# CloudEngineHub/dexrobot_isaac

Hardware: AMD Instinct MI355X
Metric: env-steps/sec BlindGrasping num_envs=4096 per MI355X (random actions) (higher is better)
Workload: dtype f32

## Files before the change

__graft_entry__.py:

```python
import os
import sys

ROOT = os.path.dirname(os.path.abspath(__file__))
if ROOT not in sys.path:
    sys.path.insert(0, ROOT)


def build():
    from dexrobot_isaac_amd.build import build_lib
    path = build_lib(force=True)
    from dexrobot_isaac_amd.build import build_debug_spin
    build_debug_spin(force=True)
    from oracle.oracle import build as build_oracle
    build_oracle(force=True)
    import dexrobot_isaac_amd
    from dexrobot_isaac_amd import _lib
    _lib.load()
    print(f"built {path}")


def smoke():
    import numpy as np
    import torch
    from dexrobot_isaac_amd.config import build_sim_config, default_cfg
    from dexrobot_isaac_amd.core import DexSimCore
    from oracle.oracle import Oracle
    cfg = default_cfg("BlindGrasping")
    cfg["env"]["numEnvs"] = 64
    sc, model = build_sim_config(cfg)
    ms = model.to_struct()
    core = DexSimCore(sc, ms, "cuda:0")
    orc = Oracle(sc, ms)
    core.reset()
    obs_ref = orc.reset()
    torch.cuda.synchronize()
    np.testing.assert_allclose(core.obs_buf.cpu().numpy(), obs_ref, atol=2e-4)
    rng = np.random.default_rng(0)
    for _ in range(3):
        a = (2 * rng.random((64, 18)) - 1).astype(np.float32)
        core.step(torch.as_tensor(a, device="cuda:0"))
        o_ref, r_ref, d_ref = orc.step(a)
        torch.cuda.synchronize()
        np.testing.assert_allclose(core.obs_buf.cpu().numpy(), o_ref, atol=5e-4)
        np.testing.assert_allclose(core.rew_buf.cpu().numpy(), r_ref, atol=5e-3, rtol=1e-4)
        assert (core.reset_buf.cpu().numpy() == d_ref).all()
    print("smoke ok: HIP step matches the CPU oracle")


if __name__ == "__main__":
    build()
```

dexrobot_isaac_amd/build.py:

```python
import os
import shutil
import subprocess

HERE = os.path.dirname(os.path.abspath(__file__))
CSRC = os.path.join(HERE, "csrc")
LIB = os.path.join(HERE, "libdexsim.so")
SOURCES = ["dexsim.hip", "dexsim_device.h", "dexsim_physics.hip.inc", "dexsim_l2.hip.inc", "dexsim_state.hip.inc",
           "dexsim_chain.hip.inc", "dexsim_render.hip.inc", "dexsim_kindyn.hip.inc", "dexsim_ik.hip.inc", "dexsim_proximity.hip.inc",
           "dexsim_invdyn.hip.inc"]


DEBUG_SPIN_LIB = os.path.join(HERE, "libdexsim_dbgspin.so")
CODEGEN_FLAGS = ["--offload-arch=gfx950", "-O3", "-fno-slp-vectorize", "-fno-hip-fp32-correctly-rounded-divide-sqrt",
                 "-mllvm", "-amdgpu-sched-strategy=max-ilp", "-std=c++17"]


def _stale(lib=LIB):
    if not os.path.exists(lib):
        return True
    t = os.path.getmtime(lib)
    deps = [os.path.join(CSRC, s) for s in SOURCES] + [os.path.join(HERE, "..", "include", "dexsim.h")]
    return any(os.path.getmtime(d) > t for d in deps if os.path.exists(d))


def build_debug_spin(force=False, bound=2000000):
    return build_lib(force=force, defs=(f"-DDEXSIM_DEBUG_SPIN={int(bound)}",), out=DEBUG_SPIN_LIB)


def build_lib(force=False, verbose=False, defs=(), out=None):
    lib = out or LIB
    if not force and not _stale(lib):
        return lib
    hipcc = shutil.which("hipcc") or "/opt/rocm/bin/hipcc"
    if not os.path.exists(hipcc):
        raise RuntimeError("hipcc not found: libdexsim.so cannot be built on this machine")
    cmd = [hipcc, *CODEGEN_FLAGS, "-fPIC", "-shared", *defs, "-o", lib, os.path.join(CSRC, "dexsim.hip")]
    if verbose:
        print(" ".join(cmd))
    subprocess.check_call(cmd, cwd=CSRC)
    return lib


if __name__ == "__main__":
    print(build_lib(force=True, verbose=True))
```

dexrobot_isaac_amd/csrc/dexsim_physics.hip.inc:

```

#define GPTR(p) ((__attribute__((address_space(1))) __typeof__(*(p))*)(p))
#define FLD(f, r) GPTR(A.f)[(size_t)(r) * N + e]
#define ROWADDR(w, lane) ((((w) >> 2) * 64 + (lane)) * 4 + ((w) & 3))

DI int wave_role(int w) { return w == 2 ? 5 : ((w >= 3 && w <= 5) ? w - 1 : w); }
#ifndef SPEC_SPLIT_NUM
#define SPEC_SPLIT_NUM 12
#endif

#define CODE_TYPE(c) ((c) & 3)
#define CODE_CAP(c) (((c) >> 2) & 31)
#define CODE_SAMPLE(c) (((c) >> 7) & 7)
#define CODE_FINGER(c) ((((c) >> 16) & 7) - 1)
#define CODE_LEVEL(c) (((c) >> 19) & 3)
#define CODE_FSLOT(c) (((c) >> 21) & 31)
DI int code_info(const DexHandModel& M, int cap) {
  const int jp = M.cap_parent[cap];
  return ((jp >= 6 ? ((jp - 6) >> 2) + 1 : 0) << 16) | ((jp >= 6 ? (jp - 6) & 3 : 0) << 19) | (M.cap_fslot[cap] << 21);
}
#define CODE_HKEY(c) (CODE_TYPE(c) == 3 ? 88 + ((CODE_FINGER(c) * 4 + CODE_LEVEL(c)) * 2 + (CODE_SAMPLE(c) & 1)) \
                                         : (CODE_CAP(c) * 2 + CODE_TYPE(c)) * 2 + (CODE_SAMPLE(c) & 1))
#define SPLIT_NB(s) ((s) & 15)
#define SPLIT_NX(s) (((s) >> 4) & 15)
#define SPLIT_NF(s, f) (((s) >> (8 + 4 * (f))) & 15)
#define SPLIT_RS(s) (((s) >> 28) & 1)
#define NP_TAG 0x40000000
#define NP_COUNT(w) (((w) >> 1) & 0x7f)
#define NP_TMASK(w) (((w) >> 8) & 0x7fff)
DI int split_pack(int nbg, const int (&cnt)[6], int hmask) {
  int nh = 0;
#pragma unroll
  for (int w = 0; w < 6; w++) nh += cnt[w];
  const int rs = nh > 12 ? 1 : 0;
  int split = max(1, (nh + rs) >> rs) | (rs << 28);
  int a = 0;
#pragma unroll
  for (int w = 0; w < 6; w++) {
    if (w < 5) split |= (cnt[w] > 0 ? (((a + cnt[w] - 1) >> rs) - (a >> rs) + 1) : 1) << (8 + 4 * w);
    a += cnt[w];
  }
  const int bmask = rs ? ((hmask | (hmask >> 1)) & 0x555555) : hmask;
  const int nX = (nbg > 0 ? 1 : 0) + __popc(bmask);
  return split | (max(nX, 1) << 4);
}
DI void push_contact(const Arena& A, int N, int e, int& nc, int type, int cap, int sample, V3 p, V3 n, float gap, float mu, int sw = -1,
                     int* tmask = nullptr, int cinfo = 0) {
  if (sw >= 0) {
    if (nc >= NP_STAGE) return;
    if (tmask && type == 1) *tmask |= 1 << nc;
    const int sc = sw * NP_STAGE + nc;
    *FQ(cstage, 2 * sc) = f4{p.x, p.y, p.z, n.x};
    *FQ(cstage, 2 * sc + 1) = f4{n.y, n.z, gap, mu};
    FLD(cstage, CSTAGE_CODE0 + sc) = __int_as_float(type | (cap << 2) | (sample << 7) | cinfo);
    nc++;
    return;
  }
  if (nc >= DEXSIM_KMAX) return;
  if (tmask && type == 1) *tmask |= 1 << nc;
  *FQ(cgeom, 2 * nc) = f4{p.x, p.y, p.z, n.x};
  *FQ(cgeom, 2 * nc + 1) = f4{n.y, n.z, gap, mu};
  FLD(ccode, nc) = type | (cap << 2) | (sample << 7) | cinfo;
  nc++;
}

DI void sphere_box(V3 P, float r, float hb, V3& nl, V3& pl, float& gapraw) {
  V3 qv = {clampf(P.x, -hb, hb), clampf(P.y, -hb, hb), clampf(P.z, -hb, hb)};
  V3 d = P - qv;
  float d2 = dot(d, d);
  if (d2 > 1e-12f) {
    float dist = sqrt_n(d2);
    nl = {div_n(d.x, dist), div_n(d.y, dist), div_n(d.z, dist)};
    pl = qv;
    gapraw = dist - r;
  } else {
    float px = hb - fabsf(P.x), py = hb - fabsf(P.y), pz = hb - fabsf(P.z);
    int ax = 0; float best = px;
    if (py < best) { best = py; ax = 1; }
    if (pz < best) { best = pz; ax = 2; }
    float c = ax == 0 ? P.x : (ax == 1 ? P.y : P.z);
    float sgn = c >= 0.f ? 1.f : -1.f;
    nl = {ax == 0 ? sgn : 0.f, ax == 1 ? sgn : 0.f, ax == 2 ? sgn : 0.f};
    pl = {ax == 0 ? sgn * hb : P.x, ax == 1 ? sgn * hb : P.y, ax == 2 ? sgn * hb : P.z};
    gapraw = -best - r;
  }
}

DI float seg_box_dfdt(V3 a, V3 d, float t, float hb) {
  V3 Pt = {a.x + t * d.x, a.y + t * d.y, a.z + t * d.z};
  V3 ex = {Pt.x - clampf(Pt.x, -hb, hb), Pt.y - clampf(Pt.y, -hb, hb), Pt.z - clampf(Pt.z, -hb, hb)};
  return ex.x * d.x + ex.y * d.y + ex.z * d.z;
}

DI void collide_capsule(const Arena& A, int N, int e, int& nc, const DexSimConfig& C, int cap, V3 e0, V3 e1, float r,
                        bool has_box, V3 bpos, const M3& Rb, float hb, float mu_hb, float mu_hg, int sw = -1, int* tmask = nullptr, int cinfo = 0) {
  const float co = C.contact_offset, rest = C.rest_offset;
  if (has_box) {
    V3 a = mulT(Rb, e0 - bpos), b = mulT(Rb, e1 - bpos), d = b - a;
    V3 mid = {0.5f * (a.x + b.x), 0.5f * (a.y + b.y), 0.5f * (a.z + b.z)};
    float reach = 0.5f * norm_n(d) + r + 1.7320508f * hb + co;
    bool near = dot(mid, mid) < reach * reach;
    if (__any(near)) {
      if (near) {
        float lo = 0.f, hi = 1.f;
#pragma unroll 4
        for (int it = 0; it < DEXSIM_BISECT_ITERS; it++) {
          float mdl = 0.5f * (lo + hi);
          if (seg_box_dfdt(a, d, mdl, hb) > 0.f) hi = mdl; else lo = mdl;
        }
        float ts = 0.5f * (lo + hi);
        const float tp = ts <= 0.02f ? 0.f : (ts >= 0.98f ? 1.f : ts);
        for (int s = 0; s < 2; s++) {
          float tc = s == 0 ? tp : (tp < 0.5f ? 1.f : 0.f);
          V3 Pc = {a.x + tc * d.x, a.y + tc * d.y, a.z + tc * d.z}, nl, pl;
          float gr;
          sphere_box(Pc, r, hb, nl, pl, gr);
          if (gr < co) push_contact(A, N, e, nc, 1, cap, s, mul(Rb, pl) + bpos, mul(Rb, nl), gr - rest, mu_hb, sw, tmask, cinfo);
        }
      }
    }
  }
  float z0 = e0.z - r, z1 = e1.z - r;
  if (z0 < co) push_contact(A, N, e, nc, 0, cap, 0, v3(e0.x, e0.y, z0), v3(0, 0, 1), z0 - rest, mu_hg, sw, tmask, cinfo);
  if (z1 < co) push_contact(A, N, e, nc, 0, cap, 1, v3(e1.x, e1.y, z1), v3(0, 0, 1), z1 - rest, mu_hg, sw, tmask, cinfo);
}

DI void collide_capsules3(const Arena& A, int N, int e, int& nc, const DexSimConfig& C, const int (&cap)[3], const V3 (&E0)[3],
                          const V3 (&E1)[3], const float (&r)[3], bool has_box, V3 bpos, const M3& Rb, float hb, float mu_hb, float mu_hg,
                          int sw, int* tmask, const int (&cinfo)[3]) {
  const float co = C.contact_offset, rest = C.rest_offset;
  V3 a[3], d[3];
  bool near[3] = {false, false, false};
  float ts[3] = {0.f, 0.f, 0.f};
  if (has_box) {
#pragma unroll
    for (int c = 0; c < 3; c++) {
      a[c] = mulT(Rb, E0[c] - bpos);
      const V3 b = mulT(Rb, E1[c] - bpos);
      d[c] = b - a[c];
      const V3 mid = {0.5f * (a[c].x + b.x), 0.5f * (a[c].y + b.y), 0.5f * (a[c].z + b.z)};
      const float reach = 0.5f * norm_n(d[c]) + r[c] + 1.7320508f * hb + co;
      near[c] = dot(mid, mid) < reach * reach;
    }
    if (__any(near[0] || near[1] || near[2])) {
      float lo[3] = {0.f, 0.f, 0.f}, hi[3] = {1.f, 1.f, 1.f};
#pragma unroll 2
      for (int it = 0; it < DEXSIM_BISECT_ITERS; it++) {
#pragma unroll
        for (int c = 0; c < 3; c++) {
          const float mdl = 0.5f * (lo[c] + hi[c]);
          if (seg_box_dfdt(a[c], d[c], mdl, hb) > 0.f) hi[c] = mdl; else lo[c] = mdl;
        }
      }
#pragma unroll
      for (int c = 0; c < 3; c++) ts[c] = 0.5f * (lo[c] + hi[c]);
    }
  }
#pragma unroll
  for (int c = 0; c < 3; c++) {
    const V3 ac = a[c], dc = d[c], e0 = E0[c], e1 = E1[c];
    const float rc = r[c], tsc = ts[c];
    const bool nr = near[c];
    const int capc = cap[c], ci = cinfo[c];
    if (has_box && nr) {
      const float tp = tsc <= 0.02f ? 0.f : (tsc >= 0.98f ? 1.f : tsc);
      for (int s = 0; s < 2; s++) {
        const float tc = s == 0 ? tp : (tp < 0.5f ? 1.f : 0.f);
        V3 Pc = {ac.x + tc * dc.x, ac.y + tc * dc.y, ac.z + tc * dc.z}, nl, pl;
        float gr;
        sphere_box(Pc, rc, hb, nl, pl, gr);
        if (gr < co) push_contact(A, N, e, nc, 1, capc, s, mul(Rb, pl) + bpos, mul(Rb, nl), gr - rest, mu_hb, sw, tmask, ci);
      }
    }
    const float z0 = e0.z - rc, z1 = e1.z - rc;
    if (z0 < co) push_contact(A, N, e, nc, 0, capc, 0, v3(e0.x, e0.y, z0), v3(0, 0, 1), z0 - rest, mu_hg, sw, tmask, ci);
    if (z1 < co) push_contact(A, N, e, nc, 0, capc, 1, v3(e1.x, e1.y, z1), v3(0, 0, 1), z1 - rest, mu_hg, sw, tmask, ci);
  }
}


struct BaseChain {
  V3 ab[6], ob[6];
  float qb[6], qdb[6];
  Q4 q5;
  V3 o5, w5, al5, ao5;
};

DI Q4 qmul_axis_y(Q4 a, float s, float c) {
  return {fmaf(-a.z, s, mulr(a.x, c)), fmaf(a.y, c, mulr(a.w, s)), fmaf(a.z, c, mulr(a.x, s)), fmaf(-a.y, s, mulr(a.w, c))};
}
DI Q4 qmul_axis_z(Q4 a, float s, float c) {
  return {fmaf(a.y, s, mulr(a.x, c)), fmaf(a.y, c, -mulr(a.x, s)), fmaf(a.z, c, mulr(a.w, s)), fmaf(-a.z, s, mulr(a.w, c))};
}
DI V3 q2mat_col_y(Q4 q) {
  return {2.f * fmaf(q.x, q.y, -mulr(q.z, q.w)), fmaf(fmaf(q.z, q.z, mulr(q.x, q.x)), -2.f, 1.f), 2.f * fmaf(q.y, q.z, mulr(q.x, q.w))};
}
DI V3 q2mat_col_z(Q4 q) {
  return {2.f * fmaf(q.x, q.z, mulr(q.y, q.w)), 2.f * fmaf(q.y, q.z, -mulr(q.x, q.w)), fmaf(fmaf(q.y, q.y, mulr(q.x, q.x)), -2.f, 1.f)};
}

template <bool MS>
DI void base_chain(const Arena& A, const DevParams* __restrict__ P, V3 grav, int N, int e, BaseChain& B, bool write_jframe,
                   const float* s_q = nullptr, const float* s_qd = nullptr, int lane = 0) {
#pragma unroll
  for (int j = 0; j < 6; j++) {
    if (s_q) { B.qb[j] = s_q[j * 64 + lane]; B.qdb[j] = s_qd[j * 64 + lane]; }
    else { B.qb[j] = FLD(q, j); B.qdb[j] = FLD(qd, j); }
  }
  V3 t = {0, 0, 0};
#pragma unroll
  for (int j = 0; j < 4; j++) {
    const V3 Aj = v3p(P->base_A[j]);
    if (j < 3) t += B.qb[j] * Aj;
    B.ab[j] = Aj;
    B.ob[j] = v3p(P->base_Oc[j]) + t;
  }
  Q4 qc;
  {
    const V3 ax = v3p(P->jc[3].axis);
    float s, c;
    sincos_joint(0.5f * B.qb[3], &s, &c);
    qc = qmul(q4p(P->base_Q3z), Q4{ax.x * s, ax.y * s, ax.z * s, c});
  }
  V3 oc = B.ob[3];
  V3 w = B.qdb[3] * B.ab[3], al = {0, 0, 0}, ao = {-grav.x, -grav.y, -grav.z};
#pragma unroll
  for (int j = 4; j < 6; j++) {
    if (MS) {
      const V3 aw = j == 4 ? q2mat_col_y(qc) : q2mat_col_z(qc);
      float s, c;
      sincos_joint(0.5f * B.qb[j], &s, &c);
      const Q4 qn = j == 4 ? qmul_axis_y(qc, s, c) : qmul_axis_z(qc, s, c);
      const V3 cw = cross(w, aw);
      al += B.qdb[j] * cw; w += B.qdb[j] * aw;
      B.ab[j] = aw; B.ob[j] = oc; qc = qn;
      continue;
    }
    M3 Rp = q2mat(qc);
    V3 on = oc + mul(Rp, v3p(P->jc[j].poff));
    Q4 qz = qmul(qc, q4p(P->jc[j].qoff));
    V3 ax = v3p(P->jc[j].axis);
    V3 aw = mul(q2mat(qz), ax);
    float s, c;
    sincos_joint(0.5f * B.qb[j], &s, &c);
    Q4 qn = qmul(qz, Q4{ax.x * s, ax.y * s, ax.z * s, c});
    V3 r = on - oc;
    V3 aoj = ao + cross(al, r) + cross(w, cross(w, r));
    V3 cw = cross(w, aw);
    al += B.qdb[j] * cw; w += B.qdb[j] * aw;
    ao = aoj; B.ab[j] = aw; B.ob[j] = on; qc = qn; oc = on;
  }
  B.q5 = qc; B.o5 = oc; B.w5 = w; B.al5 = al; B.ao5 = ao;
  if (write_jframe) {
#pragma unroll
    for (int j = 0; j < 6; j++) {
      FLD(jframe, 6 * j + 0) = B.ab[j].x; FLD(jframe, 6 * j + 1) = B.ab[j].y; FLD(jframe, 6 * j + 2) = B.ab[j].z;
      FLD(jframe, 6 * j + 3) = B.ob[j].x; FLD(jframe, 6 * j + 4) = B.ob[j].y; FLD(jframe, 6 * j + 5) = B.ob[j].z;
    }
  }
}

DI bool hand_clear(const DevParams* __restrict__ P, const BaseChain& B, V3 bpos) {
  const DexSimConfig& C = P->cfg;
  const float reach = P->hand_reach, co = C.contact_offset;
  bool clear = B.o5.z - reach > co;
  if (C.has_box) {
    const V3 d = B.o5 - bpos;
    const float rr = reach + 0.8660254f * C.box_size * 1.001f + co;
    clear = clear && dot(d, d) > rr * rr;
  }
  return __all(clear);
}

DI bool capsule_clear(V3 e0, V3 e1, float r, const DexSimConfig& C, V3 bpos, const M3& Rb) {
  const float co = C.contact_offset;
  bool clear = !((e0.z - r) < co) && !((e1.z - r) < co);
  if (C.has_box) {
    const V3 d = e1 - e0;
    const V3 mid = mulT(Rb, V3{0.5f * (e0.x + e1.x) - bpos.x, 0.5f * (e0.y + e1.y) - bpos.y, 0.5f * (e0.z + e1.z) - bpos.z});
    const float hb = 0.5f * C.box_size;
    const V3 ex = {mid.x - clampf(mid.x, -hb, hb), mid.y - clampf(mid.y, -hb, hb), mid.z - clampf(mid.z, -hb, hb)};
    const float reach = (0.5f * norm_n(d) + r + co) * 1.0001f + 1e-6f;
    clear = clear && !(dot(ex, ex) < reach * reach);
  }
  return clear;
}

#define SH(i) sh[(i) * 64 + lane]
DI void sh_put3(float* sh, int lane, int i, V3 v) { SH(i) = v.x; SH(i + 1) = v.y; SH(i + 2) = v.z; }
DI void comp_put(float* sh, int lane, int w, const Comp& c, V3 o5) {
  const V3 d = c.c - o5;
  const S6 J = c.I + pa(c.m, d);
  sh[(w) * 64 + lane] = c.m; sh_put3(sh, lane, w + 1, d);
  sh[(w + 4) * 64 + lane] = J.xx; sh[(w + 5) * 64 + lane] = J.yy; sh[(w + 6) * 64 + lane] = J.zz;
  sh[(w + 7) * 64 + lane] = J.xy; sh[(w + 8) * 64 + lane] = J.xz; sh[(w + 9) * 64 + lane] = J.yz;
}
DI V3 sh_get3(const float* sh, int lane, int i) { return {SH(i), SH(i + 1), SH(i + 2)}; }
DI void bch_get2(const float* s_bch, int lane, int i2, V3& a0, V3& o0, V3& a1, V3& o1) {
  const f4 q0 = *(const f4*)(s_bch + ROWADDR(12 * i2, lane)), q1 = *(const f4*)(s_bch + ROWADDR(12 * i2 + 4, lane)),
           q2 = *(const f4*)(s_bch + ROWADDR(12 * i2 + 8, lane));
  a0 = {q0.x, q0.y, q0.z}; o0 = {q0.w, q1.x, q1.y}; a1 = {q1.z, q1.w, q2.x}; o1 = {q2.y, q2.z, q2.w};
}


#define DL_SINV 0
#define DL_SCHUR_S 0
#define DL_SCHUR_GSUM 27
#define DL_PALM 36
#define DL_PALM_WRENCH 46
#define DL_NC 52
#define DL_PERSIST 53
#define DL_SSUB(b, f) ((b) + (f) * 43)
#define DL_GSUM(b, f) ((b) + (f) * 43 + 21)
#define DL_COMP(b, f) ((b) + (f) * 43 + 27)
#define DL_WRENCH(b, f) ((b) + (f) * 43 + 37)
#define DL_CAPS(b, f) ((b) + 215 + (f) * 18)
#define DL_HANDOFF 305
#define DL_WORDS (DL_PERSIST + DL_HANDOFF)
#define DL_SPLIT DL_WORDS

#define FS_UB 53
#define FS_BOXV 59
#define FS_UF 65
#define FS_LAM 85
#define FS_HDR 157
#define FS_ROW 197
#define FS_HDR_HI 197
#define FS_X 253
#define FS_FORCE 253
#define FS_T 513
#define FS_SPRE 513
#define FS_SPRE_BIAS 534
#define FS_BCH 545
#define FS_CTAB 581
#define FS_NITEM 593
#define FS_CMP 594
#define FS_CARRY_QD 606
#define FS_CARRY_BP 612
#define FS_COMPCNT 615
#define FS_GEN 617
#define FS_SPLIT 618
#define FS_CPACK 619
#define FS_CMP_INVM 620
#define FS_FLAG 622
#define FS_CARRY_Q 628
#define FS_TGTB 634
#define FS_WORDS 640
#define FS_LDS_BYTES (FS_WORDS * 64 * sizeof(float))

enum : unsigned { LIVE_ACROSS = 1u << 6, LIVE_PUB = 1u << 7, LIVE_POST = 1u << 8 };
constexpr unsigned lds_live(int first, int last) {
  unsigned m = 0;
  for (int p = first; p <= last; p++) m |= 1u << (p == 0 ? 1 : p);
  return m;
}
constexpr unsigned LIVE_CARRY = lds_live(5, 5) | LIVE_ACROSS | lds_live(0, 0);
constexpr unsigned LIVE_LAUNCH = lds_live(0, 5) | LIVE_ACROSS;
struct LdsRegion { int start, words; unsigned live; };
constexpr LdsRegion LDS_MAP[] = {
  {DL_SINV,      36,                      lds_live(2, 3)},
  {DL_PALM,      16,                      lds_live(1, 2)},
  {DL_NC,        1,                       lds_live(1, 5)},
  {FS_UB,        6,                       lds_live(2, 5)},
  {FS_BOXV,      6,                       lds_live(1, 5)},
  {FS_UF,        20,                      lds_live(1, 5)},
  {FS_LAM,       3 * DEXSIM_KMAX,         lds_live(1, 5)},
  {FS_HDR,       FS_HDR_HI - FS_HDR,      lds_live(1, 5)},
  {FS_ROW,       DL_HANDOFF,              lds_live(1, 2)},
  {FS_HDR_HI,    4 * DEXSIM_KMAX - (FS_HDR_HI - FS_HDR), lds_live(3, 5)},
  {FS_X,         13 * 5 * 4,              lds_live(3, 4)},
  {FS_FORCE,     5 * 3 * DEXSIM_NFSLOT,   lds_live(5, 5)},
  {FS_T,         8 * 4,                   lds_live(3, 4)},
  {FS_SPRE,      27,                      lds_live(1, 2)},
  {FS_BCH,       36,                      lds_live(1, 3)},
  {FS_CTAB,      12,                      lds_live(2, 4)},
  {FS_NITEM,     1,                       lds_live(2, 4)},
  {FS_CMP,       12,                      lds_live(1, 4)},
  {FS_CARRY_QD,  6,                       LIVE_CARRY},
  {FS_CARRY_BP,  3,                       LIVE_CARRY},
  {FS_COMPCNT,   1,                       LIVE_LAUNCH},
  {FS_GEN,       1,                       lds_live(1, 4)},
  {FS_SPLIT,     1,                       lds_live(2, 4)},
  {FS_CPACK,     1,                       lds_live(1, 4)},
  {FS_CMP_INVM,  2,                       lds_live(1, 4)},
  {FS_FLAG,      6,                       LIVE_LAUNCH},
  {FS_CARRY_Q,   6,                       LIVE_CARRY},
  {FS_TGTB,      6,                       lds_live(1, 2)},
};
constexpr int lds_map_conflict(LdsRegion extra = {0, 0, 0}) {
  constexpr int n = sizeof(LDS_MAP) / sizeof(LDS_MAP[0]);
  for (int i = 0; i <= n; i++) {
    const LdsRegion a = i < n ? LDS_MAP[i] : extra;
    if (a.start < 0 || a.words < 0 || a.start + a.words > FS_WORDS) return 1000 * (a.start < 0 ? 0 : a.start) + 999;
    for (int j = 0; j < i; j++) {
      const LdsRegion b = LDS_MAP[j];
      if ((a.live & b.live) && a.start < b.start + b.words && b.start < a.start + a.words) return 1000 * a.start + b.start;
    }
  }
  return -1;
}
static_assert(FS_LDS_BYTES == 160 * 1024, "the sub-step kernels own the CU's whole LDS: one workgroup per CU");
static_assert(lds_map_conflict() < 0, "LDS map: a region leaves the LDS or shares a word with a region live in a common phase "
                                      "(the note shows 1000 x the first word of one + the first word of the other)");
static_assert(DL_CAPS(0, 5) == DL_HANDOFF, "the per-finger hand-off is DL_HANDOFF words");
#define SOLVE_LDS_WORDS(kstage) (60 + DEXSIM_KMAX * 3 + DEXSIM_KMAX * 4 + (kstage) * 3 * CROW_W)
static_assert((DL_SPLIT + 1) * 64 * sizeof(float) <= FS_LDS_BYTES, "k_dynamics' LDS does not fit into the CU's");
static_assert(SOLVE_LDS_WORDS(4) * 64 * sizeof(float) <= FS_LDS_BYTES, "k_solve's LDS does not fit into the CU's");

struct FingerIn { float ql[4], qdl[4], tg[4]; };
DI void finger_load(const Arena& A, int f, int N, int e, FingerIn& in) {
#pragma unroll
  for (int l = 0; l < 4; l++) { const int j = 6 + 4 * f + l; in.ql[l] = FLD(q, j); in.qdl[l] = FLD(qd, j); in.tg[l] = FLD(targets, j); }
}

template <bool MS>
DI bool finger_dynamics(const Arena& A, const DevParams* __restrict__ P, const BaseChain& B, const FingerIn& in, float* sh, const int dlb,
                        float* s_uf, int lane, int f, int N, int e, int tok_seq = 0, bool sphere_clear = false,
                        V3 bpos = V3{0, 0, 0}, const M3& Rb = M3{{1, 0, 0, 0, 1, 0, 0, 0, 1}}, float* Gk = nullptr) {
  const DexHandModel& M = P->model;
  const float h = P->h;
  const int j0 = 6 + 4 * f;
  Q4 qf = B.q5; V3 of = B.o5; V3 wf = B.w5, alf = B.al5, aof = B.ao5;
  V3 a[4], o[4], cl[4], fl[4], nl[4];
  S6 Iw[4];
  float ql[4], qdl[4], tg[4];
  bool clr = true;
  if (tok_seq > 0 && sphere_clear && lane == 0) sh[(FS_FLAG + f) * 64] = __int_as_float((tok_seq << 1) | 1);
#pragma unroll
  for (int l = 0; l < 4; l++) {
    const int j = j0 + l;
    ql[l] = in.ql[l]; qdl[l] = in.qdl[l]; tg[l] = in.tg[l];
    M3 Rp = q2mat(qf);
    V3 on = of + mul(Rp, v3p(P->jc[j].poff));
    Q4 qz = qmul(qf, q4p(P->jc[j].qoff));
    V3 ax = v3p(P->jc[j].axis);
    float s, c;
    sincos_joint(0.5f * ql[l], &s, &c);
    Q4 qn = qmul(qz, Q4{ax.x * s, ax.y * s, ax.z * s, c});
    M3 R = q2mat(qn);
    V3 aw = MS && l >= 1 ? V3{mulr(R.m[1], ax.y), mulr(R.m[4], ax.y), mulr(R.m[7], ax.y)} : mul(R, ax);
    V3 r = on - of;
    V3 aoj = aof + cross(alf, r) + cross(wf, cross(wf, r));
    V3 cw = cross(wf, aw);
    alf += qdl[l] * cw; wf += qdl[l] * aw; aof = aoj;
    cl[l] = on + mul(R, v3p(P->jc[j].com));
    Iw[l] = (tok_seq > 0 && P->inertia_diag) ? rotate_inertia_diag(R, P->jc[j].inertia) : rotate_inertia(R, P->jc[j].inertia);
    V3 rc = cl[l] - on;
    V3 ac = aof + cross(alf, rc) + cross(wf, cross(wf, rc));
    fl[l] = P->jc[j].mass * ac;
    nl[l] = mul(Iw[l], alf) + cross(wf, mul(Iw[l], wf)) + cross(rc, fl[l]);
    if (l >= 1 && !(tok_seq > 0 && sphere_clear)) {
      const int cap = 3 + 3 * f + (l - 1);
      const V3 c0 = on + mul(R, v3p(M.cap_p0[cap])), c1 = on + mul(R, v3p(M.cap_p1[cap]));
      sh_put3(sh, lane, DL_CAPS(dlb, f) + 6 * (l - 1), c0);
      sh_put3(sh, lane, DL_CAPS(dlb, f) + 6 * (l - 1) + 3, c1);
      if (tok_seq > 0) clr = clr && capsule_clear(c0, c1, M.cap_r[cap], P->cfg, bpos, Rb);
    }
    a[l] = aw; o[l] = on; qf = qn; of = on;
  }
  bool fclear = false;
  if (tok_seq > 0) {
    fclear = sphere_clear || __all(clr);
    if (!sphere_clear && lane == 0) sh[(FS_FLAG + f) * 64] = __int_as_float((tok_seq << 1) | (fclear ? 1 : 0));
  }
  if (!fclear) {
    const float w24[24] = {a[0].x, a[0].y, a[0].z, o[0].x, o[0].y, o[0].z, a[1].x, a[1].y, a[1].z, o[1].x, o[1].y, o[1].z,
                           a[2].x, a[2].y, a[2].z, o[2].x, o[2].y, o[2].z, a[3].x, a[3].y, a[3].z, o[3].x, o[3].y, o[3].z};
#pragma unroll
    for (int qd = 0; qd < 6; qd++) *FQ(jframe, JFRAME_FQ0 + 6 * f + qd) = f4{w24[4 * qd], w24[4 * qd + 1], w24[4 * qd + 2], w24[4 * qd + 3]};
  }
  float bias[4];
#pragma unroll
  for (int l = 3; l >= 0; l--) {
    bias[l] = dot(a[l], nl[l]);
    if (l > 0) { fl[l - 1] += fl[l]; nl[l - 1] += nl[l] + cross(o[l] - o[l - 1], fl[l]); }
  }
  sh_put3(sh, lane, DL_WRENCH(dlb, f), fl[0]);
  sh_put3(sh, lane, DL_WRENCH(dlb, f) + 3, nl[0] + cross(o[0] - B.o5, fl[0]));
  float Fm[16], Cm[24];
  Comp cc;
#pragma unroll
  for (int l = 3; l >= 0; l--) {
    Comp b; b.m = P->jc[j0 + l].mass; b.c = cl[l]; b.I = Iw[l];
    if (l == 3) cc = b; else { comp_add(b, cc); cc = b; }
    V3 Pm = cc.m * cross(a[l], cc.c - o[l]);
    V3 Lm = mul(cc.I, a[l]);
#pragma unroll
    for (int k = 0; k <= l; k++) {
      float v = dot(a[k], Lm + cross(cc.c - o[k], Pm));
      Fm[l * 4 + k] = v; Fm[k * 4 + l] = v;
    }
    if (MS) {
      const V3 Xm = Lm + cross(cc.c - B.ob[3], Pm);
      Cm[l] = Pm.x; Cm[4 + l] = Pm.y; Cm[8 + l] = Pm.z;
#pragma unroll
      for (int i = 3; i < 6; i++) Cm[i * 4 + l] = dot(B.ab[i], Xm);
    } else {
#pragma unroll
      for (int i = 0; i < 6; i++)
        Cm[i * 4 + l] = i < 3 ? dot(B.ab[i], Pm) : dot(B.ab[i], Lm + cross(cc.c - B.ob[i], Pm));
    }
  }
  comp_put(sh, lane, DL_COMP(dlb, f), cc, B.o5);
  if (tok_seq > 0) {
    asm volatile("" ::: "memory");
    if (lane == 0) __hip_atomic_fetch_add((int*)(sh + FS_COMPCNT * 64), 1, __ATOMIC_RELAXED, __HIP_MEMORY_SCOPE_WORKGROUP);
  }
  float tau[4];
#pragma unroll
  for (int l = 0; l < 4; l++) {
    const int j = j0 + l;
    const float kp = P->jc[j].kp, kdh = P->jc[j].kd + h * kp;
    Fm[l * 4 + l] += P->jc[j].armature + h * kdh;
    tau[l] = kp * (tg[l] - ql[l]) - kdh * qdl[l] - bias[l];
  }
  spd_inverse<4>(Fm);
  float G[24];
  f2 G2[12];
#pragma unroll
  for (int l = 0; l < 4; l++)
#pragma unroll
    for (int ip = 0; ip < 3; ip++) {
      f2 s2 = {0.f, 0.f};
#pragma unroll
      for (int k = 0; k < 4; k++) s2 = f2{Cm[(2 * ip) * 4 + k], Cm[(2 * ip + 1) * 4 + k]} * Fm[l * 4 + k] + s2;
      G2[l * 3 + ip] = s2;
      G[l * 6 + 2 * ip] = s2.x; G[l * 6 + 2 * ip + 1] = s2.y;
    }
  if (!(tok_seq > 0 && sphere_clear && Gk)) {
#pragma unroll
    for (int qd = 0; qd < 6; qd++) *FQ(fac_g, 6 * f + qd) = f4{G[4 * qd], G[4 * qd + 1], G[4 * qd + 2], G[4 * qd + 3]};
  }
  if (Gk) {
#pragma unroll
    for (int i = 0; i < 24; i++) Gk[i] = G[i];
  }
#pragma unroll
  for (int i = 0; i < 6; i++)
#pragma unroll
    for (int kp = 0; kp <= i / 2; kp++) {
      f2 s2 = {0.f, 0.f};
#pragma unroll
      for (int l = 0; l < 4; l++) s2 = G2[l * 3 + kp] * Cm[i * 4 + l] + s2;
      SH(DL_SSUB(dlb, f) + i * (i + 1) / 2 + 2 * kp) = s2.x;
      if (2 * kp + 1 <= i) SH(DL_SSUB(dlb, f) + i * (i + 1) / 2 + 2 * kp + 1) = s2.y;
    }
  if (!fclear) {
    *FQ(fac_finv, 3 * f) = f4{Fm[0], Fm[4], Fm[5], Fm[8]};
    *FQ(fac_finv, 3 * f + 1) = f4{Fm[9], Fm[10], Fm[12], Fm[13]};
    *FQ(fac_finv, 3 * f + 2) = f4{Fm[14], Fm[15], 0.f, 0.f};
  }
#pragma unroll
  for (int ip = 0; ip < 3; ip++) {
    f2 s2 = {0.f, 0.f};
#pragma unroll
    for (int l = 0; l < 4; l++) s2 = G2[l * 3 + ip] * tau[l] + s2;
    SH(DL_GSUM(dlb, f) + 2 * ip) = s2.x; SH(DL_GSUM(dlb, f) + 2 * ip + 1) = s2.y;
  }
#pragma unroll
  for (int l = 0; l < 4; l++) {
    float s = qdl[l];
#pragma unroll
    for (int i = 0; i < 6; i++) s += G[l * 6 + i] * B.qdb[i];
    float acc = 0.f;
#pragma unroll
    for (int k = 0; k < 4; k++) acc += Fm[l * 4 + k] * tau[k];
    const float uf = s + h * acc;
    if (s_uf) s_uf[(4 * f + l) * 64 + lane] = uf;
    else FLD(ufree, j0 + l) = uf;
  }
  return fclear;
}

#define SCHUR_SPLIT_BIT (1 << 30)
#ifdef DEXSIM_DEBUG_SPIN
#define SPIN_GUARD_INIT() int spin_polls_ = 0
#define SPIN_GUARD(cntp, site, seq) if (++spin_polls_ > (DEXSIM_DEBUG_SPIN)) { if (cntp) GPTR(cntp)[CNT_SPIN_TIMEOUT] = ((site) << 24) | (seq); break; }
#else
#define SPIN_GUARD_INIT() do {} while (0)
#define SPIN_GUARD(cntp, site, seq) do {} while (0)
#endif
DI Comp schur_comp(const float* sh, const int dlb, int lane, V3 o5) {
  float M = SH(DL_PALM);
  V3 sd = M * sh_get3(sh, lane, DL_PALM + 1);
  S6 J = {SH(DL_PALM + 4), SH(DL_PALM + 5), SH(DL_PALM + 6), SH(DL_PALM + 7), SH(DL_PALM + 8), SH(DL_PALM + 9)};
#pragma unroll
  for (int f = 0; f < 5; f++) {
    const float mf = SH(DL_COMP(dlb, f));
    M += mf;
    sd += mf * sh_get3(sh, lane, DL_COMP(dlb, f) + 1);
    J = J + S6{SH(DL_COMP(dlb, f) + 4), SH(DL_COMP(dlb, f) + 5), SH(DL_COMP(dlb, f) + 6), SH(DL_COMP(dlb, f) + 7), SH(DL_COMP(dlb, f) + 8), SH(DL_COMP(dlb, f) + 9)};
  }
  const float inv = M > 0.f ? 1.f / M : 0.f;
  const V3 d = inv * sd;
  const S6 sh_back = pa(M, d);
  Comp c;
  c.m = M; c.c = o5 + d;
  c.I = {J.xx - sh_back.xx, J.yy - sh_back.yy, J.zz - sh_back.zz, J.xy - sh_back.xy, J.xz - sh_back.xz, J.yz - sh_back.yz};
  return c;
}
template <int i, int k0 = 0, int k1 = i>
DI void schur_row(float* sh, const int dlb, int lane) {
  float r[k1 - k0 + 1];
#pragma unroll
  for (int k = k0; k <= k1; k++) {
    const float v = SH(FS_SPRE + i * (i + 1) / 2 + k);
    float ss = 0.f;
#pragma unroll
    for (int f = 0; f < 5; f++) ss += SH(DL_SSUB(dlb, f) + i * (i + 1) / 2 + k);
    r[k - k0] = v - ss;
  }
#pragma unroll
  for (int k = k0; k <= k1; k++) SH(DL_SCHUR_S + i * (i + 1) / 2 + k) = r[k - k0];
}
DI void schur_precompute(float* sh, const int dlb, int lane, const BaseChain& B, int seq, int* dbg_cnt) {
  {
    SPIN_GUARD_INIT();
    while (*(volatile int*)(sh + FS_COMPCNT * 64) < 5 * seq) { __builtin_amdgcn_s_sleep(2); SPIN_GUARD(dbg_cnt, 4, seq); }
  }
  asm volatile("" ::: "memory");
  const Comp comp5 = schur_comp(sh, dlb, lane, B.o5);
  int idx = 0;
#pragma unroll
  for (int i = 0; i < 6; i++) {
    V3 Pm, Lm;
    if (i < 3) { Pm = comp5.m * B.ab[i]; Lm = {0, 0, 0}; }
    else { Pm = comp5.m * cross(B.ab[i], comp5.c - B.ob[i]); Lm = mul(comp5.I, B.ab[i]); }
#pragma unroll
    for (int k = 0; k <= i; k++) {
      SH(FS_SPRE + idx) = k < 3 ? dot(B.ab[k], Pm) : dot(B.ab[k], Lm + cross(comp5.c - B.ob[k], Pm));
      idx++;
    }
  }
  V3 ff = sh_get3(sh, lane, DL_PALM_WRENCH), nn = sh_get3(sh, lane, DL_PALM_WRENCH + 3);
#pragma unroll
  for (int f = 0; f < 5; f++) {
    ff += sh_get3(sh, lane, DL_WRENCH(dlb, f));
    nn += sh_get3(sh, lane, DL_WRENCH(dlb, f) + 3);
  }
  SH(FS_SPRE_BIAS + 5) = dot(B.ab[5], nn);
#pragma unroll
  for (int j = 4; j >= 0; j--) {
    nn += cross(B.ob[j + 1] - B.ob[j], ff);
    SH(FS_SPRE_BIAS + j) = j < 3 ? dot(B.ab[j], ff) : dot(B.ab[j], nn);
  }
}
DI void schur_helper(float* sh, const int dlb, int job, int lane) {
  if (job == 1) {
    float gsum[6] = {0, 0, 0, 0, 0, 0};
#pragma unroll
    for (int f = 0; f < 5; f++)
#pragma unroll
      for (int i = 0; i < 6; i++) gsum[i] += SH(DL_GSUM(dlb, f) + i);
#pragma unroll
    for (int i = 0; i < 6; i++) SH(DL_SCHUR_GSUM + i) = gsum[i];
    schur_row<0>(sh, dlb, lane); schur_row<1>(sh, dlb, lane); schur_row<2>(sh, dlb, lane);
  } else if (job == 0) {
    schur_row<3>(sh, dlb, lane); schur_row<5, 4, 5>(sh, dlb, lane);
  } else schur_row<4>(sh, dlb, lane);
}

DI void schur_base(const Arena& A, const DevParams* __restrict__ P, const BaseChain& B, float* sh, const int dlb, float* uB_out,
                   int lane, int N, int e, int tgt_lds = -1, bool solve_only = false, int split_seq = 0,
                   unsigned long long dbg_t0 = 0, int dbg_row = 0, int* dbg_cnt = nullptr) {
#if defined(DEXSIM_PROFILE_PHASES) && defined(DBG_SCHUR)
#define SCHUR_STAMP(i) do { if (lane == 0) A.crow[(size_t)(dbg_row + (i)) * N + e] = __int_as_float((int)(__builtin_amdgcn_s_memtime() - dbg_t0)); } while (0)
#else
#define SCHUR_STAMP(i) do {} while (0)
#endif
  const float h = P->h;
  SCHUR_STAMP(0);
  Comp comp5;
  V3 f5 = sh_get3(sh, lane, DL_PALM_WRENCH), n5 = sh_get3(sh, lane, DL_PALM_WRENCH + 3);
  float Ssub[21], gsum[6] = {0, 0, 0, 0, 0, 0};
#pragma unroll
  for (int i = 0; i < 21; i++) Ssub[i] = 0.f;
  if (split_seq == 0) comp5 = schur_comp(sh, dlb, lane, B.o5);
  if (split_seq == 0) {
#pragma unroll
    for (int f = 0; f < 5; f++) {
      f5 += sh_get3(sh, lane, DL_WRENCH(dlb, f));
      n5 += sh_get3(sh, lane, DL_WRENCH(dlb, f) + 3);
#pragma unroll
      for (int i = 0; i < 21; i++) Ssub[i] += SH(DL_SSUB(dlb, f) + i);
#pragma unroll
      for (int i = 0; i < 6; i++) gsum[i] += SH(DL_GSUM(dlb, f) + i);
    }
  }
  SCHUR_STAMP(1);
  float S[36];
  if (split_seq > 0) schur_row<5, 0, 3>(sh, dlb, lane);
  else {
    int idx = 0;
#pragma unroll
    for (int i = 0; i < 6; i++) {
      V3 Pm, Lm;
      if (i < 3) { Pm = comp5.m * B.ab[i]; Lm = {0, 0, 0}; }
      else { Pm = comp5.m * cross(B.ab[i], comp5.c - B.ob[i]); Lm = mul(comp5.I, B.ab[i]); }
#pragma unroll
      for (int k = 0; k <= i; k++) {
        float v = k < 3 ? dot(B.ab[k], Pm) : dot(B.ab[k], Lm + cross(comp5.c - B.ob[k], Pm));
        v -= Ssub[idx++];
        S[i * 6 + k] = v; S[k * 6 + i] = v;
      }
    }
  }
  SCHUR_STAMP(2);
  float tauB[6];
  float bias[6];
  if (split_seq > 0) {
    const int want = (split_seq << 1) | 1 | SCHUR_SPLIT_BIT;
#pragma unroll 1
    for (int w = 1; w <= 3; w++) {
      SPIN_GUARD_INIT();
      while (__float_as_int(*(volatile float*)(sh + (FS_FLAG + w) * 64)) != want) { __builtin_amdgcn_s_sleep(1); SPIN_GUARD(dbg_cnt, 1, split_seq); }
    }
    asm volatile("" ::: "memory");
    SCHUR_STAMP(3);
    {
      int idx = 0;
#pragma unroll
      for (int i = 0; i < 6; i++)
#pragma unroll
        for (int k = 0; k <= i; k++) {
          const float v = SH(DL_SCHUR_S + idx); idx++;
          S[i * 6 + k] = v; S[k * 6 + i] = v;
        }
    }
#pragma unroll
    for (int i = 0; i < 6; i++) { bias[i] = SH(FS_SPRE_BIAS + i); gsum[i] = SH(DL_SCHUR_GSUM + i); }
  } else {
    V3 nn = n5, ff = f5;
    bias[5] = dot(B.ab[5], nn);
#pragma unroll
    for (int j = 4; j >= 0; j--) {
      nn += cross(B.ob[j + 1] - B.ob[j], ff);
      bias[j] = j < 3 ? dot(B.ab[j], ff) : dot(B.ab[j], nn);
    }
  }
  {
#pragma unroll
    for (int i = 0; i < 6; i++) {
      const float kp = P->jc[i].kp, kdh = P->jc[i].kd + h * kp;
      S[i * 6 + i] += P->jc[i].armature + h * kdh;
      const float tgt = tgt_lds >= 0 ? SH(tgt_lds + i) : FLD(targets, i);
      tauB[i] = kp * (tgt - B.qb[i]) - kdh * B.qdb[i] - bias[i] - gsum[i];
    }
  }
  SCHUR_STAMP(4);
  if (solve_only) {
    float x[6];
    spd_solve<6>(S, tauB, x);
#pragma unroll
    for (int i = 0; i < 6; i++) uB_out[i] = B.qdb[i] + h * x[i];
    SCHUR_STAMP(5);
    return;
  }
  spd_inverse<6>(S);
#pragma unroll
  for (int qd = 0; qd < 9; qd++) *(f4*)(sh + DL_SINV * 64 + ROWADDR(4 * qd, lane)) = f4{S[4 * qd], S[4 * qd + 1], S[4 * qd + 2], S[4 * qd + 3]};
#pragma unroll
  for (int i = 0; i < 6; i++) {
    float acc = 0.f;
#pragma unroll
    for (int k = 0; k < 6; k++) acc += S[i * 6 + k] * tauB[k];
    const float ub = B.qdb[i] + h * acc;
    if (uB_out) uB_out[i] = ub;
    else FLD(ufree, i) = ub;
  }
}

template <bool FUSED>
DI void build_contact_rows(const Arena& A, const DevParams* __restrict__ P, const BaseChain* B, float* sh, int lane, int k, int N, int e,
                           int split, int gen) {
  const DexSimConfig& C = P->cfg;
  const float h = P->h;
  const f4 cg0 = *FQ(cgeom, 2 * k), cg1 = *FQ(cgeom, 2 * k + 1);
  const V3 p = {cg0.x, cg0.y, cg0.z};
  const V3 n = {cg0.w, cg1.x, cg1.y};
  const float gap = cg1.z, mu_k = cg1.w;
  const int code = FLD(ccode, k), type = CODE_TYPE(code);
  float inv_m = 0.f, inv_I = 0.f;
  V3 bpos = {0, 0, 0};
  if (C.has_box) {
    if (!C.box_fixed) { inv_m = rcp_n(FLD(box_mass, 0)); inv_I = P->box_inv_I_k * inv_m; }
    bpos = {FLD(box_pos, 0), FLD(box_pos, 1), FLD(box_pos, 2)};
  }
  const int f = type != 2 ? CODE_FINGER(code) : -1, lvl = f >= 0 ? CODE_LEVEL(code) : -1;
  const int nFi = (split && f >= 0) ? SPLIT_NF(split, f) : 1;
  const float nB = split ? (float)SPLIT_NB(split) : 1.f, nX = split ? (float)SPLIT_NX(split) : 1.f, nF = (float)nFi;
  f4 wq = {0.f, 0.f, 0.f, 0.f};
  if (gen >= 0) wq = *(const __attribute__((address_space(1))) f4*)(A.wlam + ((size_t)(type == 2 ? 80 + k : CODE_HKEY(code)) * N + e) * 4);
  float jfr[24], G[24], Fi[10];
  if (f >= 0) {
    const unsigned qs = (unsigned)N * 16u, oe = (unsigned)e * 16u;
    const unsigned oj = (unsigned)(JFRAME_FQ0 + 6 * f) * qs + oe, og = (unsigned)(6 * f) * qs + oe, of = (unsigned)(3 * f) * qs + oe;
    f4 qj[6], qg[6], qf[3];
#pragma unroll
    for (int qd = 0; qd < 6; qd++) {
      qj[qd] = *(const __attribute__((address_space(1))) f4*)((const char*)A.jframe + (oj + (unsigned)qd * qs));
      qg[qd] = *(const __attribute__((address_space(1))) f4*)((const char*)A.fac_g + (og + (unsigned)qd * qs));
    }
#pragma unroll
    for (int qd = 0; qd < 3; qd++) qf[qd] = *(const __attribute__((address_space(1))) f4*)((const char*)A.fac_finv + (of + (unsigned)qd * qs));
#pragma unroll
    for (int qd = 0; qd < 6; qd++) {
      jfr[4 * qd] = qj[qd].x; jfr[4 * qd + 1] = qj[qd].y; jfr[4 * qd + 2] = qj[qd].z; jfr[4 * qd + 3] = qj[qd].w;
      G[4 * qd] = qg[qd].x; G[4 * qd + 1] = qg[qd].y; G[4 * qd + 2] = qg[qd].z; G[4 * qd + 3] = qg[qd].w;
    }
    Fi[0] = qf[0].x; Fi[1] = qf[0].y; Fi[2] = qf[0].z; Fi[3] = qf[0].w; Fi[4] = qf[1].x; Fi[5] = qf[1].y; Fi[6] = qf[1].z; Fi[7] = qf[1].w;
    Fi[8] = qf[2].x; Fi[9] = qf[2].y;
  }
  const bool lim = type == 3;
  V3 dir[3];
  dir[0] = n;
  tangent_basis(lim ? v3(0, 0, 1) : n, dir[1], dir[2]);
  if (lim) { dir[1] = v3(0, 0, 0); dir[2] = v3(0, 0, 0); }
  float t[3][6], jf[3][4], St[3][6], Fj[3][4];
#pragma unroll
  for (int r = 0; r < 3; r++) {
#pragma unroll
    for (int i = 0; i < 6; i++) { t[r][i] = 0.f; St[r][i] = 0.f; }
#pragma unroll
    for (int l = 0; l < 4; l++) { jf[r][l] = 0.f; Fj[r][l] = 0.f; }
  }
  float Dq[3] = {0.f, 0.f, 0.f};
  float A10 = 0.f, A20 = 0.f, A21 = 0.f;
  if (type != 2) {
#pragma unroll
    for (int i2 = 0; i2 < 3; i2++) {
      V3 aa[2], oo[2];
      if (FUSED) {
        bch_get2(sh + FS_BCH * 64, lane, i2, aa[0], oo[0], aa[1], oo[1]);
      } else { aa[0] = B->ab[2 * i2]; oo[0] = B->ob[2 * i2]; aa[1] = B->ab[2 * i2 + 1]; oo[1] = B->ob[2 * i2 + 1]; }
#pragma unroll
      for (int h = 0; h < 2; h++) {
        const int i = 2 * i2 + h;
        const V3 ci = i < 3 ? aa[h] : cross(aa[h], p - oo[h]);
#pragma unroll
        for (int r = 0; r < 3; r++) t[r][i] = dot(dir[r], ci);
      }
    }
    if (f >= 0) {
#pragma unroll
      for (int l = 0; l < 4; l++) {
        const V3 al = {jfr[6 * l], jfr[6 * l + 1], jfr[6 * l + 2]}, ol = {jfr[6 * l + 3], jfr[6 * l + 4], jfr[6 * l + 5]};
        const V3 cl = cross(al, p - ol);
#pragma unroll
        for (int r = 0; r < 3; r++) jf[r][l] = l <= lvl ? dot(dir[r], cl) : 0.f;
        if (lim) jf[0][l] = l == lvl ? (CODE_SAMPLE(code) ? -1.f : 1.f) : 0.f;
      }
#pragma unroll
      for (int l = 0; l < 4; l++)
#pragma unroll
        for (int i = 0; i < 6; i++)
#pragma unroll
          for (int r = 0; r < 3; r++) t[r][i] -= G[l * 6 + i] * jf[r][l];
#pragma unroll
      for (int l = 0; l < 4; l++)
#pragma unroll
        for (int kk = 0; kk < 4; kk++) {
          const float fv = Fi[l >= kk ? l * (l + 1) / 2 + kk : kk * (kk + 1) / 2 + l];
#pragma unroll
          for (int r = 0; r < 3; r++) Fj[r][l] += fv * jf[r][kk];
        }
#pragma unroll
      for (int r = 0; r < 3; r++) {
        float s = 0.f;
#pragma unroll
        for (int l = 0; l < 4; l++) s += jf[r][l] * Fj[r][l];
        Dq[r] += nF * s;
      }
      A10 += nF * (jf[1][0] * Fj[0][0] + jf[1][1] * Fj[0][1] + jf[1][2] * Fj[0][2] + jf[1][3] * Fj[0][3]);
      A20 += nF * (jf[2][0] * Fj[0][0] + jf[2][1] * Fj[0][1] + jf[2][2] * Fj[0][2] + jf[2][3] * Fj[0][3]);
      A21 += nF * (jf[2][0] * Fj[1][0] + jf[2][1] * Fj[1][1] + jf[2][2] * Fj[1][2] + jf[2][3] * Fj[1][3]);
    }
#pragma unroll
    for (int i2 = 0; i2 < 3; i2++) {
      const f4 s0 = *(const f4*)(sh + DL_SINV * 64 + ROWADDR(12 * i2, lane)), s1 = *(const f4*)(sh + DL_SINV * 64 + ROWADDR(12 * i2 + 4, lane)),
               s2 = *(const f4*)(sh + DL_SINV * 64 + ROWADDR(12 * i2 + 8, lane));
      const float si[12] = {s0.x, s0.y, s0.z, s0.w, s1.x, s1.y, s1.z, s1.w, s2.x, s2.y, s2.z, s2.w};
#pragma unroll
      for (int h = 0; h < 2; h++)
#pragma unroll
        for (int r = 0; r < 3; r++) {
          float s = 0.f;
#pragma unroll
          for (int kk = 0; kk < 6; kk++) s += si[6 * h + kk] * t[r][kk];
          St[r][2 * i2 + h] = s;
        }
    }
#pragma unroll
    for (int r = 0; r < 3; r++) {
      float s = 0.f;
#pragma unroll
      for (int i = 0; i < 6; i++) s += t[r][i] * St[r][i];
      Dq[r] += nB * s;
    }
    {
      float s10 = 0.f, s20 = 0.f, s21 = 0.f;
#pragma unroll
      for (int i = 0; i < 6; i++) { s10 += t[1][i] * St[0][i]; s20 += t[2][i] * St[0][i]; s21 += t[2][i] * St[1][i]; }
      A10 += nB * s10; A20 += nB * s20; A21 += nB * s21;
    }
  }
  V3 db[3], rxd[3];
#pragma unroll
  for (int r = 0; r < 3; r++) { db[r] = {0, 0, 0}; rxd[r] = {0, 0, 0}; }
  if (type == 1 || type == 2) {
    const float sgn = type == 2 ? 1.f : -1.f;
    const V3 rb = p - bpos;
#pragma unroll
    for (int r = 0; r < 3; r++) {
      const V3 c = cross(rb, dir[r]);
      db[r] = sgn * dir[r]; rxd[r] = sgn * c;
      Dq[r] += nX * (inv_m + inv_I * dot(c, c));
    }
    const float xm = nX * inv_m, xI = nX * inv_I;
    A10 += xm * dot(db[1], db[0]) + xI * dot(rxd[1], rxd[0]);
    A20 += xm * dot(db[2], db[0]) + xI * dot(rxd[2], rxd[0]);
    A21 += xm * dot(db[2], db[1]) + xI * dot(rxd[2], rxd[1]);
  }
#pragma unroll
  for (int r = 0; r < 3; r++) {
    const float Dinv = (lim && r > 0) ? 0.f : 1.f / (Dq[r] + 1e-9f);
    const float pad = r == 0 ? A10 : (r == 1 ? A20 : A21);
    const int rw = (k * 3 + r) * CROW_W;
    if (FUSED) {
      float* qb = A.crowq + ((size_t)(k * 21 + r * 7) * N + e) * 4;
      st4_global(qb, t[r][0], t[r][1], t[r][2], t[r][3]);
      st4_global(qb + (size_t)1 * N * 4, t[r][4], t[r][5], jf[r][0], jf[r][1]);
      st4_global(qb + (size_t)2 * N * 4, jf[r][2], jf[r][3], St[r][0], St[r][1]);
      st4_global(qb + (size_t)3 * N * 4, St[r][2], St[r][3], St[r][4], St[r][5]);
      st4_global(qb + (size_t)4 * N * 4, Fj[r][0], Fj[r][1], Fj[r][2], Fj[r][3]);
      st4_global(qb + (size_t)5 * N * 4, db[r].x, db[r].y, db[r].z, rxd[r].x);
      st4_global(qb + (size_t)6 * N * 4, rxd[r].y, rxd[r].z, Dinv, pad);
    } else {
#pragma unroll
      for (int i = 0; i < 6; i++) { FLD(crow, rw + i) = t[r][i]; FLD(crow, rw + 10 + i) = St[r][i]; }
#pragma unroll
      for (int l = 0; l < 4; l++) { FLD(crow, rw + 6 + l) = jf[r][l]; FLD(crow, rw + 16 + l) = Fj[r][l]; }
      FLD(crow, rw + 20) = db[r].x; FLD(crow, rw + 21) = db[r].y; FLD(crow, rw + 22) = db[r].z;
      FLD(crow, rw + 23) = rxd[r].x; FLD(crow, rw + 24) = rxd[r].y; FLD(crow, rw + 25) = rxd[r].z;
      FLD(crow, rw + 26) = Dinv; FLD(crow, rw + 27) = pad;
    }
  }
  const float cb = gap > 0.f ? div_n(gap, h) : -fminf(div_n(-gap * C.erp, h), C.max_depenetration_velocity);
  const bool warm = gen >= 0 && __float_as_int(wq.w) == 8 * gen + (type == 2 ? CODE_SAMPLE(code) : 0);
  if (!FUSED) {
    FLD(clam, 3 * k) = warm ? wq.x : 0.f; FLD(clam, 3 * k + 1) = warm ? wq.y : 0.f; FLD(clam, 3 * k + 2) = warm ? wq.z : 0.f;
    FLD(chdr, 8 * k + 0) = __int_as_float(code | (nFi << 12));
    FLD(chdr, 8 * k + 1) = __int_as_float(f >= 0 ? 4 * f : -1);
    FLD(chdr, 8 * k + 2) = mu_k;
    FLD(chdr, 8 * k + 3) = cb;
  }
  FLD(chdr, 8 * k + 4) = __int_as_float(CODE_FSLOT(code));
  FLD(chdr, 8 * k + 5) = n.x; FLD(chdr, 8 * k + 6) = n.y; FLD(chdr, 8 * k + 7) = n.z;
  if (FUSED) {
    float* s_hdr = sh + FS_HDR * 64;
    float* s_lam = sh + FS_LAM * 64;
    s_hdr[(4 * k) * 64 + lane] = __int_as_float(code | (nFi << 12)); s_hdr[(4 * k + 1) * 64 + lane] = __int_as_float(f >= 0 ? 4 * f : -1);
    s_hdr[(4 * k + 2) * 64 + lane] = mu_k; s_hdr[(4 * k + 3) * 64 + lane] = cb;
    s_lam[(3 * k) * 64 + lane] = warm ? wq.x : 0.f; s_lam[(3 * k + 1) * 64 + lane] = warm ? wq.y : 0.f;
    s_lam[(3 * k + 2) * 64 + lane] = warm ? wq.z : 0.f;
  }
}

__global__ __launch_bounds__(384) void k_dynamics(Arena A, const DevParams* __restrict__ P, int N) {
  __shared__ __attribute__((aligned(16))) float sh[(DL_SPLIT + 1) * 64];
  constexpr int dlb = DL_PERSIST;
  const int wv = threadIdx.x >> 6, lane = threadIdx.x & 63;
  const int e = blockIdx.x * 64 + lane;
  const DexHandModel& M = P->model;
  const DexSimConfig& C = P->cfg;
  const V3 grav = v3p(C.gravity);
  const bool has_box = C.has_box != 0;
  BaseChain B;
  FingerIn fin;
  if (wv < 5) finger_load(A, wv, N, e, fin);
  base_chain<false>(A, P, grav, N, e, B, wv == 5);

  int nc = 0;
  V3 bpos = {0, 0, 0}; M3 Rb = q2mat(Q4{0, 0, 0, 1});
  float hb = 0.f, bmu = 0.f;
  if (wv < 5) {
    finger_dynamics<false>(A, P, B, fin, sh, dlb, nullptr, lane, wv, N, e);
  } else {
    const M3 R5 = q2mat(B.q5);
    Comp comp5;
    comp5.m = P->jc[5].mass;
    comp5.c = B.o5 + mul(R5, v3p(P->jc[5].com));
    comp5.I = rotate_inertia(R5, P->jc[5].inertia);
    V3 rc = comp5.c - B.o5;
    V3 ac = B.ao5 + cross(B.al5, rc) + cross(B.w5, cross(B.w5, rc));
    V3 f5 = comp5.m * ac;
    V3 n5 = mul(comp5.I, B.al5) + cross(B.w5, mul(comp5.I, B.w5)) + cross(rc, f5);
    comp_put(sh, lane, DL_PALM, comp5, B.o5);
    sh_put3(sh, lane, DL_PALM_WRENCH, f5); sh_put3(sh, lane, DL_PALM_WRENCH + 3, n5);
    const float h = P->h;
    if (has_box) {
      bpos = {FLD(box_pos, 0), FLD(box_pos, 1), FLD(box_pos, 2)};
      Rb = q2mat(Q4{FLD(box_quat, 0), FLD(box_quat, 1), FLD(box_quat, 2), FLD(box_quat, 3)});
      hb = 0.5f * C.box_size;
      bmu = FLD(box_mu, 0);
      const float mu_bg = 0.5f * (bmu + C.ground_friction);
#pragma unroll
      for (int i = 0; i < 8; i++) {
        V3 l = {(i & 1) ? hb : -hb, (i & 2) ? hb : -hb, (i & 4) ? hb : -hb};
        V3 p = mul(Rb, l) + bpos;
        if (!C.box_fixed && p.z < C.contact_offset && nc < 4) push_contact(A, N, e, nc, 2, 0, i, p, v3(0, 0, 1), p.z - C.rest_offset, mu_bg, -1, nullptr, DEXSIM_FSLOT_BOX << 21);
      }
      const float hg = C.box_fixed ? 0.f : h;
      FLD(ufree, 26) = FLD(box_lin, 0) + hg * grav.x;
      FLD(ufree, 27) = FLD(box_lin, 1) + hg * grav.y;
      FLD(ufree, 28) = FLD(box_lin, 2) + hg * grav.z;
      FLD(ufree, 29) = FLD(box_ang, 0); FLD(ufree, 30) = FLD(box_ang, 1); FLD(ufree, 31) = FLD(box_ang, 2);
    } else {
#pragma unroll
      for (int i = 26; i < 32; i++) FLD(ufree, i) = 0.f;
    }
  }
  __syncthreads();

  if (wv == 0) schur_base(A, P, B, sh, dlb, nullptr, lane, N, e);
  if (wv == 5) {
    const float mu_hg = 0.5f * (M.hand_friction + C.ground_friction);
    const float mu_hb = 0.5f * (M.hand_friction + bmu);
    const int nbg = nc;
    int cntw[6], tmask = 0;
#pragma unroll 1
    for (int f = 0; f < 5; f++) {
      const int n0 = nc;
#pragma unroll 1
      for (int l = 3; l >= 1; l--) {
        const int cap = 3 + 3 * f + (l - 1);
        const V3 e0 = sh_get3(sh, lane, DL_CAPS(dlb, f) + 6 * (l - 1)), e1 = sh_get3(sh, lane, DL_CAPS(dlb, f) + 6 * (l - 1) + 3);
        collide_capsule(A, N, e, nc, C, cap, e0, e1, M.cap_r[cap], has_box, bpos, Rb, hb, mu_hb, mu_hg, -1, &tmask, code_info(M, cap));
      }
      if (f == 0) cntw[0] = nc - n0; else if (f == 1) cntw[1] = nc - n0; else if (f == 2) cntw[2] = nc - n0; else if (f == 3) cntw[3] = nc - n0; else cntw[4] = nc - n0;
    }
    const M3 R5 = q2mat(B.q5);
    const int n5 = nc;
#pragma unroll 1
    for (int cpl = 0; cpl < 3; cpl++)
      collide_capsule(A, N, e, nc, C, cpl, B.o5 + mul(R5, v3p(M.cap_p0[cpl])), B.o5 + mul(R5, v3p(M.cap_p1[cpl])), M.cap_r[cpl],
                      has_box, bpos, Rb, hb, mu_hb, mu_hg, -1, &tmask, code_info(M, cpl));
    cntw[5] = nc - n5;
    FLD(ncontact, 0) = nc;
    SH(DL_NC) = __int_as_float(nc);
    const int split = split_pack(nbg, cntw, (int)((unsigned)tmask >> nbg));
    FLD(csplit, 0) = split;
    SH(DL_SPLIT) = __int_as_float(split);
  }
  __syncthreads();

  nc = __float_as_int(SH(DL_NC));
  int kmax = nc;
#pragma unroll
  for (int s = 32; s >= 1; s >>= 1) kmax = max(kmax, __shfl_xor(kmax, s));
  const int split = __float_as_int(SH(DL_SPLIT)), gen = FLD(wgen, 0);
#pragma unroll 1
  for (int k = wv; k < kmax; k += 6) {
    if (k < nc) build_contact_rows<false>(A, P, &B, sh, lane, k, N, e, split, gen);
  }
}

DI void solve_masks(const float* s_hdr, int nc, int kmax, int lane, unsigned& hand_mask, unsigned& fing_mask, unsigned& box_mask) {
  hand_mask = fing_mask = box_mask = 0;
  for (int k = 0; k < kmax; k++) {
    const int code = __float_as_int(s_hdr[(4 * k) * 64 + lane]), fo = __float_as_int(s_hdr[(4 * k + 1) * 64 + lane]);
    const int type = code & 3;
    const bool act = k < nc;
    if (__any(act && type != 2)) hand_mask |= 1u << k;
    if (__any(act && type != 2 && fo >= 0)) fing_mask |= 1u << k;
    if (__any(act && type != 0)) box_mask |= 1u << k;
  }
}

struct BoxBlock {
  float rx[4], ry[4], rz[4];
  float Dv[4][3], A10[4], A20[4], A21[4], mu4[4], cb4[4], lam4[4][3];
  float im, iI;
  int kms;
  template <bool QUAD>
  DI void load(int kmax, float inv_m, float inv_I, const float* s_lam, const float* s_hdr, const float* rows, int rw, int ro, int lane,
               int nc_lane, bool resume, float split = 1.f) {
    kms = __builtin_amdgcn_readfirstlane(kmax);
    inv_m *= split; inv_I *= split;
    im = inv_m; iI = inv_I;
#pragma unroll
    for (int k = 0; k < 4; k++) {
      const bool use = k < kms && (nc_lane < 0 || k < nc_lane);
      float x = 0.f, y = 0.f, z = 0.f;
      if (k < kms) {
        if (QUAD) {
          y = rows[ROWADDR((k * 3) * rw + ro + 3, lane)]; x = -rows[ROWADDR((k * 3) * rw + ro + 4, lane)];
          z = rows[ROWADDR((k * 3 + 1) * rw + ro + 3, lane)];
        } else {
          x = rows[(3 * k) * 64 + lane]; y = rows[(3 * k + 1) * 64 + lane]; z = rows[(3 * k + 2) * 64 + lane];
        }
      }
      rx[k] = use ? x : 0.f; ry[k] = use ? y : 0.f; rz[k] = use ? z : 0.f;
      mu4[k] = use ? s_hdr[(4 * k + 2) * 64 + lane] : 0.f;
      cb4[k] = use ? s_hdr[(4 * k + 3) * 64 + lane] : 0.f;
#pragma unroll
      for (int r = 0; r < 3; r++) lam4[k][r] = (use && resume) ? s_lam[(3 * k + r) * 64 + lane] : 0.f;
      const float xx = rx[k] * rx[k], yy = ry[k] * ry[k], zz = rz[k] * rz[k];
      Dv[k][0] = use ? 1.f / (inv_m + inv_I * (xx + yy) + 1e-9f) : 0.f;
      Dv[k][1] = use ? 1.f / (inv_m + inv_I * (xx + zz) + 1e-9f) : 0.f;
      Dv[k][2] = use ? 1.f / (inv_m + inv_I * (yy + zz) + 1e-9f) : 0.f;
      A10[k] = inv_I * ry[k] * rz[k]; A20[k] = -inv_I * rx[k] * rz[k]; A21[k] = inv_I * rx[k] * ry[k];
    }
  }
  DI bool sweep(f2& v01, f2& v23, f2& v45) {
    float vx = v01.x, vy = v01.y, vz = v23.x, wx = v23.y, wy = v45.x, wz = v45.y;
    bool chg = false;
#pragma unroll
    for (int k = 0; k < 4; k++) {
      if (k < kms) {
        const float vr0 = vz + ry[k] * wx - rx[k] * wy;
        float vr1 = -vy + rz[k] * wx - rx[k] * wz, vr2 = vx + rz[k] * wy - ry[k] * wz;
        const float nl0 = fmaxf(0.f, lam4[k][0] - (vr0 + cb4[k]) * Dv[k][0]);
        const float dl0 = nl0 - lam4[k][0], lim = mu4[k] * nl0;
        vr1 += A10[k] * dl0; vr2 += A20[k] * dl0;
        const float nl1 = __builtin_amdgcn_fmed3f(lam4[k][1] - vr1 * Dv[k][1], -lim, lim);
        const float dl1 = nl1 - lam4[k][1];
        vr2 += A21[k] * dl1;
        const float nl2 = __builtin_amdgcn_fmed3f(lam4[k][2] - vr2 * Dv[k][2], -lim, lim);
        const float dl2 = nl2 - lam4[k][2];
        lam4[k][0] = nl0; lam4[k][1] = nl1; lam4[k][2] = nl2;
        chg = chg || dl0 != 0.f || dl1 != 0.f || dl2 != 0.f;
        apply(k, dl0, dl1, dl2, f2{im, iI}, vx, vy, vz, wx, wy, wz);
      }
    }
    v01 = f2{vx, vy}; v23 = f2{vz, wx}; v45 = f2{wy, wz};
    return chg;
  }
  DI void sweep_delta(f2& v01, f2& v23, f2& v45, f2& d01, f2& d23, f2& d45, f2 mI0) {
    float vx = v01.x, vy = v01.y, vz = v23.x, wx = v23.y, wy = v45.x, wz = v45.y;
    float dx = 0.f, dy = 0.f, dz = 0.f, ex = 0.f, ey = 0.f, ez = 0.f;
#pragma unroll
    for (int k = 0; k < 4; k++) {
      if (k < kms) {
        const float vr0 = vz + ry[k] * wx - rx[k] * wy;
        float vr1 = -vy + rz[k] * wx - rx[k] * wz, vr2 = vx + rz[k] * wy - ry[k] * wz;
        const float nl0 = fmaxf(0.f, lam4[k][0] - (vr0 + cb4[k]) * Dv[k][0]);
        const float dl0 = nl0 - lam4[k][0], lim = mu4[k] * nl0;
        vr1 += A10[k] * dl0; vr2 += A20[k] * dl0;
        const float nl1 = __builtin_amdgcn_fmed3f(lam4[k][1] - vr1 * Dv[k][1], -lim, lim);
        const float dl1 = nl1 - lam4[k][1];
        vr2 += A21[k] * dl1;
        const float nl2 = __builtin_amdgcn_fmed3f(lam4[k][2] - vr2 * Dv[k][2], -lim, lim);
        const float dl2 = nl2 - lam4[k][2];
        lam4[k][0] = nl0; lam4[k][1] = nl1; lam4[k][2] = nl2;
        apply(k, dl0, dl1, dl2, f2{im, iI}, vx, vy, vz, wx, wy, wz);
        apply(k, dl0, dl1, dl2, mI0, dx, dy, dz, ex, ey, ez);
      }
    }
    v01 = f2{vx, vy}; v23 = f2{vz, wx}; v45 = f2{wy, wz};
    d01 = f2{dx, dy}; d23 = f2{dz, ex}; d45 = f2{ey, ez};
  }
  DI void apply(int k, float dl0, float dl1, float dl2, f2 mI, float& vx, float& vy, float& vz, float& wx, float& wy, float& wz) const {
    const float m0 = mI.x * dl0, m1 = mI.x * dl1, m2 = mI.x * dl2, i0 = mI.y * dl0, i1 = mI.y * dl1, i2 = mI.y * dl2;
    vz += m0; vy -= m1; vx += m2;
    wx += ry[k] * i0 + rz[k] * i1;
    wy += rz[k] * i2 - rx[k] * i0;
    wz -= rx[k] * i1 + ry[k] * i2;
  }
  DI void warm(f2& v01, f2& v23, f2& v45, f2 mI) const {
    float vx = v01.x, vy = v01.y, vz = v23.x, wx = v23.y, wy = v45.x, wz = v45.y;
#pragma unroll
    for (int k = 0; k < 4; k++) {
      if (k < kms) apply(k, lam4[k][0], lam4[k][1], lam4[k][2], mI, vx, vy, vz, wx, wy, wz);
    }
    v01 = f2{vx, vy}; v23 = f2{vz, wx}; v45 = f2{wy, wz};
  }
  DI void store(float* s_lam, int lane, int nmine = -1) const {
#pragma unroll
    for (int k = 0; k < 4; k++) {
      if (nmine < 0 || k < nmine) {
#pragma unroll
        for (int r = 0; r < 3; r++) s_lam[(3 * k + r) * 64 + lane] = lam4[k][r];
      }
    }
  }
};

DI void cache_box_ground(const Arena& A, const float* s_lam, int gen, int cpack, int nmine, int lane, int N, int e) {
#pragma unroll
  for (int k = 0; k < 4; k++) {
    if (k < nmine)
      st4_global(A.wlam + ((size_t)(80 + k) * N + e) * 4, s_lam[(3 * k) * 64 + lane], s_lam[(3 * k + 1) * 64 + lane], s_lam[(3 * k + 2) * 64 + lane],
                 __int_as_float(8 * gen + ((cpack >> (3 * k)) & 7)));
  }
}

DI void solve_forces(const Arena& A, const DevParams* __restrict__ P, int* __restrict__ cnt, const float* s_hdr, const float* s_lam,
                     float* s_f, int nc, int lane, int N, int e, int NR) {
  const float h = P->h;
#pragma unroll
  for (int i = 0; i < DEXSIM_NFSLOT * 3; i++) s_f[i * 64 + lane] = 0.f;
  int nhand = 0;
  for (int k = 0; k < nc; k++) {
    const int type = __float_as_int(s_hdr[(4 * k) * 64 + lane]) & 3;
    nhand += type < 2 ? 1 : 0;
    if (type == 3) continue;
    const int slot = __float_as_int(FLD(chdr, 8 * k + 4));
    const V3 n = {FLD(chdr, 8 * k + 5), FLD(chdr, 8 * k + 6), FLD(chdr, 8 * k + 7)};
    V3 t1, t2;
    tangent_basis(n, t1, t2);
    const float l0 = s_lam[(3 * k) * 64 + lane] / h, l1 = s_lam[(3 * k + 1) * 64 + lane] / h, l2 = s_lam[(3 * k + 2) * 64 + lane] / h;
    const V3 F = l0 * n + l1 * t1 + l2 * t2;
    s_f[(3 * slot) * 64 + lane] += F.x; s_f[(3 * slot + 1) * 64 + lane] += F.y; s_f[(3 * slot + 2) * 64 + lane] += F.z;
    if (type == 1) {
      s_f[(3 * DEXSIM_FSLOT_BOX) * 64 + lane] -= F.x; s_f[(3 * DEXSIM_FSLOT_BOX + 1) * 64 + lane] -= F.y;
      s_f[(3 * DEXSIM_FSLOT_BOX + 2) * 64 + lane] -= F.z;
    }
  }
#pragma unroll
  for (int i = 0; i < DEXSIM_NFSLOT * 3; i++) FLD(cforce, i) = s_f[i * 64 + lane];
  if (cnt) {
    int tot = e < NR ? (nc | (nhand << 16)) : 0;
#pragma unroll
    for (int s = 32; s >= 1; s >>= 1) tot += __shfl_xor(tot, s);
    if (lane == 0) { atomicAdd(&cnt[CNT_CONTACTS], tot & 0xffff); if (tot >> 16) atomicAdd(&cnt[CNT_HAND_CONTACTS], tot >> 16); }
  }
}

DI void solve_forces_box(const Arena& A, const DevParams* __restrict__ P, int* __restrict__ cnt, const float* s_lam, int nc, int lane, int N,
                         int e, int NR) {
  const float h = P->h;
  V3 n = v3(0, 0, 1), t1, t2;
  tangent_basis(n, t1, t2);
  V3 acc = {0.f, 0.f, 0.f};
  for (int k = 0; k < nc; k++) {
    const float l0 = s_lam[(3 * k) * 64 + lane] / h, l1 = s_lam[(3 * k + 1) * 64 + lane] / h, l2 = s_lam[(3 * k + 2) * 64 + lane] / h;
    const V3 F = l0 * n + l1 * t1 + l2 * t2;
    acc.x += F.x; acc.y += F.y; acc.z += F.z;
  }
#pragma unroll
  for (int i = 0; i < DEXSIM_NFSLOT * 3; i++) FLD(cforce, i) = 0.f;
  FLD(cforce, 3 * DEXSIM_FSLOT_BOX) = acc.x; FLD(cforce, 3 * DEXSIM_FSLOT_BOX + 1) = acc.y; FLD(cforce, 3 * DEXSIM_FSLOT_BOX + 2) = acc.z;
  if (cnt) {
    int tot = e < NR ? nc : 0;
#pragma unroll
    for (int s = 32; s >= 1; s >>= 1) tot += __shfl_xor(tot, s);
    if (lane == 0) atomicAdd(&cnt[CNT_CONTACTS], tot);
  }
}

DI void forces_partial(const Arena& A, const DevParams* __restrict__ P, const float* s_hdr, const float* s_lam, float* s_f, int nc, int w,
                       int lane, int N, int e) {
  const float rh = rcp_n(P->h);
#pragma unroll
  for (int i = 0; i < DEXSIM_NFSLOT * 3; i++) s_f[i * 64 + lane] = 0.f;
  int slot[5];
  V3 nn[5];
#pragma unroll
  for (int i = 0; i < 5; i++) {
    const int k = w + 5 * i;
    const bool act = k < nc;
    slot[i] = act ? __float_as_int(FLD(chdr, 8 * k + 4)) : 0;
    nn[i] = act ? V3{FLD(chdr, 8 * k + 5), FLD(chdr, 8 * k + 6), FLD(chdr, 8 * k + 7)} : V3{0.f, 0.f, 1.f};
  }
#pragma unroll
  for (int i = 0; i < 5; i++) {
    const int k = w + 5 * i;
    if (k < nc) {
      const int type = __float_as_int(s_hdr[(4 * k) * 64 + lane]) & 3;
      if (type == 3) continue;
      V3 t1, t2;
      tangent_basis(nn[i], t1, t2);
      const float l0 = s_lam[(3 * k) * 64 + lane] * rh, l1 = s_lam[(3 * k + 1) * 64 + lane] * rh, l2 = s_lam[(3 * k + 2) * 64 + lane] * rh;
      const V3 F = l0 * nn[i] + l1 * t1 + l2 * t2;
      const int sl = slot[i];
      s_f[(3 * sl) * 64 + lane] += F.x; s_f[(3 * sl + 1) * 64 + lane] += F.y; s_f[(3 * sl + 2) * 64 + lane] += F.z;
      if (type == 1) {
        s_f[(3 * DEXSIM_FSLOT_BOX) * 64 + lane] -= F.x; s_f[(3 * DEXSIM_FSLOT_BOX + 1) * 64 + lane] -= F.y;
        s_f[(3 * DEXSIM_FSLOT_BOX + 2) * 64 + lane] -= F.z;
      }
    }
  }
}
DI void forces_reduce(const Arena& A, int* __restrict__ cnt, const float* s_hdr, const float* s_f, int nc, int lane, int N, int e, int NR,
                      int w0 = 0, int nw = 1) {
#pragma unroll 3
  for (int i = w0; i < DEXSIM_NFSLOT * 3; i += nw) {
    float v = s_f[i * 64 + lane];
#pragma unroll
    for (int w = 1; w < 5; w++) v += s_f[(w * DEXSIM_NFSLOT * 3 + i) * 64 + lane];
    FLD(cforce, i) = v;
  }
}
DI void contact_stats(int* __restrict__ cnt, const float* s_hdr, int nc, int lane, int e, int NR) {
  if (cnt) {
    int nhand = 0;
    for (int k = 0; k < nc; k++) nhand += (__float_as_int(s_hdr[(4 * k) * 64 + lane]) & 3) < 2 ? 1 : 0;
    int tot = e < NR ? (nc | (nhand << 16)) : 0;
#pragma unroll
    for (int s = 32; s >= 1; s >>= 1) tot += __shfl_xor(tot, s);
    if (lane == 0) { atomicAdd(&cnt[CNT_CONTACTS], tot & 0xffff); if (tot >> 16) atomicAdd(&cnt[CNT_HAND_CONTACTS], tot >> 16); }
  }
}

DI void integrate_joint(const Arena& A, const DevParams* __restrict__ P, float h, int j, float q0, float v, int N, int e,
                        float* q_new = nullptr, float* qd_new = nullptr, bool store = true) {
  float qn = q0 + h * v;
  const float lo = P->jc[j].lo, hi = P->jc[j].hi;
  if (qn < lo) { qn = lo; v = fmaxf(v, 0.f); }
  if (qn > hi) { qn = hi; v = fminf(v, 0.f); }
  if (store) { FLD(q, j) = qn; FLD(qd, j) = v; }
  if (q_new) { *q_new = qn; *qd_new = v; }
}
DI void integrate_box(const Arena& A, float h, const float* vb, const float* wb, int N, int e) {
#pragma unroll
  for (int i = 0; i < 3; i++) { FLD(box_lin, i) = vb[i]; FLD(box_ang, i) = wb[i]; FLD(box_pos, i) = fmaf(h, vb[i], FLD(box_pos, i)); }
  Q4 bq = {FLD(box_quat, 0), FLD(box_quat, 1), FLD(box_quat, 2), FLD(box_quat, 3)};
  Q4 dq = qmul(Q4{wb[0], wb[1], wb[2], 0.f}, bq);
  Q4 qn = {bq.x + 0.5f * h * dq.x, bq.y + 0.5f * h * dq.y, bq.z + 0.5f * h * dq.z, bq.w + 0.5f * h * dq.w};
  float l = sqrt_n(qn.x * qn.x + qn.y * qn.y + qn.z * qn.z + qn.w * qn.w);
  FLD(box_quat, 0) = div_n(qn.x, l); FLD(box_quat, 1) = div_n(qn.y, l); FLD(box_quat, 2) = div_n(qn.z, l); FLD(box_quat, 3) = div_n(qn.w, l);
}

__global__ __launch_bounds__(64) void k_solve(Arena A, const DevParams* __restrict__ P, int* __restrict__ cnt, int stamp, int kstage,
                                              int N, int NR) {
  extern __shared__ float lds[];
  const int lane = threadIdx.x;
  const int e = blockIdx.x * 64 + lane;
  float* s_uf = lds;
  float* s_lam = lds + 60 * 64;
  float* s_hdr = lds + (60 + DEXSIM_KMAX * 3) * 64;
  float* s_row = lds + (60 + DEXSIM_KMAX * 3 + DEXSIM_KMAX * 4) * 64;
  const DexSimConfig& C = P->cfg;
  const float h = P->h;
  const bool has_box = C.has_box != 0;

  float uB[6], vb[3], wb[3];
#pragma unroll
  for (int i = 0; i < 6; i++) uB[i] = FLD(ufree, i);
#pragma unroll
  for (int i = 0; i < 20; i++) s_uf[i * 64 + lane] = FLD(ufree, 6 + i);
#pragma unroll
  for (int i = 0; i < 3; i++) { vb[i] = FLD(ufree, 26 + i); wb[i] = FLD(ufree, 29 + i); }
  const int nc = FLD(ncontact, 0);
  float inv_m = 0.f, inv_I = 0.f;
  if (has_box && !C.box_fixed) { inv_m = rcp_n(FLD(box_mass, 0)); inv_I = P->box_inv_I_k * inv_m; }
  int kmax = nc;
#pragma unroll
  for (int s = 32; s >= 1; s >>= 1) kmax = max(kmax, __shfl_xor(kmax, s));
  const int kst = min(kmax, kstage);
  for (int k = 0; k < kmax * 3; k++) s_lam[k * 64 + lane] = k < nc * 3 ? FLD(clam, k) : 0.f;
#pragma unroll 4
  for (int k = 0; k < kmax; k++) {
    const bool act = k < nc;
    const float w0 = act ? FLD(chdr, 8 * k + 0) : __int_as_float(2), w1 = act ? FLD(chdr, 8 * k + 1) : __int_as_float(0);
    const float w2 = act ? FLD(chdr, 8 * k + 2) : 0.f, w3 = act ? FLD(chdr, 8 * k + 3) : 0.f;
    s_hdr[(4 * k) * 64 + lane] = w0; s_hdr[(4 * k + 1) * 64 + lane] = w1;
    s_hdr[(4 * k + 2) * 64 + lane] = w2; s_hdr[(4 * k + 3) * 64 + lane] = w3;
  }
  unsigned hand_mask, fing_mask, box_mask;
  solve_masks(s_hdr, nc, kmax, lane, hand_mask, fing_mask, box_mask);
  for (int k = 0; k < kst; k++) {
    const int base = k * 3 * CROW_W;
    const bool act = k < nc;
    if ((hand_mask >> k) & 1) {
      float tmp[3 * CROW_W];
#pragma unroll
      for (int w = 0; w < 3 * CROW_W; w++) tmp[w] = act ? FLD(crow, base + w) : 0.f;
#pragma unroll
      for (int w = 0; w < 3 * CROW_W; w++) s_row[ROWADDR(base + w, lane)] = tmp[w];
    } else {
      float tmp[24];
#pragma unroll
      for (int r = 0; r < 3; r++)
#pragma unroll
        for (int w = 0; w < 8; w++) tmp[8 * r + w] = act ? FLD(crow, base + r * CROW_W + 20 + w) : 0.f;
#pragma unroll
      for (int r = 0; r < 3; r++)
#pragma unroll
        for (int w = 0; w < 8; w++) s_row[ROWADDR(base + r * CROW_W + 20 + w, lane)] = tmp[8 * r + w];
    }
  }
  const int gen = FLD(wgen, 0);
  int nbg = 0;
  for (int k = 0; k < min(kmax, 4); k++) nbg += (k < nc && (__float_as_int(s_hdr[(4 * k) * 64 + lane]) & 3) == 2) ? 1 : 0;
  if (hand_mask == 0 && kmax <= 4 && kmax <= kst) {
    BoxBlock bb;
    bb.load<true>(kmax, inv_m, inv_I, s_lam, s_hdr, s_row, CROW_W, 20, lane, nc, true);
    f2 v01 = {vb[0], vb[1]}, v23 = {vb[2], wb[0]}, v45 = {wb[1], wb[2]};
    bb.warm(v01, v23, v45, f2{inv_m, inv_I});
#pragma unroll 1
    for (int it = 0; it < C.num_position_iterations; it++) bb.sweep(v01, v23, v45);
    vb[0] = v01.x; vb[1] = v01.y; vb[2] = v23.x; wb[0] = v23.y; wb[1] = v45.x; wb[2] = v45.y;
    bb.store(s_lam, lane);
  } else {
    const int split = FLD(csplit, 0), rs = SPLIT_RS(split), nh = nc - nbg;
    const float nBf = (float)SPLIT_NB(split), nXf = (float)SPLIT_NX(split);
    float* s_ufl = s_uf + 20 * 64;
    float* s_ufd = s_uf + 40 * 64;
    auto contact = [&](int k, bool act, float (&U)[6], float (&Vb)[3], float (&Wb)[3], float* uf, float sB, float sX, int mode) {
      const int kk = act ? k : 0;
      const int code = __float_as_int(s_hdr[(4 * kk) * 64 + lane]), fo = __float_as_int(s_hdr[(4 * kk + 1) * 64 + lane]);
      const float mu = s_hdr[(4 * kk + 2) * 64 + lane], cb = s_hdr[(4 * kk + 3) * 64 + lane];
      const float sF = mode ? (float)((code >> 12) & 15) : 1.f;
      const bool fing = act && fo >= 0;
      const int foe = max(fo, 0);
      float lam_n = 0.f;
      for (int r = 0; r < 3; r++) {
        const float* rp = A.crow + (size_t)((kk * 3 + r) * CROW_W) * N + e;
        float row[CROW_W];
        for (int w = 0; w < CROW_W; w++) row[w] = act ? rp[(size_t)w * N] : 0.f;
        float lam = act ? s_lam[(3 * kk + r) * 64 + lane] : 0.f, dl;
        if (mode) {
          float vr = 0.f;
          for (int i = 0; i < 6; i++) vr += row[i] * U[i];
          for (int l = 0; l < 4; l++) vr += row[6 + l] * uf[(foe + l) * 64 + lane];
          for (int i = 0; i < 3; i++) vr += row[20 + i] * Vb[i] + row[23 + i] * Wb[i];
          float nl;
          if (r == 0) { nl = fmaxf(0.f, lam - (vr + cb) * row[26]); lam_n = nl; }
          else { const float lim = mu * lam_n; nl = clampf(lam - vr * row[26], -lim, lim); }
          dl = nl - lam;
          if (act) s_lam[(3 * kk + r) * 64 + lane] = nl;
        } else dl = lam;
        for (int i = 0; i < 6; i++) U[i] += row[10 + i] * (sB * dl);
        if (fing) for (int l = 0; l < 4; l++) uf[(foe + l) * 64 + lane] += row[16 + l] * (sF * dl);
        for (int i = 0; i < 3; i++) { Vb[i] += row[20 + i] * (sX * inv_m * dl); Wb[i] += row[23 + i] * (sX * inv_I * dl); }
      }
    };
    for (int k = 0; k < kmax; k++) contact(k, k < nc, uB, vb, wb, s_uf, 1.f, 1.f, 0);
    for (int i = 0; i < 20; i++) s_ufd[i * 64 + lane] = 0.f;
#pragma unroll 1
    for (int it = 0; it < C.num_position_iterations; it++) {
      float dU[6] = {0, 0, 0, 0, 0, 0}, dV[3] = {0, 0, 0}, dW[3] = {0, 0, 0};
#pragma unroll 1
      for (int b = 0; b < 13; b++) {
        if (b < 12 && !__any((b << rs) < nh)) continue;
        float U[6], Vb[3], Wb[3];
        for (int i = 0; i < 6; i++) U[i] = uB[i];
        for (int i = 0; i < 3; i++) { Vb[i] = vb[i]; Wb[i] = wb[i]; }
        for (int i = 0; i < 20; i++) s_ufl[i * 64 + lane] = s_uf[i * 64 + lane];
        for (int i = 0; i < 4; i++) {
          const int k = b == 12 ? i : nbg + (b << rs) + i;
          const bool act = b == 12 ? i < nbg : (i < (1 << rs) && (b << rs) + i < nh);
          if (__any(act)) contact(k, act, U, Vb, Wb, s_ufl, nBf, nXf, 1);
        }
        for (int i = 0; i < 6; i++) dU[i] += (U[i] - uB[i]) / nBf;
        for (int i = 0; i < 3; i++) { dV[i] += (Vb[i] - vb[i]) / nXf; dW[i] += (Wb[i] - wb[i]) / nXf; }
        for (int i = 0; i < 20; i++) s_ufd[i * 64 + lane] += (s_ufl[i * 64 + lane] - s_uf[i * 64 + lane]) / (float)SPLIT_NF(split, i >> 2);
      }
      for (int i = 0; i < 6; i++) uB[i] += dU[i];
      for (int i = 0; i < 3; i++) { vb[i] += dV[i]; wb[i] += dW[i]; }
      for (int i = 0; i < 20; i++) { s_uf[i * 64 + lane] += s_ufd[i * 64 + lane]; s_ufd[i * 64 + lane] = 0.f; }
    }
    for (int k = nbg; k < kmax; k++) {
      if (k < nc) {
        const int code = __float_as_int(s_hdr[(4 * k) * 64 + lane]);
        st4_global(A.wlam + ((size_t)CODE_HKEY(code) * N + e) * 4, s_lam[(3 * k) * 64 + lane], s_lam[(3 * k + 1) * 64 + lane], s_lam[(3 * k + 2) * 64 + lane],
                   __int_as_float(8 * DEXSIM_WGEN_NEXT(gen)));
      }
    }
  }
  {
    int cpack = 0;
    for (int k = 0; k < 4; k++) if (k < nbg) cpack |= CODE_SAMPLE(__float_as_int(s_hdr[(4 * k) * 64 + lane])) << (3 * k);
    cache_box_ground(A, s_lam, DEXSIM_WGEN_NEXT(gen), cpack, nbg, lane, N, e);
    FLD(wgen, 0) = DEXSIM_WGEN_NEXT(gen);
  }

  solve_forces(A, P, cnt + (stamp & 1), s_hdr, s_lam, s_row , nc, lane, N, e, NR);

#pragma unroll
  for (int i = 0; i < 6; i++) integrate_joint(A, P, h, i, FLD(q, i), uB[i], N, e);
#pragma unroll
  for (int f = 0; f < 5; f++) {
#pragma unroll
    for (int l = 0; l < 4; l++) {
      float v = s_uf[(4 * f + l) * 64 + lane];
#pragma unroll
      for (int i = 0; i < 6; i++) v -= GPTR(A.fac_g)[((size_t)(6 * f + ((l * 6 + i) >> 2)) * N + e) * 4 + ((l * 6 + i) & 3)] * uB[i];
      integrate_joint(A, P, h, 6 + 4 * f + l, FLD(q, 6 + 4 * f + l), v, N, e);
    }
  }
  if (has_box && !C.box_fixed) integrate_box(A, h, vb, wb, N, e);
}

struct ApiPtrs {
  float* obs_buf; float* rew_buf; uint8_t* reset_buf; int64_t* episode_step_count; int64_t* episode_length;
  float* dof_state; float* root_state; float* rigid_body_states; float* contact_forces_all; float* full_dof_targets;
  const float* reset_samples;
  uint8_t* masks; const float* raw_targets;
  float* stats; int* counters;
  float* sink_obs; float* sink_rew; uint8_t* sink_done;
  float* sink_stats;
  float* actions_copy;
  int skip_obs_all;
  unsigned* probe;
  int stamp;
};

DI void store_pose(const Arena& A, int N, int e, int s, V3 p, Q4 q) {
  FLD(site_pose, 7 * s + 0) = p.x; FLD(site_pose, 7 * s + 1) = p.y; FLD(site_pose, 7 * s + 2) = p.z;
  FLD(site_pose, 7 * s + 3) = q.x; FLD(site_pose, 7 * s + 4) = q.y; FLD(site_pose, 7 * s + 5) = q.z;
  FLD(site_pose, 7 * s + 6) = q.w;
}

DI void publish_body(const Arena& A, const ApiPtrs& T, const DevParams* __restrict__ P, int full_bodies_req, int N, int NR, int root_wave = 5) {
  const int wv = __builtin_amdgcn_readfirstlane(wave_role(threadIdx.x >> 6));
  const int e = blockIdx.x * 64 + (threadIdx.x & 63);
  const bool w5 = wv == 5;
  const bool real = e < NR;
  const int full_bodies = full_bodies_req && real;
  const DexHandModel& M = P->model;
  const DexSimConfig& C = P->cfg;
  const int NB = DEXSIM_NUM_HAND_BODIES + (C.has_box ? 1 : 0);
  float* rbs = full_bodies ? T.rigid_body_states + (size_t)e * NB * 13 : nullptr;
  float* cfa = full_bodies ? T.contact_forces_all + (size_t)e * NB * 3 : nullptr;
  auto put_roots = [&]() {
    const int NA = 1 + (C.has_box ? 1 : 0);
    float* root = T.root_state + (size_t)e * NA * 13;
    root[0] = M.spawn_pos[0]; root[1] = M.spawn_pos[1]; root[2] = M.spawn_pos[2];
    root[3] = M.spawn_quat[0]; root[4] = M.spawn_quat[1]; root[5] = M.spawn_quat[2]; root[6] = M.spawn_quat[3];
#pragma unroll
    for (int i = 7; i < 13; i++) root[i] = 0.f;
    if (C.has_box) {
      float* b = root + 13;
      float bs[13];
#pragma unroll
      for (int i = 0; i < 3; i++) { bs[i] = FLD(box_pos, i); bs[7 + i] = FLD(box_lin, i); bs[10 + i] = FLD(box_ang, i); }
#pragma unroll
      for (int i = 0; i < 4; i++) bs[3 + i] = FLD(box_quat, i);
#pragma unroll
      for (int i = 0; i < 13; i++) b[i] = bs[i];
      if (full_bodies) {
        float* d = rbs + DEXSIM_NUM_HAND_BODIES * 13;
#pragma unroll
        for (int i = 0; i < 13; i++) d[i] = bs[i];
        float* c = cfa + DEXSIM_NUM_HAND_BODIES * 3;
#pragma unroll
        for (int i = 0; i < 3; i++) c[i] = FLD(cforce, 3 * DEXSIM_FSLOT_BOX + i);
      }
    }
  };
  if (wv > 5) {
    if (wv == root_wave && real) put_roots();
    return;
  }

  auto put_body = [&](int b, V3 o, Q4 q, V3 vo, V3 w) {
    const M3 R = q2mat(q);
    const V3 p = o + mul(R, v3p(M.body_p[b]));
    const Q4 bq = qmul(q, q4p(M.body_q[b]));
    const V3 v = vo + cross(w, p - o);
    float* d = rbs + b * 13;
    d[0] = p.x; d[1] = p.y; d[2] = p.z; d[3] = bq.x; d[4] = bq.y; d[5] = bq.z; d[6] = bq.w;
    d[7] = v.x; d[8] = v.y; d[9] = v.z; d[10] = w.x; d[11] = w.y; d[12] = w.z;
    const int s = M.body_fslot[b];
    float* c = cfa + b * 3;
    c[0] = s >= 0 ? FLD(cforce, 3 * s) : 0.f; c[1] = s >= 0 ? FLD(cforce, 3 * s + 1) : 0.f; c[2] = s >= 0 ? FLD(cforce, 3 * s + 2) : 0.f;
  };

  Q4 qc = q4p(M.spawn_quat);
  V3 oc = v3p(M.spawn_pos);
  V3 w = {0, 0, 0}, vo = {0, 0, 0};
  if (full_bodies && w5) put_body(0, oc, qc, vo, w);
  int j_first = 0;
  if (!full_bodies_req) {
    float qb[4], qdb[4];
#pragma unroll
    for (int j = 0; j < 4; j++) { qb[j] = FLD(q, j); qdb[j] = FLD(qd, j); }
    V3 t = {0, 0, 0};
#pragma unroll
    for (int j = 0; j < 3; j++) { t += qb[j] * v3p(P->base_A[j]); vo += qdb[j] * v3p(P->base_A[j]); }
    oc = v3p(P->base_Oc[3]) + t;
    const V3 ax = v3p(P->jc[3].axis);
    float s, c;
    sincos_joint(0.5f * qb[3], &s, &c);
    qc = qmul(q4p(P->base_Q3z), Q4{ax.x * s, ax.y * s, ax.z * s, c});
    w = qdb[3] * v3p(P->base_A[3]);
    if (real && w5) {
#pragma unroll
      for (int j = 0; j < 4; j++) { T.dof_state[((size_t)e * 26 + j) * 2] = qb[j]; T.dof_state[((size_t)e * 26 + j) * 2 + 1] = qdb[j]; }
    }
    j_first = 4;
  }
#pragma unroll
  for (int j = 0; j < 6; j++) {
    if (j < j_first) continue;
    const float qj = FLD(q, j), qdj = FLD(qd, j);
    M3 Rp = q2mat(qc);
    V3 on = oc + mul(Rp, v3p(P->jc[j].poff));
    Q4 qz = qmul(qc, q4p(P->jc[j].qoff));
    V3 ax = v3p(P->jc[j].axis);
    V3 aw = mul(q2mat(qz), ax);
    Q4 qn = qz;
    if (j < 3) on += qj * aw;
    else { float s, c; sincos_joint(0.5f * qj, &s, &c); qn = qmul(qz, Q4{ax.x * s, ax.y * s, ax.z * s, c}); }
    vo = vo + cross(w, on - oc);
    if (j < 3) vo += qdj * aw; else w += qdj * aw;
    qc = qn; oc = on;
    if (full_bodies && w5) put_body(j < 5 ? j + 1 : 6, oc, qc, vo, w);
    if (real && w5) { T.dof_state[((size_t)e * 26 + j) * 2] = qj; T.dof_state[((size_t)e * 26 + j) * 2 + 1] = qdj; }
  }
  const Q4 q5 = qc; const V3 o5 = oc, wb5 = w, v5 = vo;
  if (w5) {
    store_pose(A, N, e, 0, o5 + mul(q2mat(q5), v3p(M.site_p[0])), qmul(q5, q4p(M.site_q[0])));
    const V3 ps = o5 + mul(q2mat(q5), v3p(M.site_p[0]));
    const V3 v = v5 + cross(wb5, ps - o5);
    FLD(hand_vel, 0) = v.x; FLD(hand_vel, 1) = v.y; FLD(hand_vel, 2) = v.z;
    FLD(hand_vel, 3) = wb5.x; FLD(hand_vel, 4) = wb5.y; FLD(hand_vel, 5) = wb5.z;
  } else {
    const int f = wv;
    Q4 qf = q5; V3 of = o5, wf = wb5, vf = v5;
#pragma unroll
    for (int l = 0; l < 4; l++) {
      const int j = 6 + 4 * f + l;
      const float qj = FLD(q, j), qdj = FLD(qd, j);
      M3 Rp = q2mat(qf);
      V3 on = of + mul(Rp, v3p(P->jc[j].poff));
      Q4 qz = qmul(qf, q4p(P->jc[j].qoff));
      V3 ax = v3p(P->jc[j].axis);
      V3 aw = mul(q2mat(qz), ax);
      float s, c;
      sincos_joint(0.5f * qj, &s, &c);
      Q4 qn = qmul(qz, Q4{ax.x * s, ax.y * s, ax.z * s, c});
      vf = vf + cross(wf, on - of);
      wf += qdj * aw;
      qf = qn; of = on;
      if (full_bodies) put_body(7 + 6 * f + l, of, qf, vf, wf);
      if (real) { T.dof_state[((size_t)e * 26 + j) * 2] = qj; T.dof_state[((size_t)e * 26 + j) * 2 + 1] = qdj; }
    }
    const M3 R = q2mat(qf);
    store_pose(A, N, e, 1 + f, of + mul(R, v3p(M.site_p[1 + f])), qmul(qf, q4p(M.site_q[1 + f])));
    store_pose(A, N, e, 6 + f, of + mul(R, v3p(M.site_p[6 + f])), qmul(qf, q4p(M.site_q[6 + f])));
    if (full_bodies) { put_body(7 + 6 * f + 4, of, qf, vf, wf); put_body(7 + 6 * f + 5, of, qf, vf, wf); }
  }
  if (real && w5 && root_wave == 5) put_roots();
}

__global__ __launch_bounds__(384) void k_publish(Arena A, ApiPtrs T, const DevParams* __restrict__ P, const int* __restrict__ cnt,
                                                 int full_bodies_req, int N, int NR) {
  publish_body(A, T, P, full_bodies_req, N, NR);
}


#define XQ(b, q) ((f4*)(sh + FS_X * 64 + (((b) * 5 + (q)) * 64 + lane) * 4))
#define TQ(q) ((f4*)(sh + FS_T * 64 + ((q) * 64 + lane) * 4))

DI void post_pre_tasks(const Arena& A, const DevParams* __restrict__ P, const int* __restrict__ cnt, float* s_ob, int N);
#define POST_PRE_MASK 0x01

struct HandRows {
  f4 q[21];
  int kk;
  bool act;
};
DI void hand_fetch(HandRows& R, const Arena& A, int j, int nbg, int nh, int N, int e) {
  R.act = j < nh;
  R.kk = R.act ? nbg + j : 0;
  const unsigned off0 = ((unsigned)((R.act ? R.kk : DEXSIM_KMAX) * 21) * (unsigned)N + (unsigned)e) * 16u;
  const unsigned stride = R.act ? (unsigned)N * 16u : 0u;
  const char* base = (const char*)A.crowq;
#pragma unroll
  for (int q = 0; q < 21; q++) R.q[q] = *(const __attribute__((address_space(1))) f4*)(base + (off0 + (unsigned)q * stride));
}
struct TurnVel { f2 U01, U23, U45, V01, VW, W12; };
DI void turn_from_quads(TurnVel& v, f4 q0, f4 q1, f4 q2) { v.U01 = q0.xy; v.U23 = q0.zw; v.U45 = q1.xy; v.V01 = q1.zw; v.VW = q2.xy; v.W12 = q2.zw; }
DI void hand_update(const HandRows& R, TurnVel& v, f2& G01, f2& G23, f2 inv_mI_x, float nB, float nF, float mu, float cb, float (&lam)[3]) {
  const f4* q0 = R.q; const f4* q1 = R.q + 7; const f4* q2 = R.q + 14;
  f2 a0 = q0[0].xy * v.U01, a1 = q1[0].xy * v.U01, a2 = q2[0].xy * v.U01;
  a0 = q0[0].zw * v.U23 + a0; a1 = q1[0].zw * v.U23 + a1; a2 = q2[0].zw * v.U23 + a2;
  a0 = q0[1].xy * v.U45 + a0; a1 = q1[1].xy * v.U45 + a1; a2 = q2[1].xy * v.U45 + a2;
  a0 = q0[5].xy * v.V01 + a0; a1 = q1[5].xy * v.V01 + a1; a2 = q2[5].xy * v.V01 + a2;
  a0 = q0[5].zw * v.VW + a0; a1 = q1[5].zw * v.VW + a1; a2 = q2[5].zw * v.VW + a2;
  a0 = q0[6].xy * v.W12 + a0; a1 = q1[6].xy * v.W12 + a1; a2 = q2[6].xy * v.W12 + a2;
  a0 = q0[1].zw * G01 + a0; a1 = q1[1].zw * G01 + a1; a2 = q2[1].zw * G01 + a2;
  a0 = q0[2].xy * G23 + a0; a1 = q1[2].xy * G23 + a1; a2 = q2[2].xy * G23 + a2;
  float vr[3] = {a0.x + a0.y, a1.x + a1.y, a2.x + a2.y};
  const float A10 = R.q[6].w, A20 = R.q[13].w, A21 = R.q[20].w;
  const float nl0 = fmaxf(0.f, lam[0] - (vr[0] + cb) * R.q[6].z);
  const float dl0 = nl0 - lam[0], lim = mu * nl0;
  vr[1] += A10 * dl0; vr[2] += A20 * dl0;
  const float nl1 = clampf(lam[1] - vr[1] * R.q[13].z, -lim, lim);
  const float dl1 = nl1 - lam[1];
  vr[2] += A21 * dl1;
  const float nl2 = clampf(lam[2] - vr[2] * R.q[20].z, -lim, lim);
  const float dl2 = nl2 - lam[2];
  const float dl[3] = {dl0, dl1, dl2};
#pragma unroll
  for (int r = 0; r < 3; r++) {
    const f4 *q = R.q + 7 * r;
    const float dB = nB * dl[r], dF = nF * dl[r];
    v.U01 = q[2].zw * dB + v.U01; v.U23 = q[3].xy * dB + v.U23; v.U45 = q[3].zw * dB + v.U45;
    G01 = q[4].xy * dF + G01; G23 = q[4].zw * dF + G23;
    const f2 dmI = inv_mI_x * dl[r];
    v.V01 = q[5].xy * dmI.xx + v.V01; v.VW = q[5].zw * dmI + v.VW; v.W12 = q[6].xy * dmI.yy + v.W12;
  }
  lam[0] = nl0; lam[1] = nl1; lam[2] = nl2;
}
DI void hand_warm(const HandRows& R, TurnVel& v, f2& G01, f2& G23, f2 inv_mI, const float (&lam)[3]) {
#pragma unroll
  for (int r = 0; r < 3; r++) {
    const f4 *q = R.q + 7 * r;
    v.U01 = q[2].zw * lam[r] + v.U01; v.U23 = q[3].xy * lam[r] + v.U23; v.U45 = q[3].zw * lam[r] + v.U45;
    G01 = q[4].xy * lam[r] + G01; G23 = q[4].zw * lam[r] + G23;
    const f2 dmI = inv_mI * lam[r];
    v.V01 = q[5].xy * dmI.xx + v.V01; v.VW = q[5].zw * dmI + v.VW; v.W12 = q[6].xy * dmI.yy + v.W12;
  }
}

DI void build_rows_item(const DevParams* __restrict__ P, int N, int ol, int k, int eo, int split, int gen) {
  extern __shared__ __attribute__((aligned(16))) float sh[];
  build_contact_rows<true>(P->arena, P, nullptr, sh, ol, k, N, eo, split, gen);
}

#ifdef DEXSIM_PROFILE_PHASES
#define GP_STAMP(i) do { if (lane == 0) A.crow[(size_t)(stamp_base + wv * 8 + (i)) * N + e] = __int_as_float((int)(__builtin_amdgcn_s_memtime() - t_start)); } while (0)
#endif
#if defined(DEXSIM_PROFILE_PHASES) && !defined(DBG_PH2) && !defined(DBG_ROWS)
#define SWEEP_STAMP(i) do { if (it == 2 && lane == 0 && (wv == 0 || wv == 5) && stamp_base + 64 <= DEXSIM_KMAX * 3 * 28) A.crow[(size_t)(stamp_base + 56 + (i) + (wv == 5 ? 5 : 0)) * N + e] = __int_as_float((int)(__builtin_amdgcn_s_memtime() - t_start)); } while (0)
#else
#define SWEEP_STAMP(i) do {} while (0)
#endif
#ifndef DEXSIM_PROFILE_PHASES
#define GP_STAMP(i) do {} while (0)
#endif
#if defined(DEXSIM_PROFILE_PHASES) && defined(DBG_SWEEP)
#define SWEEP_STAMP2X(cond, i) do { if ((cond) && (threadIdx.x & 63) == 0 && stamp_base == 0) A.crow[(size_t)(400 + wv * 8 + (i)) * N + blockIdx.x * 64] = __int_as_float((int)(__builtin_amdgcn_s_memtime() - t_start)); } while (0)
#else
#define SWEEP_STAMP2X(cond, i) do {} while (0)
#endif
#define SWEEP_STAMP2(i) SWEEP_STAMP2X(it == 2, i)
DI void general_contact_phases(const DevParams* __restrict__ P, int N, int wv, int lane, int e,
                                                                  unsigned long long t_start, int stamp_base, unsigned* probe) {
  extern __shared__ __attribute__((aligned(16))) float sh[];
  const Arena& A = P->arena;
  const DexSimConfig& C = P->cfg;
  const bool has_box = C.has_box != 0;
  float* s_uf = sh + FS_UF * 64;
  float* s_lam = sh + FS_LAM * 64;
  float* s_hdr = sh + FS_HDR * 64;
  int nc = __float_as_int(SH(DL_NC));
  const int nbg = (nc >> 8) & 0xff; nc &= 0xff;
  const int nh = nc - nbg;
  int jmax = nh, kbg = nbg;
#pragma unroll
  for (int s = 32; s >= 1; s >>= 1) { jmax = max(jmax, __shfl_xor(jmax, s)); kbg = max(kbg, __shfl_xor(kbg, s)); }
  jmax = __builtin_amdgcn_readfirstlane(jmax); kbg = __builtin_amdgcn_readfirstlane(kbg);
  if (wv == 6) __builtin_amdgcn_s_setprio(0);
  const int n_items = __builtin_amdgcn_readfirstlane(__float_as_int(sh[FS_NITEM * 64]));
  if (wv < 6) {
#pragma unroll 1
    for (int base = wv * 64; base < n_items; base += 6 * 64) {
      const int item = base + lane;
      if (item < n_items) {
        const int ent = __float_as_int(sh[FS_CTAB * 64 + item]);
        const int ol = ent & 0xff, blk = ent >> 8;
        const int nc_o = __float_as_int(sh[DL_NC * 64 + ol]), nbg_o = (nc_o >> 8) & 0xff, nh_o = (nc_o & 0xff) - nbg_o;
        const int split_o = __float_as_int(sh[FS_SPLIT * 64 + ol]), rs_o = SPLIT_RS(split_o);
#pragma unroll 1
        for (int c = 0; c <= rs_o; c++) {
          const int j = (blk << rs_o) + c;
          if (j < nh_o) build_rows_item(P, N, ol, nbg_o + j, blockIdx.x * 64 + ol, split_o, __float_as_int(sh[FS_GEN * 64 + ol]));
        }
      }
    }
  }
  GP_STAMP(3);
  __syncthreads();
  unsigned long long pr_t4 = 0;
  if (probe && wv == 0) pr_t4 = __builtin_amdgcn_s_memtime();

  {
    const int iters = C.num_position_iterations;
    const bool bgstage = kbg > 0;
    const int split = __float_as_int(SH(FS_SPLIT)), gen = __float_as_int(SH(FS_GEN));
    float inv_m = 0.f, inv_I = 0.f;
    if (has_box) { inv_m = SH(FS_CMP_INVM); inv_I = SH(FS_CMP_INVM + 1); }
    const int nb_l = nh > 0 ? SPLIT_NB(split) : 0;
    int nbmax = nb_l;
#pragma unroll
    for (int s = 32; s >= 1; s >>= 1) nbmax = max(nbmax, __shfl_xor(nbmax, s));
    nbmax = __builtin_amdgcn_readfirstlane(nbmax);
    const float nXf = (float)SPLIT_NX(split), rX = 1.f / nXf;
    if (wv == 6) {
      const int cpack = __float_as_int(SH(FS_CPACK));
      BoxBlock bb;
      bb.load<false>(kbg, inv_m, inv_I, s_lam, s_hdr, sh + FS_CMP * 64, 0, 0, lane, nbg, true, nXf);
      f4 Tm0 = *TQ(2);
      {
        f2 d01 = {0.f, 0.f}, d23 = {0.f, 0.f}, d45 = {0.f, 0.f};
        if (bgstage) bb.warm(d01, d23, d45, f2{inv_m, inv_I});
        *XQ(12, 1) = f4{0.f, 0.f, d01.x, d01.y}; *XQ(12, 2) = f4{d23.x, d23.y, d45.x, d45.y};
      }
#pragma unroll 1
      for (int it = 0; it <= iters; it++) {
        SWEEP_STAMP2(1);
        __syncthreads();
        SWEEP_STAMP2(2);
        int b = 0;
        if (((nbmax + 3) & ~3) >= 8) {
          const f4 y0 = *XQ(0, 2), y1 = *XQ(1, 2), y2 = *XQ(2, 2), y3 = *XQ(3, 2), y4 = *XQ(4, 2), y5 = *XQ(5, 2), y6 = *XQ(6, 2), y7 = *XQ(7, 2);
          Tm0 += y0; Tm0 += y1; Tm0 += y2; Tm0 += y3; Tm0 += y4; Tm0 += y5; Tm0 += y6; Tm0 += y7;
          b = 8;
        }
#pragma unroll 1
        for (; b < ((nbmax + 3) & ~3); b += 4) {
          const f4 y0 = *XQ(b, 2), y1 = *XQ(b + 1, 2), y2 = *XQ(b + 2, 2), y3 = *XQ(b + 3, 2);
          Tm0 += y0; Tm0 += y1; Tm0 += y2; Tm0 += y3;
        }
        Tm0 += *XQ(12, 2);
        *TQ(2) = Tm0;
        SWEEP_STAMP2(3);
        __syncthreads();
        SWEEP_STAMP2(4);
        if (it == iters) break;
        SWEEP_STAMP2X(it == 1, 0);
        const f4 q1 = *TQ(1);
        const f2 o01 = q1.zw, o23 = Tm0.xy, o45 = Tm0.zw;
        f2 v01 = o01, v23 = o23, v45 = o45, d01 = {0.f, 0.f}, d23 = {0.f, 0.f}, d45 = {0.f, 0.f};
        if (bgstage) bb.sweep_delta(v01, v23, v45, d01, d23, d45, f2{inv_m, inv_I});
        *XQ(12, 1) = f4{0.f, 0.f, d01.x, d01.y}; *XQ(12, 2) = f4{d23.x, d23.y, d45.x, d45.y};
      }
      if (bgstage) { bb.store(s_lam, lane, nbg); cache_box_ground(A, s_lam, DEXSIM_WGEN_NEXT(gen), cpack, nbg, lane, N, e); }
      FLD(wgen, 0) = DEXSIM_WGEN_NEXT(gen);
      SH(FS_BOXV + 2) = Tm0.x; SH(FS_BOXV + 3) = Tm0.y; SH(FS_BOXV + 4) = Tm0.z; SH(FS_BOXV + 5) = Tm0.w;
    } else {
      const int rs_l = SPLIT_RS(split);
      int flo = 0, fcnt = 0, q4mask = 0;
      if (wv < 5) {
        int a = 0, cntf = 0;
#pragma unroll
        for (int w = 0; w < 5; w++) {
          const int word = NP_COUNT(__float_as_int(SH(FS_FLAG + w)));
          if (w < wv) a += word;
          if (w == wv) cntf = word;
        }
        cntf = max(0, min(cntf, nh - a));
        if (cntf > 0) {
          flo = a >> rs_l; fcnt = ((a + cntf - 1) >> rs_l) - flo + 1;
          if (rs_l && (a & 1)) q4mask = 1 << flo;
        }
      }
      int fcmax = fcnt;
#pragma unroll
      for (int s = 32; s >= 1; s >>= 1) fcmax = max(fcmax, __shfl_xor(fcmax, s));
      fcmax = __builtin_amdgcn_readfirstlane(fcmax);
      int it = 0;
      (void)it;
      const int nb4 = (nbmax + 3) & ~3;
      auto exchange = [&]() {
        SWEEP_STAMP2(1);
        __syncthreads();
        SWEEP_STAMP(2); SWEEP_STAMP2(2);
        if (wv < 5) {
          f4 t = *TQ(3 + wv);
#pragma unroll 1
          for (int i = 0; i < fcmax; i += 2) {
            const int b0 = min(flo + i, 11), b1 = min(flo + i + 1, 11);
            const f4 x0 = *XQ(b0, 3 + ((q4mask >> b0) & 1)), x1 = *XQ(b1, 3 + ((q4mask >> b1) & 1));
            if (i < fcnt) t += x0;
            if (i + 1 < fcnt) t += x1;
          }
          *TQ(3 + wv) = t;
        }
        if (wv == 5) {
          f4 t0 = *TQ(0);
          f4 t1 = *TQ(1);
          int b = 0;
          if (nb4 >= 8) {
            const f4 y0 = *XQ(0, 0), y1 = *XQ(1, 0), y2 = *XQ(2, 0), y3 = *XQ(3, 0), y4 = *XQ(4, 0), y5 = *XQ(5, 0), y6 = *XQ(6, 0), y7 = *XQ(7, 0);
            const f4 z0 = *XQ(0, 1), z1 = *XQ(1, 1), z2 = *XQ(2, 1), z3 = *XQ(3, 1), z4 = *XQ(4, 1), z5 = *XQ(5, 1), z6 = *XQ(6, 1), z7 = *XQ(7, 1);
            t0 += y0; t0 += y1; t0 += y2; t0 += y3; t0 += y4; t0 += y5; t0 += y6; t0 += y7;
            t1 += z0; t1 += z1; t1 += z2; t1 += z3; t1 += z4; t1 += z5; t1 += z6; t1 += z7;
            b = 8;
          }
#pragma unroll 1
          for (; b < nb4; b += 4) {
            const f4 y0 = *XQ(b, 0), y1 = *XQ(b + 1, 0), y2 = *XQ(b + 2, 0), y3 = *XQ(b + 3, 0);
            const f4 z0 = *XQ(b, 1), z1 = *XQ(b + 1, 1), z2 = *XQ(b + 2, 1), z3 = *XQ(b + 3, 1);
            t0 += y0; t0 += y1; t0 += y2; t0 += y3;
            t1 += z0; t1 += z1; t1 += z2; t1 += z3;
          }
          *TQ(0) = t0;
          t1 += *XQ(12, 1);
          *TQ(1) = t1;
        }
        SWEEP_STAMP(3); SWEEP_STAMP2(3);
        __syncthreads();
        SWEEP_STAMP2(4);
      };
      const bool fast = jmax <= 12 && n_items <= 6 * 64;
      {
      const int lane_phys = lane;
      if (fast) {
        const bool have = wv * 64 + lane_phys < n_items;
        const int ent = have ? __float_as_int(sh[FS_CTAB * 64 + wv * 64 + lane_phys]) : lane_phys;
        const int lane = ent & 0xff, blk = ent >> 8, e = blockIdx.x * 64 + lane;
        const int nc_o = __float_as_int(SH(DL_NC)), nbg_o = (nc_o >> 8) & 0xff;
        const int split_o = __float_as_int(SH(FS_SPLIT)), gen_o = __float_as_int(SH(FS_GEN));
        const float nBo = (float)SPLIT_NB(split_o), nXo = (float)SPLIT_NX(split_o), rBo = 1.f / nBo, rXo = 1.f / nXo;
        const f2 inv_mI = {has_box ? SH(FS_CMP_INVM) : 0.f, has_box ? SH(FS_CMP_INVM + 1) : 0.f}, inv_mI_x = inv_mI * nXo;
        HandRows R;
        hand_fetch(R, A, have ? blk : DEXSIM_KMAX, nbg_o, have ? (nc_o & 0xff) - nbg_o : 0, N, e);
        const int kk = R.kk;
        const int code = __float_as_int(s_hdr[(4 * kk) * 64 + lane]), fo = __float_as_int(s_hdr[(4 * kk + 1) * 64 + lane]);
        const bool hasF = R.act && fo >= 0;
        const int qi = 3 + (max(fo, 0) >> 2);
        const float nFo = hasF ? (float)((code >> 12) & 15) : 0.f, rFo = hasF ? 1.f / nFo : 0.f;
        const float mu = R.act ? s_hdr[(4 * kk + 2) * 64 + lane] : 0.f, cb = R.act ? s_hdr[(4 * kk + 3) * 64 + lane] : 0.f;
        float lam[3];
#pragma unroll
        for (int r = 0; r < 3; r++) { const float l = s_lam[(3 * kk + r) * 64 + lane]; lam[r] = R.act ? l : 0.f; }
        if (have) {
          const f4 z4 = {0.f, 0.f, 0.f, 0.f};
          TurnVel vl;
          turn_from_quads(vl, z4, z4, z4);
          f2 G01 = z4.xy, G23 = z4.xy;
          hand_warm(R, vl, G01, G23, inv_mI, lam);
          *XQ(blk, 0) = f4{vl.U01.x, vl.U01.y, vl.U23.x, vl.U23.y}; *XQ(blk, 1) = f4{vl.U45.x, vl.U45.y, vl.V01.x, vl.V01.y};
          *XQ(blk, 2) = f4{vl.VW.x, vl.VW.y, vl.W12.x, vl.W12.y}; *XQ(blk, 3) = f4{G01.x, G01.y, G23.x, G23.y};
        }
        exchange();
#pragma unroll 1
        for (it = 1; it <= iters; it++) {
          SWEEP_STAMP(0); SWEEP_STAMP2(0);
          if (have) {
            const f4 t0 = *TQ(0), t1 = *TQ(1), t2 = *TQ(2), tq = *TQ(qi);
            TurnVel vl;
            turn_from_quads(vl, t0, t1, t2);
            f2 G01 = tq.xy, G23 = tq.zw;
            hand_update(R, vl, G01, G23, inv_mI_x, nBo, nFo, mu, cb, lam);
            const f2 dU01 = (vl.U01 - t0.xy) * rBo, dU23 = (vl.U23 - t0.zw) * rBo, dU45 = (vl.U45 - t1.xy) * rBo;
            const f2 dV01 = (vl.V01 - t1.zw) * rXo, dVW = (vl.VW - t2.xy) * rXo, dW12 = (vl.W12 - t2.zw) * rXo;
            const f2 dG01 = (G01 - tq.xy) * rFo, dG23 = (G23 - tq.zw) * rFo;
            *XQ(blk, 0) = f4{dU01.x, dU01.y, dU23.x, dU23.y}; *XQ(blk, 1) = f4{dU45.x, dU45.y, dV01.x, dV01.y};
            *XQ(blk, 2) = f4{dVW.x, dVW.y, dW12.x, dW12.y}; *XQ(blk, 3) = f4{dG01.x, dG01.y, dG23.x, dG23.y};
          }
          SWEEP_STAMP(1);
          exchange();
          SWEEP_STAMP(4);
        }
        if (R.act) {
          s_lam[(3 * kk) * 64 + lane] = lam[0]; s_lam[(3 * kk + 1) * 64 + lane] = lam[1]; s_lam[(3 * kk + 2) * 64 + lane] = lam[2];
          st4_global(A.wlam + ((size_t)CODE_HKEY(code) * N + e) * 4, lam[0], lam[1], lam[2], __int_as_float(8 * DEXSIM_WGEN_NEXT(gen_o)));
        }
      } else {
        auto block_pass = [&](const bool warm) {
#pragma unroll 1
          for (int base = wv * 64; base < n_items; base += 6 * 64) {
            const bool have = base + lane_phys < n_items;
            const int ent = have ? __float_as_int(sh[FS_CTAB * 64 + base + lane_phys]) : lane_phys;
            const int lane = ent & 0xff, blk = ent >> 8, e = blockIdx.x * 64 + lane;
            const int nc_o = __float_as_int(SH(DL_NC)), nbg_o = (nc_o >> 8) & 0xff, nh_o = have ? (nc_o & 0xff) - nbg_o : 0;
            const int split_o = __float_as_int(SH(FS_SPLIT)), rs_o = SPLIT_RS(split_o);
            const float nBo = (float)SPLIT_NB(split_o), nXo = (float)SPLIT_NX(split_o);
            const f2 inv_mI = {has_box ? SH(FS_CMP_INVM) : 0.f, has_box ? SH(FS_CMP_INVM + 1) : 0.f}, inv_mI_x = inv_mI * nXo;
            const f4 z4 = {0.f, 0.f, 0.f, 0.f};
            TurnVel vl;
            if (warm) turn_from_quads(vl, z4, z4, z4); else turn_from_quads(vl, *TQ(0), *TQ(1), *TQ(2));
            int cur_fo = -1, cur_q = 3;
            float nFc = 1.f;
            f2 Gc01 = {0.f, 0.f}, Gc23 = {0.f, 0.f};
            auto flush = [&]() {
              if (cur_fo >= 0) {
                const f4 To = *TQ(3 + (cur_fo >> 2));
                const float rF = warm ? 1.f : 1.f / nFc;
                const f2 d01 = (Gc01 - (warm ? z4.xy : To.xy)) * rF, d23 = (Gc23 - (warm ? z4.zw : To.zw)) * rF;
                *XQ(blk, cur_q) = f4{d01.x, d01.y, d23.x, d23.y};
              }
            };
            HandRows R;
#pragma unroll 1
            for (int c = 0; c < (jmax > 12 ? 2 : 1); c++) {
              hand_fetch(R, A, c <= rs_o ? (blk << rs_o) + c : DEXSIM_KMAX, nbg_o, nh_o, N, e);
              const int kk = R.kk;
              const int code = __float_as_int(s_hdr[(4 * kk) * 64 + lane]), fo = __float_as_int(s_hdr[(4 * kk + 1) * 64 + lane]);
              const float mu = R.act ? s_hdr[(4 * kk + 2) * 64 + lane] : 0.f, cb = R.act ? s_hdr[(4 * kk + 3) * 64 + lane] : 0.f;
              const bool hasF = R.act && fo >= 0;
              const f4 Tq = *TQ(3 + (max(fo, 0) >> 2));
              if (hasF && fo != cur_fo) {
                flush();
                Gc01 = warm ? z4.xy : Tq.xy; Gc23 = warm ? z4.zw : Tq.zw;
                cur_fo = fo; cur_q = 3 + c; nFc = (float)((code >> 12) & 15);
              }
              float lam[3];
#pragma unroll
              for (int r = 0; r < 3; r++) { const float l = s_lam[(3 * kk + r) * 64 + lane]; lam[r] = R.act ? l : 0.f; }
              if (warm) hand_warm(R, vl, Gc01, Gc23, inv_mI, lam);
              else {
                hand_update(R, vl, Gc01, Gc23, inv_mI_x, nBo, hasF ? nFc : 0.f, mu, cb, lam);
                if (R.act) { s_lam[(3 * kk) * 64 + lane] = lam[0]; s_lam[(3 * kk + 1) * 64 + lane] = lam[1]; s_lam[(3 * kk + 2) * 64 + lane] = lam[2]; }
              }
            }
            flush();
            if (have) {
              const float sB = warm ? 1.f : 1.f / nBo, sX = warm ? 1.f : 1.f / nXo;
              TurnVel vo;
              if (warm) turn_from_quads(vo, z4, z4, z4); else turn_from_quads(vo, *TQ(0), *TQ(1), *TQ(2));
              const f2 dU01 = (vl.U01 - vo.U01) * sB, dU23 = (vl.U23 - vo.U23) * sB, dU45 = (vl.U45 - vo.U45) * sB;
              const f2 dV01 = (vl.V01 - vo.V01) * sX, dVW = (vl.VW - vo.VW) * sX, dW12 = (vl.W12 - vo.W12) * sX;
              *XQ(blk, 0) = f4{dU01.x, dU01.y, dU23.x, dU23.y}; *XQ(blk, 1) = f4{dU45.x, dU45.y, dV01.x, dV01.y};
              *XQ(blk, 2) = f4{dVW.x, dVW.y, dW12.x, dW12.y};
              if (cur_fo < 0) *XQ(blk, 3) = z4;
            }
          }
        };
#pragma unroll 1
        for (int it = 0; it <= iters; it++) {
          block_pass(it == 0);
          exchange();
        }
#pragma unroll 1
        for (int base = wv * 64; base < n_items; base += 6 * 64) {
          if (base + lane_phys < n_items) {
            const int ent = __float_as_int(sh[FS_CTAB * 64 + base + lane_phys]);
            const int lane = ent & 0xff, blk = ent >> 8, e = blockIdx.x * 64 + lane;
            const int nc_o = __float_as_int(SH(DL_NC)), nbg_o = (nc_o >> 8) & 0xff, nh_o = (nc_o & 0xff) - nbg_o;
            const int rs_o = SPLIT_RS(__float_as_int(SH(FS_SPLIT))), gen_o = __float_as_int(SH(FS_GEN));
            for (int c = 0; c <= rs_o; c++) {
              const int j = (blk << rs_o) + c;
              if (j < nh_o) {
                const int kk = nbg_o + j;
                const int code = __float_as_int(s_hdr[(4 * kk) * 64 + lane]);
                st4_global(A.wlam + ((size_t)CODE_HKEY(code) * N + e) * 4, s_lam[(3 * kk) * 64 + lane], s_lam[(3 * kk + 1) * 64 + lane],
                           s_lam[(3 * kk + 2) * 64 + lane], __int_as_float(8 * DEXSIM_WGEN_NEXT(gen_o)));
              }
            }
          }
        }
      }
      }
      if (wv < 5) {
        const f4 t = *TQ(3 + wv);
        s_uf[(4 * wv) * 64 + lane] = t.x; s_uf[(4 * wv + 1) * 64 + lane] = t.y; s_uf[(4 * wv + 2) * 64 + lane] = t.z;
        s_uf[(4 * wv + 3) * 64 + lane] = t.w;
      } else {
        const f4 t0 = *TQ(0), t1 = *TQ(1);
        SH(FS_UB) = t0.x; SH(FS_UB + 1) = t0.y; SH(FS_UB + 2) = t0.z; SH(FS_UB + 3) = t0.w; SH(FS_UB + 4) = t1.x; SH(FS_UB + 5) = t1.y;
        SH(FS_BOXV) = t1.z; SH(FS_BOXV + 1) = t1.w;
      }
    }
  }
  GP_STAMP(4);
  if (wv == 6) __builtin_amdgcn_s_setprio(2);
  __syncthreads();
  if (probe && wv == 0 && lane == 0) atomicAdd(probe + blockIdx.x * 4 + 3, (unsigned)(__builtin_amdgcn_s_memtime() - pr_t4));
}
#undef GP_STAMP
#undef SWEEP_STAMP

struct SubstepCarry { float ql[4], qdl[4], tg[4]; };
template <bool LAST, bool MS>
DI void substep_body(const Arena& A, const ApiPtrs& T, const DevParams* __restrict__ P, int* __restrict__ cnt, int N, int NR, float* sh,
                     int seq, int stamp_base, bool post_pre, bool count_contacts, SubstepCarry& carry, bool carry_in, bool carry_out) {
  constexpr int dlb = FS_ROW;
  int* const ccnt = count_contacts ? cnt + (T.stamp & 1) : nullptr;
  constexpr int last = LAST ? 1 : 0;
  const int wv = __builtin_amdgcn_readfirstlane(wave_role(threadIdx.x >> 6)), lane = threadIdx.x & 63;
  const int e = blockIdx.x * 64 + lane;
#ifdef DEXSIM_PROFILE_PHASES
  const unsigned long long t_start = __builtin_amdgcn_s_memtime();
  int stamp_i = 0;
#ifdef DBG_PH2
#define PH2_STAMP(i) do { if (lane == 0 && (wv == 1 || wv == 5)) A.crow[(size_t)(stamp_base + 56 + (i) + (wv == 5 ? 4 : 0)) * N + e] = __int_as_float((int)(__builtin_amdgcn_s_memtime() - t_start)); } while (0)
#else
#define PH2_STAMP(i) do {} while (0)
#endif
#define PHASE_STAMP() do { if (lane == 0) A.crow[(size_t)(stamp_base + wv * 8 + stamp_i) * N + e] = __int_as_float((int)(__builtin_amdgcn_s_memtime() - t_start)); stamp_i++; } while (0)
#else
#define PH2_STAMP(i) do {} while (0)
#define PHASE_STAMP() do {} while (0)
#endif
  {
  const DexHandModel& M = P->model;
  const DexSimConfig& C = P->cfg;
  const float h = P->h;
  const V3 grav = v3p(C.gravity);
  const bool has_box = C.has_box != 0;
  float* s_uf = sh + FS_UF * 64;
  float* s_lam = sh + FS_LAM * 64;
  float* s_hdr = sh + FS_HDR * 64;
  if (wv == 6) __builtin_amdgcn_s_setprio(2);
  BaseChain B;
  FingerIn fin;
  bool hand_free = false, sphere = false;
  V3 bpos_h = {0, 0, 0};
  M3 Rb_h = q2mat(Q4{0, 0, 0, 1});
  if (wv != 6) {
    if (carry_in) {
      if (has_box) bpos_h = {SH(FS_CARRY_BP), SH(FS_CARRY_BP + 1), SH(FS_CARRY_BP + 2)};
      base_chain<MS>(A, P, grav, N, e, B, false, sh + FS_CARRY_Q * 64, sh + FS_CARRY_QD * 64, lane);
      if (wv < 5) {
#pragma unroll
        for (int l = 0; l < 4; l++) { fin.ql[l] = carry.ql[l]; fin.qdl[l] = carry.qdl[l]; fin.tg[l] = carry.tg[l]; }
      }
    } else {
      if (has_box) bpos_h = {FLD(box_pos, 0), FLD(box_pos, 1), FLD(box_pos, 2)};
      base_chain<MS>(A, P, grav, N, e, B, false);
      if (wv < 5) finger_load(A, wv, N, e, fin);
    }
    sphere = hand_clear(P, B, bpos_h);
    if (!sphere && has_box) Rb_h = q2mat(Q4{FLD(box_quat, 0), FLD(box_quat, 1), FLD(box_quat, 2), FLD(box_quat, 3)});
    if (wv == 5) {
      bool pclear = sphere;
      if (!sphere) {
        const M3 R5 = q2mat(B.q5);
        bool clr = true;
#pragma unroll
        for (int cpl = 0; cpl < 3; cpl++)
          clr = clr && capsule_clear(B.o5 + mul(R5, v3p(M.cap_p0[cpl])), B.o5 + mul(R5, v3p(M.cap_p1[cpl])), M.cap_r[cpl], C, bpos_h, Rb_h);
        pclear = __all(clr);
      }
      if (lane == 0) sh[(FS_FLAG + 5) * 64] = __int_as_float((seq << 1) | (pclear ? 1 : 0));
    }
  }
  PHASE_STAMP();

  int nc = 0, nbg = 0;
  float Gkeep[24];
#pragma unroll
  for (int i = 0; i < 24; i++) Gkeep[i] = 0.f;
  V3 bpos = {0, 0, 0}; M3 Rb = q2mat(Q4{0, 0, 0, 1});
  float hb = 0.f, bmu = 0.f;
  if (wv < 5) {
    finger_dynamics<MS>(A, P, B, fin, sh, dlb, s_uf, lane, wv, N, e, seq, sphere, bpos_h, Rb_h, Gkeep);
  } else if (wv == 5) {
    const M3 R5 = q2mat(B.q5);
    Comp comp5;
    comp5.m = P->jc[5].mass;
    comp5.c = B.o5 + mul(R5, v3p(P->jc[5].com));
    comp5.I = rotate_inertia(R5, P->jc[5].inertia);
    V3 rc = comp5.c - B.o5;
    V3 ac = B.ao5 + cross(B.al5, rc) + cross(B.w5, cross(B.w5, rc));
    V3 f5 = comp5.m * ac;
    V3 n5 = mul(comp5.I, B.al5) + cross(B.w5, mul(comp5.I, B.w5)) + cross(rc, f5);
    comp_put(sh, lane, DL_PALM, comp5, B.o5);
    sh_put3(sh, lane, DL_PALM_WRENCH, f5); sh_put3(sh, lane, DL_PALM_WRENCH + 3, n5);
#pragma unroll
    for (int i = 0; i < 6; i++) SH(FS_TGTB + i) = FLD(targets, i);
#pragma unroll
    for (int i2 = 0; i2 < 3; i2++) {
      const V3 a0 = B.ab[2 * i2], o0 = B.ob[2 * i2], a1 = B.ab[2 * i2 + 1], o1 = B.ob[2 * i2 + 1];
      *(f4*)(sh + FS_BCH * 64 + ROWADDR(12 * i2, lane)) = f4{a0.x, a0.y, a0.z, o0.x};
      *(f4*)(sh + FS_BCH * 64 + ROWADDR(12 * i2 + 4, lane)) = f4{o0.y, o0.z, a1.x, a1.y};
      *(f4*)(sh + FS_BCH * 64 + ROWADDR(12 * i2 + 8, lane)) = f4{a1.z, o1.x, o1.y, o1.z};
    }
    schur_precompute(sh, dlb, lane, B, seq, cnt);
  } else if (wv == 6) {
    float bv[6] = {0, 0, 0, 0, 0, 0};
    const int gen = FLD(wgen, 0);
    f4 wq[4];
#pragma unroll
    for (int k = 0; k < 4; k++) wq[k] = *(const __attribute__((address_space(1))) f4*)(A.wlam + ((size_t)(80 + k) * N + e) * 4);
    int cpack = 0;
    SH(FS_GEN) = __int_as_float(gen);
    if (has_box) {
      bpos = {FLD(box_pos, 0), FLD(box_pos, 1), FLD(box_pos, 2)};
      Rb = q2mat(Q4{FLD(box_quat, 0), FLD(box_quat, 1), FLD(box_quat, 2), FLD(box_quat, 3)});
      hb = 0.5f * C.box_size;
      bmu = FLD(box_mu, 0);
      const float mu_bg = 0.5f * (bmu + C.ground_friction);
      const bool bfix = C.box_fixed != 0;
      const float inv_m = bfix ? 0.f : rcp_n(FLD(box_mass, 0)) , inv_I = P->box_inv_I_k * inv_m;
      SH(FS_CMP_INVM) = inv_m; SH(FS_CMP_INVM + 1) = inv_I;
      V3 dirz[3];
      dirz[0] = v3(0, 0, 1);
      tangent_basis(dirz[0], dirz[1], dirz[2]);
      int k_unused = 0;
#pragma unroll 1
      for (int i = 0; i < 8; i++) {
        V3 l = {(i & 1) ? hb : -hb, (i & 2) ? hb : -hb, (i & 4) ? hb : -hb};
        V3 p = mul(Rb, l) + bpos;
        if (!bfix && p.z < C.contact_offset && nc < 4) {
          const int k = nc++;
          cpack |= i << (3 * k);
          const float gap = p.z - C.rest_offset;
          const V3 rb = p - bpos;
          { float* rp = sh + (FS_CMP + 3 * k) * 64 + lane; rp[0] = rb.x; rp[64] = rb.y; rp[128] = rb.z; }
          const float cb = gap > 0.f ? div_n(gap, h) : -fminf(div_n(-gap * C.erp, h), C.max_depenetration_velocity);
          s_hdr[(4 * k) * 64 + lane] = __int_as_float(2); s_hdr[(4 * k + 1) * 64 + lane] = __int_as_float(-1);
          s_hdr[(4 * k + 2) * 64 + lane] = mu_bg; s_hdr[(4 * k + 3) * 64 + lane] = cb;
          if (LAST) {
            push_contact(A, N, e, k_unused, 2, 0, i, p, dirz[0], gap, mu_bg, -1, nullptr, DEXSIM_FSLOT_BOX << 21);
            FLD(chdr, 8 * k + 4) = __int_as_float(DEXSIM_FSLOT_BOX);
            FLD(chdr, 8 * k + 5) = 0.f; FLD(chdr, 8 * k + 6) = 0.f; FLD(chdr, 8 * k + 7) = 1.f;
          }
        }
      }
      if (!bfix) {
        bv[0] = FLD(box_lin, 0) + h * grav.x; bv[1] = FLD(box_lin, 1) + h * grav.y; bv[2] = FLD(box_lin, 2) + h * grav.z;
        bv[3] = FLD(box_ang, 0); bv[4] = FLD(box_ang, 1); bv[5] = FLD(box_ang, 2);
      }
    }
    nbg = nc;
#pragma unroll
    for (int i = 0; i < 6; i++) SH(FS_BOXV + i) = bv[i];
#pragma unroll
    for (int k = 0; k < 4; k++) {
      const bool warm = k < nc && __float_as_int(wq[k].w) == 8 * gen + ((cpack >> (3 * k)) & 7);
      s_lam[(3 * k) * 64 + lane] = warm ? wq[k].x : 0.f; s_lam[(3 * k + 1) * 64 + lane] = warm ? wq[k].y : 0.f;
      s_lam[(3 * k + 2) * 64 + lane] = warm ? wq[k].z : 0.f;
    }
    SH(FS_CPACK) = __int_as_float(cpack);
    BoxBlock sb;
    bool box_conv = false;
    f2 sv01 = {bv[0], bv[1]}, sv23 = {bv[2], bv[3]}, sv45 = {bv[4], bv[5]};
    const int it_split = (C.num_position_iterations * SPEC_SPLIT_NUM) >> 4;
    if (has_box) {
      int km = nc;
#pragma unroll
      for (int s = 32; s >= 1; s >>= 1) km = max(km, __shfl_xor(km, s));
      sb.load<false>(km, SH(FS_CMP_INVM), SH(FS_CMP_INVM + 1), s_lam, s_hdr, sh + FS_CMP * 64, 0, 0, lane, nc, true);
      sb.warm(sv01, sv23, sv45, f2{SH(FS_CMP_INVM), SH(FS_CMP_INVM + 1)});
#pragma unroll 1
      for (int it = 0; it < it_split && !box_conv; it++) {
        const int tokv = __float_as_int(*(volatile float*)(sh + (FS_FLAG + (lane < 6 ? lane : 0)) * 64));
        box_conv = !__any(sb.sweep(sv01, sv23, sv45));
        if (__any((tokv >> 1) == seq && !(tokv & 1))) break;
      }
    }
    {
      hand_free = true;
#pragma unroll 1
      for (int w = 0; w < 6; w++) {
        int tok;
        SPIN_GUARD_INIT();
        do {
          tok = __float_as_int(*(volatile float*)(sh + (FS_FLAG + w) * 64));
          if ((tok >> 1) != seq) { __builtin_amdgcn_s_sleep(2); SPIN_GUARD(cnt, 2, seq); }
        } while ((tok >> 1) != seq);
        hand_free = hand_free && (tok & 1) != 0;
      }
    }
    if (LAST && hand_free) FLD(ncontact, 0) = nc;
    SH(DL_NC) = __int_as_float(nc | (nbg << 8));
    PHASE_STAMP();
    __syncthreads();
    if (hand_free) {
      if (has_box) {
#pragma unroll 1
        for (int it = it_split; it < C.num_position_iterations && !box_conv; it++) box_conv = !__any(sb.sweep(sv01, sv23, sv45));
        SH(FS_BOXV) = sv01.x; SH(FS_BOXV + 1) = sv01.y; SH(FS_BOXV + 2) = sv23.x; SH(FS_BOXV + 3) = sv23.y;
        SH(FS_BOXV + 4) = sv45.x; SH(FS_BOXV + 5) = sv45.y;
        sb.store(s_lam, lane);
        cache_box_ground(A, s_lam, DEXSIM_WGEN_NEXT(gen), cpack, nc, lane, N, e);
      }
      FLD(wgen, 0) = DEXSIM_WGEN_NEXT(gen);
      if (last) solve_forces_box(A, P, ccnt, s_lam, nc, lane, N, e, NR);
    }
  }
  if (wv != 6) {
    PHASE_STAMP();
    __syncthreads();
  }
  int clear_mask = 0;
#pragma unroll
  for (int w = 0; w < 6; w++) clear_mask |= (__float_as_int(sh[(FS_FLAG + w) * 64]) & 1) << w;
  hand_free = clear_mask == 63;
  const bool early = hand_free;

  float uB[6] = {0, 0, 0, 0, 0, 0};
  if (early && wv >= 1 && wv <= 3) {
    schur_helper(sh, dlb, wv - 1, lane);
    asm volatile("" ::: "memory");
    if (lane == 0) *(volatile float*)(sh + (FS_FLAG + wv) * 64) = __int_as_float((seq << 1) | 1 | SCHUR_SPLIT_BIT);
  }
  if (wv == 0) {
    #ifdef DEXSIM_PROFILE_PHASES
    schur_base(A, P, B, sh, dlb, uB, lane, N, e, FS_TGTB, early, early ? seq : 0, t_start, stamp_base + 56, cnt);
#else
    schur_base(A, P, B, sh, dlb, uB, lane, N, e, FS_TGTB, early, early ? seq : 0, 0, 0, cnt);
#endif
    if (early) {
#pragma unroll
      for (int i = 0; i < 6; i++) SH(FS_UB + i) = uB[i];
    }
  }
  if (!hand_free) {
    int nloc = 0, tmask = 0;
    const int cw = wv == 6 ? 0 : (wv == 0 ? -1 : wv);
    if (cw >= 0 && !((clear_mask >> cw) & 1)) {
      V3 bp = {0, 0, 0}; M3 Rbx = q2mat(Q4{0, 0, 0, 1});
      float hbx = 0.f, bmux = 0.f;
      if (has_box) {
        bp = wv == 6 ? bpos : bpos_h;
        Rbx = q2mat(Q4{FLD(box_quat, 0), FLD(box_quat, 1), FLD(box_quat, 2), FLD(box_quat, 3)});
        hbx = 0.5f * C.box_size;
        bmux = FLD(box_mu, 0);
      }
      const float mu_hg = 0.5f * (M.hand_friction + C.ground_friction);
      const float mu_hb = 0.5f * (M.hand_friction + bmux);
      int caps[3], cinf[3];
      V3 E0[3], E1[3];
      float rr[3];
      if (cw < 5) {
#pragma unroll
        for (int c = 0; c < 3; c++) {
          const int l = 3 - c;
          caps[c] = 3 + 3 * cw + (l - 1);
          E0[c] = sh_get3(sh, lane, DL_CAPS(dlb, cw) + 6 * (l - 1)); E1[c] = sh_get3(sh, lane, DL_CAPS(dlb, cw) + 6 * (l - 1) + 3);
        }
      } else {
        const M3 R5 = q2mat(B.q5);
#pragma unroll
        for (int c = 0; c < 3; c++) {
          caps[c] = c;
          E0[c] = B.o5 + mul(R5, v3p(M.cap_p0[c])); E1[c] = B.o5 + mul(R5, v3p(M.cap_p1[c]));
        }
      }
#pragma unroll
      for (int c = 0; c < 3; c++) { rr[c] = M.cap_r[caps[c]]; cinf[c] = code_info(M, caps[c]); }
      collide_capsules3(A, N, e, nloc, C, caps, E0, E1, rr, has_box, bp, Rbx, hbx, mu_hb, mu_hg, cw, &tmask, cinf);
    }
    const int nreal = nloc;
    if (C.joint_limit_rows && cw >= 0 && cw < 5 && __any(nreal > 0)) {
      const bool touch = nreal > 0;
#pragma unroll
      for (int l = 0; l < 4; l++) {
        const int j = 6 + 4 * cw + l;
        const float qj = FLD(q, j);
        const float gl = qj - P->jc[j].lo, gu = P->jc[j].hi - qj;
        const int ci = ((cw + 1) << 16) | (l << 19);
        if (touch && gl < C.joint_limit_margin) push_contact(A, N, e, nloc, 3, l, 0, v3(0, 0, 0), v3(0, 0, 0), gl, 0.f, cw, nullptr, ci);
        if (touch && gu < C.joint_limit_margin) push_contact(A, N, e, nloc, 3, l, 1, v3(0, 0, 0), v3(0, 0, 0), gu, 0.f, cw, nullptr, ci);
      }
    }
    const int nbg0 = __float_as_int(SH(DL_NC)) & 0xff;
    PH2_STAMP(0);
    if (cw >= 0) SH(FS_FLAG + cw) = __int_as_float(NP_TAG | ((clear_mask >> cw) & 1) | (nloc << 1) | (tmask << 8));
    __syncthreads();
    PH2_STAMP(1);
    if (cw >= 0) {
      int off = nbg0;
      int tot = off;
#pragma unroll
      for (int w = 0; w < 6; w++) {
        const int c = NP_COUNT(__float_as_int(SH(FS_FLAG + w)));
        if (w < cw) off += c;
        tot += c;
      }
#pragma unroll 1
      for (int i0 = 0; __any(i0 < nloc); i0 += 4) {
        f4 g0[4], g1[4];
        float gc[4];
#pragma unroll
        for (int c = 0; c < 4; c++) {
          const bool ok = i0 + c < nloc && off + i0 + c < DEXSIM_KMAX;
          const int sc = cw * NP_STAGE + (ok ? i0 + c : 0);
          g0[c] = *FQ(cstage, 2 * sc); g1[c] = *FQ(cstage, 2 * sc + 1); gc[c] = FLD(cstage, CSTAGE_CODE0 + sc);
        }
#pragma unroll
        for (int c = 0; c < 4; c++) {
          const int kk = off + i0 + c;
          if (i0 + c < nloc && kk < DEXSIM_KMAX) {
            *FQ(cgeom, 2 * kk) = g0[c]; *FQ(cgeom, 2 * kk + 1) = g1[c];
            FLD(ccode, kk) = __float_as_int(gc[c]);
          }
        }
      }
      PH2_STAMP(2);
    }
    if (wv == 0) {
      int tot = nbg0;
#pragma unroll
      for (int w = 0; w < 6; w++) tot += NP_COUNT(__float_as_int(SH(FS_FLAG + w)));
      nc = min(tot, DEXSIM_KMAX);
      if (LAST) FLD(ncontact, 0) = nc;
      SH(DL_NC) = __int_as_float(nc | (nbg0 << 8));
      int cntw[6], hmask = 0, o = nbg0;
#pragma unroll
      for (int w = 0; w < 6; w++) {
        const int word = __float_as_int(SH(FS_FLAG + w));
        const int c = NP_COUNT(word), eff = max(0, min(c, DEXSIM_KMAX - o)), a = min(o - nbg0, 31);
        cntw[w] = eff;
        hmask |= (NP_TMASK(word) & ((1 << eff) - 1)) << a;
        o += c;
      }
      const int split = split_pack(nbg0, cntw, hmask);
      SH(FS_SPLIT) = __int_as_float(split);
      const int nh_l = nc - nbg0, nb_l = nh_l > 0 ? SPLIT_NB(split) : 0;
      float* ctab = sh + FS_CTAB * 64;
      int tot_items = 0;
#pragma unroll 1
      for (int b = 0; b < 12; b++) {
        const unsigned long long m = __ballot(b < nb_l);
        if (!m) break;
        if (b < nb_l) ctab[tot_items + __popcll(m & ((1ull << lane) - 1ull))] = __int_as_float(lane | (b << 8));
        tot_items += __popcll(m);
      }
      if (lane == 0) sh[FS_NITEM * 64] = __int_as_float(tot_items);
    }
  }
  PHASE_STAMP();
  __syncthreads();

  nc = __float_as_int(SH(DL_NC));
  nbg = (nc >> 8) & 0xff; nc &= 0xff;
  const int n_items_wg = early ? 0 : __builtin_amdgcn_readfirstlane(__float_as_int(sh[FS_NITEM * 64]));
  const bool gp = !early && n_items_wg > 0;
  if (!early && !gp) {
    if (wv == 0) {
#pragma unroll
      for (int i = 0; i < 6; i++) SH(FS_UB + i) = uB[i];
    } else if (wv == 6) {
      const int gen = __float_as_int(SH(FS_GEN)), cpack = __float_as_int(SH(FS_CPACK));
      if (has_box) {
        int km = nbg;
#pragma unroll
        for (int sf = 32; sf >= 1; sf >>= 1) km = max(km, __shfl_xor(km, sf));
        const f2 mI = {SH(FS_CMP_INVM), SH(FS_CMP_INVM + 1)};
        BoxBlock bb;
        f2 v01 = {SH(FS_BOXV), SH(FS_BOXV + 1)}, v23 = {SH(FS_BOXV + 2), SH(FS_BOXV + 3)}, v45 = {SH(FS_BOXV + 4), SH(FS_BOXV + 5)};
        bb.load<false>(km, mI.x, mI.y, s_lam, s_hdr, sh + FS_CMP * 64, 0, 0, lane, nbg, true);
        bb.warm(v01, v23, v45, mI);
#pragma unroll 1
        for (int it = 0; it < C.num_position_iterations; it++) if (!__any(bb.sweep(v01, v23, v45))) break;
        SH(FS_BOXV) = v01.x; SH(FS_BOXV + 1) = v01.y; SH(FS_BOXV + 2) = v23.x; SH(FS_BOXV + 3) = v23.y; SH(FS_BOXV + 4) = v45.x; SH(FS_BOXV + 5) = v45.y;
        bb.store(s_lam, lane);
        cache_box_ground(A, s_lam, DEXSIM_WGEN_NEXT(gen), cpack, nbg, lane, N, e);
      }
      FLD(wgen, 0) = DEXSIM_WGEN_NEXT(gen);
      if (last) solve_forces_box(A, P, ccnt, s_lam, nbg, lane, N, e, NR);
    }
    PHASE_STAMP(); PHASE_STAMP();
    __syncthreads();
  }
  if (gp) {
  {
    const f4 z4 = {0.f, 0.f, 0.f, 0.f};
#pragma unroll
    for (int q = 0; q < 10; q++) if (wv * 10 + q < 65) *XQ(0, wv * 10 + q) = z4;
    if (wv == 0) {
      *TQ(0) = f4{uB[0], uB[1], uB[2], uB[3]};
      float* t1 = (float*)TQ(1);
      t1[0] = uB[4]; t1[1] = uB[5];
    } else if (wv == 6) {
      float* t1 = (float*)TQ(1);
      t1[2] = SH(FS_BOXV); t1[3] = SH(FS_BOXV + 1);
      *TQ(2) = f4{SH(FS_BOXV + 2), SH(FS_BOXV + 3), SH(FS_BOXV + 4), SH(FS_BOXV + 5)};
    }
    if (wv < 5) *TQ(3 + wv) = f4{s_uf[(4 * wv) * 64 + lane], s_uf[(4 * wv + 1) * 64 + lane], s_uf[(4 * wv + 2) * 64 + lane], s_uf[(4 * wv + 3) * 64 + lane]};
  }
#pragma unroll
    for (int i = 0; i < 24; i++) Gkeep[i] = 0.f;
    unsigned long long pr_t3 = 0;
    if (T.probe && wv == 0) pr_t3 = __builtin_amdgcn_s_memtime();
#ifdef DEXSIM_PROFILE_PHASES
    general_contact_phases(P, N, wv, lane, e, t_start, stamp_base, T.probe);
    stamp_i += 2;
#else
    general_contact_phases(P, N, wv, lane, e, 0ull, 0, T.probe);
#endif
    if (T.probe && wv == 0 && lane == 0) {
      atomicAdd(T.probe + blockIdx.x * 4, (unsigned)(__builtin_amdgcn_s_memtime() - pr_t3));
      atomicAdd(T.probe + blockIdx.x * 4 + 2, 1u);
    }
  } else if (early) {
    PHASE_STAMP(); PHASE_STAMP();
  }

  if (last && gp) {
    if (wv < 5) forces_partial(A, P, s_hdr, s_lam, sh + (FS_FORCE + wv * DEXSIM_NFSLOT * 3) * 64, nc, wv, lane, N, e);
    __syncthreads();
  }
#pragma unroll
  for (int i = 0; i < 6; i++) uB[i] = SH(FS_UB + i);
  const bool store_q = LAST || !carry_out || C.joint_limit_rows != 0;
  if (wv < 5) {
    const int f = wv;
    float G[24];
    if (sphere) {
#pragma unroll
      for (int i = 0; i < 24; i++) G[i] = Gkeep[i];
    } else {
#pragma unroll
      for (int qd = 0; qd < 6; qd++) { const f4 g4 = *FQ(fac_g, 6 * f + qd); G[4 * qd] = g4.x; G[4 * qd + 1] = g4.y; G[4 * qd + 2] = g4.z; G[4 * qd + 3] = g4.w; }
    }
#pragma unroll
    for (int l = 0; l < 4; l++) {
      float v = s_uf[(4 * f + l) * 64 + lane];
#pragma unroll
      for (int i = 0; i < 6; i++) v -= G[l * 6 + i] * uB[i];
      float qn = 0.f, vn = 0.f;
      integrate_joint(A, P, h, 6 + 4 * f + l, fin.ql[l], v, N, e, &qn, &vn, store_q);
      if (carry_out) { carry.ql[l] = qn; carry.qdl[l] = vn; carry.tg[l] = fin.tg[l]; }
    }
  } else if (wv == 5) {
#pragma unroll
    for (int i = 0; i < 6; i++) {
      float qn = 0.f, vn = 0.f;
      integrate_joint(A, P, h, i, B.qb[i], uB[i], N, e, &qn, &vn, store_q);
      if (carry_out) { SH(FS_CARRY_Q + i) = qn; SH(FS_CARRY_QD + i) = vn; }
    }
  } else {
    if (has_box) {
      float vb[3], wb[3];
#pragma unroll
      for (int i = 0; i < 3; i++) { vb[i] = SH(FS_BOXV + i); wb[i] = SH(FS_BOXV + 3 + i); }
      if (carry_out) { SH(FS_CARRY_BP) = fmaf(h, vb[0], bpos.x); SH(FS_CARRY_BP + 1) = fmaf(h, vb[1], bpos.y); SH(FS_CARRY_BP + 2) = fmaf(h, vb[2], bpos.z); }
      if (!C.box_fixed) integrate_box(A, h, vb, wb, N, e);
    }
  }
  if (last && wv < 5 && gp) forces_reduce(A, ccnt, s_hdr, sh + FS_FORCE * 64, nc, lane, N, e, NR, wv, 5);
  if (last && wv == 5 && gp) contact_stats(ccnt, s_hdr, nc, lane, e, NR);
  PHASE_STAMP();
  }
  if (LAST) {
    __syncthreads();
    publish_body(A, T, P, 0, N, NR, 6);
    if (post_pre && wv == 6) post_pre_tasks(A, P, cnt, sh, N);
    PHASE_STAMP();
  }
#undef PHASE_STAMP
#undef PH2_STAMP
}

DI void reset_phase1(const Arena& A, int N, int e);
DI void finalize_stats(const ApiPtrs& T, const DevParams* __restrict__ P, int NR);
DI void post_block(const Arena& A, const ApiPtrs& T, const DevParams* __restrict__ P, int* __restrict__ cnt, float* s_ob,
                   int obs_only, int fold_reset, int N, int NR, int done_mask);
DI void actions_block(const Arena& A, const ApiPtrs& T, const DevParams* __restrict__ P, const float* __restrict__ act,
                      int zero_targets, int N, int NR);

enum {
  TAIL_RESET = 1,
  TAIL_POST = 2,
  TAIL_NOT_FINAL = 4,
};

template <bool GATED>
DI unsigned long long physics_prologue(const ApiPtrs& T, float* sh) {
  unsigned long long pr_k0 = 0;
  if (T.probe && threadIdx.x == 0) pr_k0 = __builtin_amdgcn_s_memtime();
  if (threadIdx.x < 6) sh[(FS_FLAG + threadIdx.x) * 64] = 0.f;
  if (threadIdx.x == 6) sh[FS_COMPCNT * 64] = 0.f;
  return pr_k0;
}
template <bool GATED>
DI void physics_epilogue(const ApiPtrs& T, const DevParams* __restrict__ P, int tail, unsigned long long pr_k0, int NR) {
  if (GATED && (tail & TAIL_RESET) && blockIdx.x == 0 && threadIdx.x == 0) finalize_stats(T, P, NR);
  if (!GATED && T.probe && threadIdx.x == 0) atomicAdd(T.probe + blockIdx.x * 4 + 1, (unsigned)(__builtin_amdgcn_s_memtime() - pr_k0));
}

template <bool GATED, bool MS>
__global__ __launch_bounds__(448) void k_physics4(Arena A, ApiPtrs T, const DevParams* __restrict__ P, int* __restrict__ cnt,
                                                  const float* __restrict__ act, int tail, int N, int NR) {
  extern __shared__ float sh[];
  const unsigned long long pr_k0 = physics_prologue<GATED>(T, sh);
  if (!GATED && act) actions_block(P->arena, T, P, act, 0, N, NR);
  __syncthreads();
  if (!GATED || cnt[CNT_ANY_RESET] == T.stamp) {
    SubstepCarry K;
    substep_body<false, MS>(P->arena, T, P, cnt, N, NR, sh, 1, 64, false, true, K, false, true);
    __syncthreads();
    substep_body<false, MS>(P->arena, T, P, cnt, N, NR, sh, 2, 128, false, true, K, true, true);
    __syncthreads();
    substep_body<false, MS>(P->arena, T, P, cnt, N, NR, sh, 3, 192, false, true, K, true, true);
    __syncthreads();
    substep_body<true, MS>(P->arena, T, P, cnt, N, NR, sh, 4, 256, !GATED && (tail & TAIL_POST), !GATED && !(tail & TAIL_NOT_FINAL), K, true, false);
    if (!GATED && (tail & TAIL_POST)) {
      __syncthreads();
      post_block(P->arena, T, P, cnt, sh, 0, 1, N, NR, POST_PRE_MASK);
    }
    if (GATED && (tail & TAIL_RESET)) {
      const int e = blockIdx.x * 64 + (threadIdx.x & 63);
      if (threadIdx.x < 64 && e < NR && A.reset_flag[e] != 0) reset_phase1(A, N, e);
    }
  }
  physics_epilogue<GATED>(T, P, tail, pr_k0, NR);
}

template <bool GATED, bool MS>
__global__ __launch_bounds__(448) void k_physics1(Arena A, ApiPtrs T, const DevParams* __restrict__ P, int* __restrict__ cnt,
                                                  const float* __restrict__ act, int tail, int N, int NR) {
  extern __shared__ float sh[];
  const unsigned long long pr_k0 = physics_prologue<GATED>(T, sh);
  if (!GATED && act) actions_block(P->arena, T, P, act, 0, N, NR);
  __syncthreads();
  if (!GATED || cnt[CNT_ANY_RESET] == T.stamp) {
    SubstepCarry K;
    substep_body<true, MS>(P->arena, T, P, cnt, N, NR, sh, 1, 0, !GATED && (tail & TAIL_POST), !GATED && !(tail & TAIL_NOT_FINAL), K, false, false);
    if (!GATED && (tail & TAIL_POST)) {
      __syncthreads();
      post_block(P->arena, T, P, cnt, sh, 0, 1, N, NR, POST_PRE_MASK);
    }
    if (GATED && (tail & TAIL_RESET)) {
      const int e = blockIdx.x * 64 + (threadIdx.x & 63);
      if (threadIdx.x < 64 && e < NR && A.reset_flag[e] != 0) reset_phase1(A, N, e);
    }
  }
  physics_epilogue<GATED>(T, P, tail, pr_k0, NR);
}
```

Before: 68.40 million.

## Address shared-memory words through per-window base registers within ds immediate reach

```diff
diff --git a/__graft_entry__.py b/__graft_entry__.py
--- a/__graft_entry__.py
+++ b/__graft_entry__.py
@@ -11,6 +11,8 @@
     path = build_lib(force=True)
     from dexrobot_isaac_amd.build import build_debug_spin
     build_debug_spin(force=True)
+    from dexrobot_isaac_amd.build import build_lds_flat
+    build_lds_flat(force=True)
     from oracle.oracle import build as build_oracle
     build_oracle(force=True)
     import dexrobot_isaac_amd
diff --git a/dexrobot_isaac_amd/build.py b/dexrobot_isaac_amd/build.py
--- a/dexrobot_isaac_amd/build.py
+++ b/dexrobot_isaac_amd/build.py
@@ -5,7 +5,7 @@
 HERE = os.path.dirname(os.path.abspath(__file__))
 CSRC = os.path.join(HERE, "csrc")
 LIB = os.path.join(HERE, "libdexsim.so")
-SOURCES = ["dexsim.hip", "dexsim_device.h", "dexsim_physics.hip.inc", "dexsim_l2.hip.inc", "dexsim_state.hip.inc",
+SOURCES = ["dexsim.hip", "dexsim_device.h", "dexsim_lds.h", "dexsim_physics.hip.inc", "dexsim_l2.hip.inc", "dexsim_state.hip.inc",
            "dexsim_chain.hip.inc", "dexsim_render.hip.inc", "dexsim_kindyn.hip.inc", "dexsim_ik.hip.inc", "dexsim_proximity.hip.inc",
            "dexsim_invdyn.hip.inc"]
 
@@ -27,6 +27,13 @@
     return build_lib(force=force, defs=(f"-DDEXSIM_DEBUG_SPIN={int(bound)}",), out=DEBUG_SPIN_LIB)
 
 
+LDS_FLAT_LIB = os.path.join(HERE, "libdexsim_ldsflat.so")
+
+
+def build_lds_flat(force=False):
+    return build_lib(force=force, defs=("-DDEXSIM_LDS_FLAT=1",), out=LDS_FLAT_LIB)
+
+
 def build_lib(force=False, verbose=False, defs=(), out=None):
     lib = out or LIB
     if not force and not _stale(lib):
diff --git a/dexrobot_isaac_amd/csrc/dexsim_lds.h b/dexrobot_isaac_amd/csrc/dexsim_lds.h
--- /dev/null
+++ b/dexrobot_isaac_amd/csrc/dexsim_lds.h
@@ -0,0 +1,45 @@
+#pragma once
+#ifndef DEXSIM_LDS_FLAT
+#define DEXSIM_LDS_FLAT 0
+#endif
+DI int lds_hide(int x) {
+#if !DEXSIM_LDS_FLAT
+  asm("" : "+v"(x));
+#endif
+  return x;
+}
+#define LDS_WIN 256
+#define LDS_WIN_F (LDS_WIN * 64)
+#define LDS_NWIN 3
+struct LdsWin {
+  float* sh;
+  int b0, b1, b2;
+  DI LdsWin(float* s, int lane, bool hide = true)
+      : sh(s), b0(lane), b1(hide ? lds_hide(LDS_WIN_F + lane) : LDS_WIN_F + lane), b2(hide ? lds_hide(2 * LDS_WIN_F + lane) : 2 * LDS_WIN_F + lane) {}
+  DI int base(int w) const { return w < LDS_WIN ? b0 : (w < 2 * LDS_WIN ? b1 : b2); }
+  DI float& operator()(int w) const { return sh[base(w) + (w & (LDS_WIN - 1)) * 64]; }
+  DI float& at(int cw, int dyn) const { return sh[base(cw) + ((cw & (LDS_WIN - 1)) + dyn) * 64]; }
+};
+struct LdsQuadWin {
+  float* sh;
+  int b0, b1, b2;
+  DI LdsQuadWin(float* s, int lane, bool hide = true)
+      : sh(s), b0(lane * 4), b1(hide ? lds_hide(LDS_WIN_F + lane * 4) : LDS_WIN_F + lane * 4),
+        b2(hide ? lds_hide(2 * LDS_WIN_F + lane * 4) : 2 * LDS_WIN_F + lane * 4) {}
+  DI int base(int f) const { return f < LDS_WIN_F ? b0 : (f < 2 * LDS_WIN_F ? b1 : b2); }
+  DI f4& quad(int w, int qd) const { const int f = w * 64 + qd * 256; return *(f4*)(sh + base(f) + (f & (LDS_WIN_F - 1))); }
+  DI f4& flat(int w, int qd) const { return *(f4*)(sh + (w * 64 + qd * 256) + b0); }
+  DI f4& qat(int w, int cq, int dyn) const { const int f = w * 64 + cq * 256; return *(f4*)(sh + base(f) + (f & (LDS_WIN_F - 1)) + dyn * 256); }
+};
+constexpr bool lds_word_ok(int w0, int n) {
+  for (int w = w0; w < w0 + n; w++) if ((w & (LDS_WIN - 1)) * 256 > 65280 || w >= LDS_NWIN * LDS_WIN) return false;
+  return true;
+}
+constexpr bool lds_quad_ok(int w0, int nq) {
+  for (int q = 0; q < nq; q++) {
+    const int f = w0 * 64 + q * 256;
+    if ((f & (LDS_WIN_F - 1)) * 4 > 65520 || f >= LDS_NWIN * LDS_WIN_F) return false;
+  }
+  return true;
+}
+constexpr bool lds_one_window(int w0, int words) { return (w0 * 64) / LDS_WIN_F == ((w0 + words) * 64 - 1) / LDS_WIN_F; }
diff --git a/dexrobot_isaac_amd/csrc/dexsim_physics.hip.inc b/dexrobot_isaac_amd/csrc/dexsim_physics.hip.inc
--- a/dexrobot_isaac_amd/csrc/dexsim_physics.hip.inc
+++ b/dexrobot_isaac_amd/csrc/dexsim_physics.hip.inc
@@ -198,12 +198,14 @@
   return {2.f * fmaf(q.x, q.z, mulr(q.y, q.w)), 2.f * fmaf(q.y, q.z, -mulr(q.x, q.w)), fmaf(fmaf(q.y, q.y, mulr(q.x, q.x)), -2.f, 1.f)};
 }
 
+#include "dexsim_lds.h"
+
 template <bool MS>
 DI void base_chain(const Arena& A, const DevParams* __restrict__ P, V3 grav, int N, int e, BaseChain& B, bool write_jframe,
-                   const float* s_q = nullptr, const float* s_qd = nullptr, int lane = 0) {
+                   const LdsWin* Wc = nullptr, int cq = 0, int cqd = 0) {
 #pragma unroll
   for (int j = 0; j < 6; j++) {
-    if (s_q) { B.qb[j] = s_q[j * 64 + lane]; B.qdb[j] = s_qd[j * 64 + lane]; }
+    if (Wc) { B.qb[j] = (*Wc)(cq + j); B.qdb[j] = (*Wc)(cqd + j); }
     else { B.qb[j] = FLD(q, j); B.qdb[j] = FLD(qd, j); }
   }
   V3 t = {0, 0, 0};
@@ -285,19 +287,18 @@
   return clear;
 }
 
-#define SH(i) sh[(i) * 64 + lane]
-DI void sh_put3(float* sh, int lane, int i, V3 v) { SH(i) = v.x; SH(i + 1) = v.y; SH(i + 2) = v.z; }
-DI void comp_put(float* sh, int lane, int w, const Comp& c, V3 o5) {
+#define SH(i) W(i)
+DI void sh_put3(const LdsWin& W, int i, V3 v, int dyn = 0) { W.at(i, dyn) = v.x; W.at(i + 1, dyn) = v.y; W.at(i + 2, dyn) = v.z; }
+DI void comp_put(const LdsWin& W, int w, const Comp& c, V3 o5, int dyn = 0) {
   const V3 d = c.c - o5;
   const S6 J = c.I + pa(c.m, d);
-  sh[(w) * 64 + lane] = c.m; sh_put3(sh, lane, w + 1, d);
-  sh[(w + 4) * 64 + lane] = J.xx; sh[(w + 5) * 64 + lane] = J.yy; sh[(w + 6) * 64 + lane] = J.zz;
-  sh[(w + 7) * 64 + lane] = J.xy; sh[(w + 8) * 64 + lane] = J.xz; sh[(w + 9) * 64 + lane] = J.yz;
-}
-DI V3 sh_get3(const float* sh, int lane, int i) { return {SH(i), SH(i + 1), SH(i + 2)}; }
-DI void bch_get2(const float* s_bch, int lane, int i2, V3& a0, V3& o0, V3& a1, V3& o1) {
-  const f4 q0 = *(const f4*)(s_bch + ROWADDR(12 * i2, lane)), q1 = *(const f4*)(s_bch + ROWADDR(12 * i2 + 4, lane)),
-           q2 = *(const f4*)(s_bch + ROWADDR(12 * i2 + 8, lane));
+  W.at(w, dyn) = c.m; sh_put3(W, w + 1, d, dyn);
+  W.at(w + 4, dyn) = J.xx; W.at(w + 5, dyn) = J.yy; W.at(w + 6, dyn) = J.zz;
+  W.at(w + 7, dyn) = J.xy; W.at(w + 8, dyn) = J.xz; W.at(w + 9, dyn) = J.yz;
+}
+DI V3 sh_get3(const LdsWin& W, int i, int dyn = 0) { return {W.at(i, dyn), W.at(i + 1, dyn), W.at(i + 2, dyn)}; }
+DI void bch_get2(const LdsQuadWin& Q, int w_bch, int i2, V3& a0, V3& o0, V3& a1, V3& o1) {
+  const f4 q0 = Q.flat(w_bch, 3 * i2), q1 = Q.flat(w_bch, 3 * i2 + 1), q2 = Q.flat(w_bch, 3 * i2 + 2);
   a0 = {q0.x, q0.y, q0.z}; o0 = {q0.w, q1.x, q1.y}; a1 = {q1.z, q1.w, q2.x}; o1 = {q2.y, q2.z, q2.w};
 }
 
@@ -402,6 +403,14 @@
 static_assert(lds_map_conflict() < 0, "LDS map: a region leaves the LDS or shares a word with a region live in a common phase "
                                       "(the note shows 1000 x the first word of one + the first word of the other)");
 static_assert(DL_CAPS(0, 5) == DL_HANDOFF, "the per-finger hand-off is DL_HANDOFF words");
+static_assert(LDS_NWIN * LDS_WIN >= FS_WORDS && (LDS_NWIN - 1) * LDS_WIN < FS_WORDS, "the LDS windows cover FS_WORDS, none of them is empty");
+static_assert(lds_word_ok(0, FS_WORDS), "a word access (ds_read_b32 / ds_read2st64_b32: offset1 <= 255 x 256 bytes) leaves the reach of its window's base");
+static_assert(lds_quad_ok(DL_SINV, 9) && lds_quad_ok(FS_BCH, 9) && lds_quad_ok(FS_X, 13 * 5) && lds_quad_ok(FS_T, 8),
+              "a quad access lies more than 65 520 bytes above its window's base or leaves the LDS");
+static_assert(lds_one_window(DL_SINV, 36) && lds_one_window(FS_BCH, 36) && lds_one_window(FS_T, 8 * 4),
+              "a ROWADDR / quad block crosses a window boundary (FS_X does, quad by quad: LdsQuadWin picks every quad's window)");
+static_assert(FS_HDR + 4 * DEXSIM_KMAX <= LDS_WIN && FS_UF >= 0,
+              "s_uf / s_lam / s_hdr (runtime entry index, flat from the lane base) must lie in window 0: their constant part is the immediate");
 #define SOLVE_LDS_WORDS(kstage) (60 + DEXSIM_KMAX * 3 + DEXSIM_KMAX * 4 + (kstage) * 3 * CROW_W)
 static_assert((DL_SPLIT + 1) * 64 * sizeof(float) <= FS_LDS_BYTES, "k_dynamics' LDS does not fit into the CU's");
 static_assert(SOLVE_LDS_WORDS(4) * 64 * sizeof(float) <= FS_LDS_BYTES, "k_solve's LDS does not fit into the CU's");
@@ -419,6 +428,7 @@
   const DexHandModel& M = P->model;
   const float h = P->h;
   const int j0 = 6 + 4 * f;
+  const LdsWin W(sh, lane);
   Q4 qf = B.q5; V3 of = B.o5; V3 wf = B.w5, alf = B.al5, aof = B.ao5;
   V3 a[4], o[4], cl[4], fl[4], nl[4];
   S6 Iw[4];
@@ -451,8 +461,8 @@
     if (l >= 1 && !(tok_seq > 0 && sphere_clear)) {
       const int cap = 3 + 3 * f + (l - 1);
       const V3 c0 = on + mul(R, v3p(M.cap_p0[cap])), c1 = on + mul(R, v3p(M.cap_p1[cap]));
-      sh_put3(sh, lane, DL_CAPS(dlb, f) + 6 * (l - 1), c0);
-      sh_put3(sh, lane, DL_CAPS(dlb, f) + 6 * (l - 1) + 3, c1);
+      sh_put3(W, DL_CAPS(dlb, 0) + 6 * (l - 1), c0, 18 * f);
+      sh_put3(W, DL_CAPS(dlb, 0) + 6 * (l - 1) + 3, c1, 18 * f);
       if (tok_seq > 0) clr = clr && capsule_clear(c0, c1, M.cap_r[cap], P->cfg, bpos, Rb);
     }
     a[l] = aw; o[l] = on; qf = qn; of = on;
@@ -474,8 +484,8 @@
     bias[l] = dot(a[l], nl[l]);
     if (l > 0) { fl[l - 1] += fl[l]; nl[l - 1] += nl[l] + cross(o[l] - o[l - 1], fl[l]); }
   }
-  sh_put3(sh, lane, DL_WRENCH(dlb, f), fl[0]);
-  sh_put3(sh, lane, DL_WRENCH(dlb, f) + 3, nl[0] + cross(o[0] - B.o5, fl[0]));
+  sh_put3(W, DL_WRENCH(dlb, 0), fl[0], 43 * f);
+  sh_put3(W, DL_WRENCH(dlb, 0) + 3, nl[0] + cross(o[0] - B.o5, fl[0]), 43 * f);
   float Fm[16], Cm[24];
   Comp cc;
 #pragma unroll
@@ -500,7 +510,7 @@
         Cm[i * 4 + l] = i < 3 ? dot(B.ab[i], Pm) : dot(B.ab[i], Lm + cross(cc.c - B.ob[i], Pm));
     }
   }
-  comp_put(sh, lane, DL_COMP(dlb, f), cc, B.o5);
+  comp_put(W, DL_COMP(dlb, 0), cc, B.o5, 43 * f);
   if (tok_seq > 0) {
     asm volatile("" ::: "memory");
     if (lane == 0) __hip_atomic_fetch_add((int*)(sh + FS_COMPCNT * 64), 1, __ATOMIC_RELAXED, __HIP_MEMORY_SCOPE_WORKGROUP);
@@ -541,8 +551,8 @@
       f2 s2 = {0.f, 0.f};
 #pragma unroll
       for (int l = 0; l < 4; l++) s2 = G2[l * 3 + kp] * Cm[i * 4 + l] + s2;
-      SH(DL_SSUB(dlb, f) + i * (i + 1) / 2 + 2 * kp) = s2.x;
-      if (2 * kp + 1 <= i) SH(DL_SSUB(dlb, f) + i * (i + 1) / 2 + 2 * kp + 1) = s2.y;
+      W.at(DL_SSUB(dlb, 0) + i * (i + 1) / 2 + 2 * kp, 43 * f) = s2.x;
+      if (2 * kp + 1 <= i) W.at(DL_SSUB(dlb, 0) + i * (i + 1) / 2 + 2 * kp + 1, 43 * f) = s2.y;
     }
   if (!fclear) {
     *FQ(fac_finv, 3 * f) = f4{Fm[0], Fm[4], Fm[5], Fm[8]};
@@ -554,7 +564,7 @@
     f2 s2 = {0.f, 0.f};
 #pragma unroll
     for (int l = 0; l < 4; l++) s2 = G2[l * 3 + ip] * tau[l] + s2;
-    SH(DL_GSUM(dlb, f) + 2 * ip) = s2.x; SH(DL_GSUM(dlb, f) + 2 * ip + 1) = s2.y;
+    W.at(DL_GSUM(dlb, 0) + 2 * ip, 43 * f) = s2.x; W.at(DL_GSUM(dlb, 0) + 2 * ip + 1, 43 * f) = s2.y;
   }
 #pragma unroll
   for (int l = 0; l < 4; l++) {
@@ -579,15 +589,15 @@
 #define SPIN_GUARD_INIT() do {} while (0)
 #define SPIN_GUARD(cntp, site, seq) do {} while (0)
 #endif
-DI Comp schur_comp(const float* sh, const int dlb, int lane, V3 o5) {
+DI Comp schur_comp(const LdsWin& W, const int dlb, V3 o5) {
   float M = SH(DL_PALM);
-  V3 sd = M * sh_get3(sh, lane, DL_PALM + 1);
+  V3 sd = M * sh_get3(W, DL_PALM + 1);
   S6 J = {SH(DL_PALM + 4), SH(DL_PALM + 5), SH(DL_PALM + 6), SH(DL_PALM + 7), SH(DL_PALM + 8), SH(DL_PALM + 9)};
 #pragma unroll
   for (int f = 0; f < 5; f++) {
     const float mf = SH(DL_COMP(dlb, f));
     M += mf;
-    sd += mf * sh_get3(sh, lane, DL_COMP(dlb, f) + 1);
+    sd += mf * sh_get3(W, DL_COMP(dlb, f) + 1);
     J = J + S6{SH(DL_COMP(dlb, f) + 4), SH(DL_COMP(dlb, f) + 5), SH(DL_COMP(dlb, f) + 6), SH(DL_COMP(dlb, f) + 7), SH(DL_COMP(dlb, f) + 8), SH(DL_COMP(dlb, f) + 9)};
   }
   const float inv = M > 0.f ? 1.f / M : 0.f;
@@ -599,7 +609,7 @@
   return c;
 }
 template <int i, int k0 = 0, int k1 = i>
-DI void schur_row(float* sh, const int dlb, int lane) {
+DI void schur_row(const LdsWin& W, const int dlb) {
   float r[k1 - k0 + 1];
 #pragma unroll
   for (int k = k0; k <= k1; k++) {
@@ -618,7 +628,8 @@
     while (*(volatile int*)(sh + FS_COMPCNT * 64) < 5 * seq) { __builtin_amdgcn_s_sleep(2); SPIN_GUARD(dbg_cnt, 4, seq); }
   }
   asm volatile("" ::: "memory");
-  const Comp comp5 = schur_comp(sh, dlb, lane, B.o5);
+  const LdsWin W(sh, lane);
+  const Comp comp5 = schur_comp(W, dlb, B.o5);
   int idx = 0;
 #pragma unroll
   for (int i = 0; i < 6; i++) {
@@ -631,11 +642,11 @@
       idx++;
     }
   }
-  V3 ff = sh_get3(sh, lane, DL_PALM_WRENCH), nn = sh_get3(sh, lane, DL_PALM_WRENCH + 3);
+  V3 ff = sh_get3(W, DL_PALM_WRENCH), nn = sh_get3(W, DL_PALM_WRENCH + 3);
 #pragma unroll
   for (int f = 0; f < 5; f++) {
-    ff += sh_get3(sh, lane, DL_WRENCH(dlb, f));
-    nn += sh_get3(sh, lane, DL_WRENCH(dlb, f) + 3);
+    ff += sh_get3(W, DL_WRENCH(dlb, f));
+    nn += sh_get3(W, DL_WRENCH(dlb, f) + 3);
   }
   SH(FS_SPRE_BIAS + 5) = dot(B.ab[5], nn);
 #pragma unroll
@@ -645,6 +656,7 @@
   }
 }
 DI void schur_helper(float* sh, const int dlb, int job, int lane) {
+  const LdsWin W(sh, lane);
   if (job == 1) {
     float gsum[6] = {0, 0, 0, 0, 0, 0};
 #pragma unroll
@@ -653,10 +665,10 @@
       for (int i = 0; i < 6; i++) gsum[i] += SH(DL_GSUM(dlb, f) + i);
 #pragma unroll
     for (int i = 0; i < 6; i++) SH(DL_SCHUR_GSUM + i) = gsum[i];
-    schur_row<0>(sh, dlb, lane); schur_row<1>(sh, dlb, lane); schur_row<2>(sh, dlb, lane);
+    schur_row<0>(W, dlb); schur_row<1>(W, dlb); schur_row<2>(W, dlb);
   } else if (job == 0) {
-    schur_row<3>(sh, dlb, lane); schur_row<5, 4, 5>(sh, dlb, lane);
-  } else schur_row<4>(sh, dlb, lane);
+    schur_row<3>(W, dlb); schur_row<5, 4, 5>(W, dlb);
+  } else schur_row<4>(W, dlb);
 }
 
 DI void schur_base(const Arena& A, const DevParams* __restrict__ P, const BaseChain& B, float* sh, const int dlb, float* uB_out,
@@ -668,18 +680,19 @@
 #define SCHUR_STAMP(i) do {} while (0)
 #endif
   const float h = P->h;
+  const LdsWin W(sh, lane);
   SCHUR_STAMP(0);
   Comp comp5;
-  V3 f5 = sh_get3(sh, lane, DL_PALM_WRENCH), n5 = sh_get3(sh, lane, DL_PALM_WRENCH + 3);
+  V3 f5 = sh_get3(W, DL_PALM_WRENCH), n5 = sh_get3(W, DL_PALM_WRENCH + 3);
   float Ssub[21], gsum[6] = {0, 0, 0, 0, 0, 0};
 #pragma unroll
   for (int i = 0; i < 21; i++) Ssub[i] = 0.f;
-  if (split_seq == 0) comp5 = schur_comp(sh, dlb, lane, B.o5);
+  if (split_seq == 0) comp5 = schur_comp(W, dlb, B.o5);
   if (split_seq == 0) {
 #pragma unroll
     for (int f = 0; f < 5; f++) {
-      f5 += sh_get3(sh, lane, DL_WRENCH(dlb, f));
-      n5 += sh_get3(sh, lane, DL_WRENCH(dlb, f) + 3);
+      f5 += sh_get3(W, DL_WRENCH(dlb, f));
+      n5 += sh_get3(W, DL_WRENCH(dlb, f) + 3);
 #pragma unroll
       for (int i = 0; i < 21; i++) Ssub[i] += SH(DL_SSUB(dlb, f) + i);
 #pragma unroll
@@ -688,7 +701,7 @@
   }
   SCHUR_STAMP(1);
   float S[36];
-  if (split_seq > 0) schur_row<5, 0, 3>(sh, dlb, lane);
+  if (split_seq > 0) schur_row<5, 0, 3>(W, dlb);
   else {
     int idx = 0;
 #pragma unroll
@@ -826,11 +839,12 @@
   float Dq[3] = {0.f, 0.f, 0.f};
   float A10 = 0.f, A20 = 0.f, A21 = 0.f;
   if (type != 2) {
+    const LdsQuadWin Q(sh, lane);
 #pragma unroll
     for (int i2 = 0; i2 < 3; i2++) {
       V3 aa[2], oo[2];
       if (FUSED) {
-        bch_get2(sh + FS_BCH * 64, lane, i2, aa[0], oo[0], aa[1], oo[1]);
+        bch_get2(Q, FS_BCH, i2, aa[0], oo[0], aa[1], oo[1]);
       } else { aa[0] = B->ab[2 * i2]; oo[0] = B->ob[2 * i2]; aa[1] = B->ab[2 * i2 + 1]; oo[1] = B->ob[2 * i2 + 1]; }
 #pragma unroll
       for (int h = 0; h < 2; h++) {
@@ -970,6 +984,7 @@
   constexpr int dlb = DL_PERSIST;
   const int wv = threadIdx.x >> 6, lane = threadIdx.x & 63;
   const int e = blockIdx.x * 64 + lane;
+  const LdsWin W(sh, lane);
   const DexHandModel& M = P->model;
   const DexSimConfig& C = P->cfg;
   const V3 grav = v3p(C.gravity);
@@ -994,8 +1009,8 @@
     V3 ac = B.ao5 + cross(B.al5, rc) + cross(B.w5, cross(B.w5, rc));
     V3 f5 = comp5.m * ac;
     V3 n5 = mul(comp5.I, B.al5) + cross(B.w5, mul(comp5.I, B.w5)) + cross(rc, f5);
-    comp_put(sh, lane, DL_PALM, comp5, B.o5);
-    sh_put3(sh, lane, DL_PALM_WRENCH, f5); sh_put3(sh, lane, DL_PALM_WRENCH + 3, n5);
+    comp_put(W, DL_PALM, comp5, B.o5);
+    sh_put3(W, DL_PALM_WRENCH, f5); sh_put3(W, DL_PALM_WRENCH + 3, n5);
     const float h = P->h;
     if (has_box) {
       bpos = {FLD(box_pos, 0), FLD(box_pos, 1), FLD(box_pos, 2)};
@@ -1033,7 +1048,7 @@
 #pragma unroll 1
       for (int l = 3; l >= 1; l--) {
         const int cap = 3 + 3 * f + (l - 1);
-        const V3 e0 = sh_get3(sh, lane, DL_CAPS(dlb, f) + 6 * (l - 1)), e1 = sh_get3(sh, lane, DL_CAPS(dlb, f) + 6 * (l - 1) + 3);
+        const V3 e0 = sh_get3(W, DL_CAPS(dlb, 0), 18 * f + 6 * (l - 1)), e1 = sh_get3(W, DL_CAPS(dlb, 0) + 3, 18 * f + 6 * (l - 1));
         collide_capsule(A, N, e, nc, C, cap, e0, e1, M.cap_r[cap], has_box, bpos, Rb, hb, mu_hb, mu_hg, -1, &tmask, code_info(M, cap));
       }
       if (f == 0) cntw[0] = nc - n0; else if (f == 1) cntw[1] = nc - n0; else if (f == 2) cntw[2] = nc - n0; else if (f == 3) cntw[3] = nc - n0; else cntw[4] = nc - n0;
@@ -1096,7 +1111,7 @@
           y = rows[ROWADDR((k * 3) * rw + ro + 3, lane)]; x = -rows[ROWADDR((k * 3) * rw + ro + 4, lane)];
           z = rows[ROWADDR((k * 3 + 1) * rw + ro + 3, lane)];
         } else {
-          x = rows[(3 * k) * 64 + lane]; y = rows[(3 * k + 1) * 64 + lane]; z = rows[(3 * k + 2) * 64 + lane];
+          x = rows[(3 * k) * 64]; y = rows[(3 * k + 1) * 64]; z = rows[(3 * k + 2) * 64];
         }
       }
       rx[k] = use ? x : 0.f; ry[k] = use ? y : 0.f; rz[k] = use ? z : 0.f;
@@ -1642,8 +1657,10 @@
 }
 
 
-#define XQ(b, q) ((f4*)(sh + FS_X * 64 + (((b) * 5 + (q)) * 64 + lane) * 4))
-#define TQ(q) ((f4*)(sh + FS_T * 64 + ((q) * 64 + lane) * 4))
+#define XQ(b, q) (&Q.quad(FS_X, (b) * 5 + (q)))
+#define XQB(b, cq) (&Q.qat(FS_X, (cq), (b) * 5))
+#define TQ(q) (&Q.quad(FS_T, (q)))
+#define TQD(cq, d) (&Q.qat(FS_T, (cq), (d)))
 
 DI void post_pre_tasks(const Arena& A, const DevParams* __restrict__ P, const int* __restrict__ cnt, float* s_ob, int N);
 #define POST_PRE_MASK 0x01
@@ -1738,7 +1755,7 @@
   float* s_uf = sh + FS_UF * 64;
   float* s_lam = sh + FS_LAM * 64;
   float* s_hdr = sh + FS_HDR * 64;
-  int nc = __float_as_int(SH(DL_NC));
+  int nc = __float_as_int(sh[DL_NC * 64 + lane]);
   const int nbg = (nc >> 8) & 0xff; nc &= 0xff;
   const int nh = nc - nbg;
   int jmax = nh, kbg = nbg;
@@ -1754,12 +1771,13 @@
       if (item < n_items) {
         const int ent = __float_as_int(sh[FS_CTAB * 64 + item]);
         const int ol = ent & 0xff, blk = ent >> 8;
-        const int nc_o = __float_as_int(sh[DL_NC * 64 + ol]), nbg_o = (nc_o >> 8) & 0xff, nh_o = (nc_o & 0xff) - nbg_o;
-        const int split_o = __float_as_int(sh[FS_SPLIT * 64 + ol]), rs_o = SPLIT_RS(split_o);
+        const LdsWin Wo(sh, ol);
+        const int nc_o = __float_as_int(Wo(DL_NC)), nbg_o = (nc_o >> 8) & 0xff, nh_o = (nc_o & 0xff) - nbg_o;
+        const int split_o = __float_as_int(Wo(FS_SPLIT)), rs_o = SPLIT_RS(split_o), gen_o = __float_as_int(Wo(FS_GEN));
 #pragma unroll 1
         for (int c = 0; c <= rs_o; c++) {
           const int j = (blk << rs_o) + c;
-          if (j < nh_o) build_rows_item(P, N, ol, nbg_o + j, blockIdx.x * 64 + ol, split_o, __float_as_int(sh[FS_GEN * 64 + ol]));
+          if (j < nh_o) build_rows_item(P, N, ol, nbg_o + j, blockIdx.x * 64 + ol, split_o, gen_o);
         }
       }
     }
@@ -1772,6 +1790,8 @@
   {
     const int iters = C.num_position_iterations;
     const bool bgstage = kbg > 0;
+    const LdsWin W(sh, lane);
+    const LdsQuadWin Q(sh, lane);
     const int split = __float_as_int(SH(FS_SPLIT)), gen = __float_as_int(SH(FS_GEN));
     float inv_m = 0.f, inv_I = 0.f;
     if (has_box) { inv_m = SH(FS_CMP_INVM); inv_I = SH(FS_CMP_INVM + 1); }
@@ -1784,7 +1804,7 @@
     if (wv == 6) {
       const int cpack = __float_as_int(SH(FS_CPACK));
       BoxBlock bb;
-      bb.load<false>(kbg, inv_m, inv_I, s_lam, s_hdr, sh + FS_CMP * 64, 0, 0, lane, nbg, true, nXf);
+      bb.load<false>(kbg, inv_m, inv_I, s_lam, s_hdr, &W(FS_CMP), 0, 0, lane, nbg, true, nXf);
       f4 Tm0 = *TQ(2);
       {
         f2 d01 = {0.f, 0.f}, d23 = {0.f, 0.f}, d45 = {0.f, 0.f};
@@ -1804,7 +1824,7 @@
         }
 #pragma unroll 1
         for (; b < ((nbmax + 3) & ~3); b += 4) {
-          const f4 y0 = *XQ(b, 2), y1 = *XQ(b + 1, 2), y2 = *XQ(b + 2, 2), y3 = *XQ(b + 3, 2);
+          const f4 y0 = *XQB(b, 2), y1 = *XQB(b, 7), y2 = *XQB(b, 12), y3 = *XQB(b, 17);
           Tm0 += y0; Tm0 += y1; Tm0 += y2; Tm0 += y3;
         }
         Tm0 += *XQ(12, 2);
@@ -1852,15 +1872,15 @@
         __syncthreads();
         SWEEP_STAMP(2); SWEEP_STAMP2(2);
         if (wv < 5) {
-          f4 t = *TQ(3 + wv);
+          f4 t = *TQD(3, wv);
 #pragma unroll 1
           for (int i = 0; i < fcmax; i += 2) {
             const int b0 = min(flo + i, 11), b1 = min(flo + i + 1, 11);
-            const f4 x0 = *XQ(b0, 3 + ((q4mask >> b0) & 1)), x1 = *XQ(b1, 3 + ((q4mask >> b1) & 1));
+            const f4 x0 = Q.qat(FS_X, 3, b0 * 5 + ((q4mask >> b0) & 1)), x1 = Q.qat(FS_X, 3, b1 * 5 + ((q4mask >> b1) & 1));
             if (i < fcnt) t += x0;
             if (i + 1 < fcnt) t += x1;
           }
-          *TQ(3 + wv) = t;
+          *TQD(3, wv) = t;
         }
         if (wv == 5) {
           f4 t0 = *TQ(0);
@@ -1875,8 +1895,8 @@
           }
 #pragma unroll 1
           for (; b < nb4; b += 4) {
-            const f4 y0 = *XQ(b, 0), y1 = *XQ(b + 1, 0), y2 = *XQ(b + 2, 0), y3 = *XQ(b + 3, 0);
-            const f4 z0 = *XQ(b, 1), z1 = *XQ(b + 1, 1), z2 = *XQ(b + 2, 1), z3 = *XQ(b + 3, 1);
+            const f4 y0 = *XQB(b, 0), y1 = *XQB(b, 5), y2 = *XQB(b, 10), y3 = *XQB(b, 15);
+            const f4 z0 = *XQB(b, 1), z1 = *XQB(b, 6), z2 = *XQB(b, 11), z3 = *XQB(b, 16);
             t0 += y0; t0 += y1; t0 += y2; t0 += y3;
             t1 += z0; t1 += z1; t1 += z2; t1 += z3;
           }
@@ -1895,6 +1915,8 @@
         const bool have = wv * 64 + lane_phys < n_items;
         const int ent = have ? __float_as_int(sh[FS_CTAB * 64 + wv * 64 + lane_phys]) : lane_phys;
         const int lane = ent & 0xff, blk = ent >> 8, e = blockIdx.x * 64 + lane;
+        const LdsWin W(sh, lane);
+        const LdsQuadWin Q(sh, lane);
         const int nc_o = __float_as_int(SH(DL_NC)), nbg_o = (nc_o >> 8) & 0xff;
         const int split_o = __float_as_int(SH(FS_SPLIT)), gen_o = __float_as_int(SH(FS_GEN));
         const float nBo = (float)SPLIT_NB(split_o), nXo = (float)SPLIT_NX(split_o), rBo = 1.f / nBo, rXo = 1.f / nXo;
@@ -1916,15 +1938,15 @@
           turn_from_quads(vl, z4, z4, z4);
           f2 G01 = z4.xy, G23 = z4.xy;
           hand_warm(R, vl, G01, G23, inv_mI, lam);
-          *XQ(blk, 0) = f4{vl.U01.x, vl.U01.y, vl.U23.x, vl.U23.y}; *XQ(blk, 1) = f4{vl.U45.x, vl.U45.y, vl.V01.x, vl.V01.y};
-          *XQ(blk, 2) = f4{vl.VW.x, vl.VW.y, vl.W12.x, vl.W12.y}; *XQ(blk, 3) = f4{G01.x, G01.y, G23.x, G23.y};
+          *XQB(blk, 0) = f4{vl.U01.x, vl.U01.y, vl.U23.x, vl.U23.y}; *XQB(blk, 1) = f4{vl.U45.x, vl.U45.y, vl.V01.x, vl.V01.y};
+          *XQB(blk, 2) = f4{vl.VW.x, vl.VW.y, vl.W12.x, vl.W12.y}; *XQB(blk, 3) = f4{G01.x, G01.y, G23.x, G23.y};
         }
         exchange();
 #pragma unroll 1
         for (it = 1; it <= iters; it++) {
           SWEEP_STAMP(0); SWEEP_STAMP2(0);
           if (have) {
-            const f4 t0 = *TQ(0), t1 = *TQ(1), t2 = *TQ(2), tq = *TQ(qi);
+            const f4 t0 = *TQ(0), t1 = *TQ(1), t2 = *TQ(2), tq = *TQD(0, qi);
             TurnVel vl;
             turn_from_quads(vl, t0, t1, t2);
             f2 G01 = tq.xy, G23 = tq.zw;
@@ -1932,8 +1954,8 @@
             const f2 dU01 = (vl.U01 - t0.xy) * rBo, dU23 = (vl.U23 - t0.zw) * rBo, dU45 = (vl.U45 - t1.xy) * rBo;
             const f2 dV01 = (vl.V01 - t1.zw) * rXo, dVW = (vl.VW - t2.xy) * rXo, dW12 = (vl.W12 - t2.zw) * rXo;
             const f2 dG01 = (G01 - tq.xy) * rFo, dG23 = (G23 - tq.zw) * rFo;
-            *XQ(blk, 0) = f4{dU01.x, dU01.y, dU23.x, dU23.y}; *XQ(blk, 1) = f4{dU45.x, dU45.y, dV01.x, dV01.y};
-            *XQ(blk, 2) = f4{dVW.x, dVW.y, dW12.x, dW12.y}; *XQ(blk, 3) = f4{dG01.x, dG01.y, dG23.x, dG23.y};
+            *XQB(blk, 0) = f4{dU01.x, dU01.y, dU23.x, dU23.y}; *XQB(blk, 1) = f4{dU45.x, dU45.y, dV01.x, dV01.y};
+            *XQB(blk, 2) = f4{dVW.x, dVW.y, dW12.x, dW12.y}; *XQB(blk, 3) = f4{dG01.x, dG01.y, dG23.x, dG23.y};
           }
           SWEEP_STAMP(1);
           exchange();
@@ -1950,6 +1972,8 @@
             const bool have = base + lane_phys < n_items;
             const int ent = have ? __float_as_int(sh[FS_CTAB * 64 + base + lane_phys]) : lane_phys;
             const int lane = ent & 0xff, blk = ent >> 8, e = blockIdx.x * 64 + lane;
+            const LdsWin W(sh, lane);
+            const LdsQuadWin Q(sh, lane);
             const int nc_o = __float_as_int(SH(DL_NC)), nbg_o = (nc_o >> 8) & 0xff, nh_o = have ? (nc_o & 0xff) - nbg_o : 0;
             const int split_o = __float_as_int(SH(FS_SPLIT)), rs_o = SPLIT_RS(split_o);
             const float nBo = (float)SPLIT_NB(split_o), nXo = (float)SPLIT_NX(split_o);
@@ -1962,10 +1986,10 @@
             f2 Gc01 = {0.f, 0.f}, Gc23 = {0.f, 0.f};
             auto flush = [&]() {
               if (cur_fo >= 0) {
-                const f4 To = *TQ(3 + (cur_fo >> 2));
+                const f4 To = *TQD(3, cur_fo >> 2);
                 const float rF = warm ? 1.f : 1.f / nFc;
                 const f2 d01 = (Gc01 - (warm ? z4.xy : To.xy)) * rF, d23 = (Gc23 - (warm ? z4.zw : To.zw)) * rF;
-                *XQ(blk, cur_q) = f4{d01.x, d01.y, d23.x, d23.y};
+                Q.qat(FS_X, 3, blk * 5 + (cur_q - 3)) = f4{d01.x, d01.y, d23.x, d23.y};
               }
             };
             HandRows R;
@@ -1976,7 +2000,7 @@
               const int code = __float_as_int(s_hdr[(4 * kk) * 64 + lane]), fo = __float_as_int(s_hdr[(4 * kk + 1) * 64 + lane]);
               const float mu = R.act ? s_hdr[(4 * kk + 2) * 64 + lane] : 0.f, cb = R.act ? s_hdr[(4 * kk + 3) * 64 + lane] : 0.f;
               const bool hasF = R.act && fo >= 0;
-              const f4 Tq = *TQ(3 + (max(fo, 0) >> 2));
+              const f4 Tq = *TQD(3, max(fo, 0) >> 2);
               if (hasF && fo != cur_fo) {
                 flush();
                 Gc01 = warm ? z4.xy : Tq.xy; Gc23 = warm ? z4.zw : Tq.zw;
@@ -1998,9 +2022,9 @@
               if (warm) turn_from_quads(vo, z4, z4, z4); else turn_from_quads(vo, *TQ(0), *TQ(1), *TQ(2));
               const f2 dU01 = (vl.U01 - vo.U01) * sB, dU23 = (vl.U23 - vo.U23) * sB, dU45 = (vl.U45 - vo.U45) * sB;
               const f2 dV01 = (vl.V01 - vo.V01) * sX, dVW = (vl.VW - vo.VW) * sX, dW12 = (vl.W12 - vo.W12) * sX;
-              *XQ(blk, 0) = f4{dU01.x, dU01.y, dU23.x, dU23.y}; *XQ(blk, 1) = f4{dU45.x, dU45.y, dV01.x, dV01.y};
-              *XQ(blk, 2) = f4{dVW.x, dVW.y, dW12.x, dW12.y};
-              if (cur_fo < 0) *XQ(blk, 3) = z4;
+              *XQB(blk, 0) = f4{dU01.x, dU01.y, dU23.x, dU23.y}; *XQB(blk, 1) = f4{dU45.x, dU45.y, dV01.x, dV01.y};
+              *XQB(blk, 2) = f4{dVW.x, dVW.y, dW12.x, dW12.y};
+              if (cur_fo < 0) *XQB(blk, 3) = z4;
             }
           }
         };
@@ -2014,6 +2038,8 @@
           if (base + lane_phys < n_items) {
             const int ent = __float_as_int(sh[FS_CTAB * 64 + base + lane_phys]);
             const int lane = ent & 0xff, blk = ent >> 8, e = blockIdx.x * 64 + lane;
+            const LdsWin W(sh, lane);
+            const LdsQuadWin Q(sh, lane);
             const int nc_o = __float_as_int(SH(DL_NC)), nbg_o = (nc_o >> 8) & 0xff, nh_o = (nc_o & 0xff) - nbg_o;
             const int rs_o = SPLIT_RS(__float_as_int(SH(FS_SPLIT))), gen_o = __float_as_int(SH(FS_GEN));
             for (int c = 0; c <= rs_o; c++) {
@@ -2030,7 +2056,7 @@
       }
       }
       if (wv < 5) {
-        const f4 t = *TQ(3 + wv);
+        const f4 t = *TQD(3, wv);
         s_uf[(4 * wv) * 64 + lane] = t.x; s_uf[(4 * wv + 1) * 64 + lane] = t.y; s_uf[(4 * wv + 2) * 64 + lane] = t.z;
         s_uf[(4 * wv + 3) * 64 + lane] = t.w;
       } else {
@@ -2087,8 +2113,9 @@
   M3 Rb_h = q2mat(Q4{0, 0, 0, 1});
   if (wv != 6) {
     if (carry_in) {
+      const LdsWin W(sh, lane);
       if (has_box) bpos_h = {SH(FS_CARRY_BP), SH(FS_CARRY_BP + 1), SH(FS_CARRY_BP + 2)};
-      base_chain<MS>(A, P, grav, N, e, B, false, sh + FS_CARRY_Q * 64, sh + FS_CARRY_QD * 64, lane);
+      base_chain<MS>(A, P, grav, N, e, B, false, &W, FS_CARRY_Q, FS_CARRY_QD);
       if (wv < 5) {
 #pragma unroll
         for (int l = 0; l < 4; l++) { fin.ql[l] = carry.ql[l]; fin.qdl[l] = carry.qdl[l]; fin.tg[l] = carry.tg[l]; }
@@ -2133,19 +2160,22 @@
     V3 ac = B.ao5 + cross(B.al5, rc) + cross(B.w5, cross(B.w5, rc));
     V3 f5 = comp5.m * ac;
     V3 n5 = mul(comp5.I, B.al5) + cross(B.w5, mul(comp5.I, B.w5)) + cross(rc, f5);
-    comp_put(sh, lane, DL_PALM, comp5, B.o5);
-    sh_put3(sh, lane, DL_PALM_WRENCH, f5); sh_put3(sh, lane, DL_PALM_WRENCH + 3, n5);
+    const LdsWin W(sh, lane);
+    const LdsQuadWin Q(sh, lane);
+    comp_put(W, DL_PALM, comp5, B.o5);
+    sh_put3(W, DL_PALM_WRENCH, f5); sh_put3(W, DL_PALM_WRENCH + 3, n5);
 #pragma unroll
     for (int i = 0; i < 6; i++) SH(FS_TGTB + i) = FLD(targets, i);
 #pragma unroll
     for (int i2 = 0; i2 < 3; i2++) {
       const V3 a0 = B.ab[2 * i2], o0 = B.ob[2 * i2], a1 = B.ab[2 * i2 + 1], o1 = B.ob[2 * i2 + 1];
-      *(f4*)(sh + FS_BCH * 64 + ROWADDR(12 * i2, lane)) = f4{a0.x, a0.y, a0.z, o0.x};
-      *(f4*)(sh + FS_BCH * 64 + ROWADDR(12 * i2 + 4, lane)) = f4{o0.y, o0.z, a1.x, a1.y};
-      *(f4*)(sh + FS_BCH * 64 + ROWADDR(12 * i2 + 8, lane)) = f4{a1.z, o1.x, o1.y, o1.z};
+      Q.flat(FS_BCH, 3 * i2) = f4{a0.x, a0.y, a0.z, o0.x};
+      Q.flat(FS_BCH, 3 * i2 + 1) = f4{o0.y, o0.z, a1.x, a1.y};
+      Q.flat(FS_BCH, 3 * i2 + 2) = f4{a1.z, o1.x, o1.y, o1.z};
     }
     schur_precompute(sh, dlb, lane, B, seq, cnt);
   } else if (wv == 6) {
+    const LdsWin W(sh, lane);
     float bv[6] = {0, 0, 0, 0, 0, 0};
     const int gen = FLD(wgen, 0);
     f4 wq[4];
@@ -2175,7 +2205,7 @@
           cpack |= i << (3 * k);
           const float gap = p.z - C.rest_offset;
           const V3 rb = p - bpos;
-          { float* rp = sh + (FS_CMP + 3 * k) * 64 + lane; rp[0] = rb.x; rp[64] = rb.y; rp[128] = rb.z; }
+          W.at(FS_CMP, 3 * k) = rb.x; W.at(FS_CMP + 1, 3 * k) = rb.y; W.at(FS_CMP + 2, 3 * k) = rb.z;
           const float cb = gap > 0.f ? div_n(gap, h) : -fminf(div_n(-gap * C.erp, h), C.max_depenetration_velocity);
           s_hdr[(4 * k) * 64 + lane] = __int_as_float(2); s_hdr[(4 * k + 1) * 64 + lane] = __int_as_float(-1);
           s_hdr[(4 * k + 2) * 64 + lane] = mu_bg; s_hdr[(4 * k + 3) * 64 + lane] = cb;
@@ -2209,7 +2239,7 @@
       int km = nc;
 #pragma unroll
       for (int s = 32; s >= 1; s >>= 1) km = max(km, __shfl_xor(km, s));
-      sb.load<false>(km, SH(FS_CMP_INVM), SH(FS_CMP_INVM + 1), s_lam, s_hdr, sh + FS_CMP * 64, 0, 0, lane, nc, true);
+      sb.load<false>(km, SH(FS_CMP_INVM), SH(FS_CMP_INVM + 1), s_lam, s_hdr, &W(FS_CMP), 0, 0, lane, nc, true);
       sb.warm(sv01, sv23, sv45, f2{SH(FS_CMP_INVM), SH(FS_CMP_INVM + 1)});
 #pragma unroll 1
       for (int it = 0; it < it_split && !box_conv; it++) {
@@ -2272,11 +2302,12 @@
 #endif
     if (early) {
 #pragma unroll
-      for (int i = 0; i < 6; i++) SH(FS_UB + i) = uB[i];
+      for (int i = 0; i < 6; i++) sh[(FS_UB + i) * 64 + lane] = uB[i];
     }
   }
   if (!hand_free) {
     int nloc = 0, tmask = 0;
+    const LdsWin W(sh, lane);
     const int cw = wv == 6 ? 0 : (wv == 0 ? -1 : wv);
     if (cw >= 0 && !((clear_mask >> cw) & 1)) {
       V3 bp = {0, 0, 0}; M3 Rbx = q2mat(Q4{0, 0, 0, 1});
@@ -2297,7 +2328,7 @@
         for (int c = 0; c < 3; c++) {
           const int l = 3 - c;
           caps[c] = 3 + 3 * cw + (l - 1);
-          E0[c] = sh_get3(sh, lane, DL_CAPS(dlb, cw) + 6 * (l - 1)); E1[c] = sh_get3(sh, lane, DL_CAPS(dlb, cw) + 6 * (l - 1) + 3);
+          E0[c] = sh_get3(W, DL_CAPS(dlb, 0) + 6 * (l - 1), 18 * cw); E1[c] = sh_get3(W, DL_CAPS(dlb, 0) + 6 * (l - 1) + 3, 18 * cw);
         }
       } else {
         const M3 R5 = q2mat(B.q5);
@@ -2326,7 +2357,7 @@
     }
     const int nbg0 = __float_as_int(SH(DL_NC)) & 0xff;
     PH2_STAMP(0);
-    if (cw >= 0) SH(FS_FLAG + cw) = __int_as_float(NP_TAG | ((clear_mask >> cw) & 1) | (nloc << 1) | (tmask << 8));
+    if (cw >= 0) W.at(FS_FLAG, cw) = __int_as_float(NP_TAG | ((clear_mask >> cw) & 1) | (nloc << 1) | (tmask << 8));
     __syncthreads();
     PH2_STAMP(1);
     if (cw >= 0) {
@@ -2393,11 +2424,12 @@
   PHASE_STAMP();
   __syncthreads();
 
-  nc = __float_as_int(SH(DL_NC));
+  nc = __float_as_int(sh[DL_NC * 64 + lane]);
   nbg = (nc >> 8) & 0xff; nc &= 0xff;
   const int n_items_wg = early ? 0 : __builtin_amdgcn_readfirstlane(__float_as_int(sh[FS_NITEM * 64]));
   const bool gp = !early && n_items_wg > 0;
   if (!early && !gp) {
+    const LdsWin W(sh, lane);
     if (wv == 0) {
 #pragma unroll
       for (int i = 0; i < 6; i++) SH(FS_UB + i) = uB[i];
@@ -2410,7 +2442,7 @@
         const f2 mI = {SH(FS_CMP_INVM), SH(FS_CMP_INVM + 1)};
         BoxBlock bb;
         f2 v01 = {SH(FS_BOXV), SH(FS_BOXV + 1)}, v23 = {SH(FS_BOXV + 2), SH(FS_BOXV + 3)}, v45 = {SH(FS_BOXV + 4), SH(FS_BOXV + 5)};
-        bb.load<false>(km, mI.x, mI.y, s_lam, s_hdr, sh + FS_CMP * 64, 0, 0, lane, nbg, true);
+        bb.load<false>(km, mI.x, mI.y, s_lam, s_hdr, &W(FS_CMP), 0, 0, lane, nbg, true);
         bb.warm(v01, v23, v45, mI);
 #pragma unroll 1
         for (int it = 0; it < C.num_position_iterations; it++) if (!__any(bb.sweep(v01, v23, v45))) break;
@@ -2427,8 +2459,10 @@
   if (gp) {
   {
     const f4 z4 = {0.f, 0.f, 0.f, 0.f};
-#pragma unroll
-    for (int q = 0; q < 10; q++) if (wv * 10 + q < 65) *XQ(0, wv * 10 + q) = z4;
+    const LdsWin W(sh, lane);
+    const LdsQuadWin Q(sh, lane);
+#pragma unroll
+    for (int q = 0; q < 10; q++) if (wv * 10 + q < 65) Q.qat(FS_X, q, wv * 10) = z4;
     if (wv == 0) {
       *TQ(0) = f4{uB[0], uB[1], uB[2], uB[3]};
       float* t1 = (float*)TQ(1);
@@ -2438,7 +2472,7 @@
       t1[2] = SH(FS_BOXV); t1[3] = SH(FS_BOXV + 1);
       *TQ(2) = f4{SH(FS_BOXV + 2), SH(FS_BOXV + 3), SH(FS_BOXV + 4), SH(FS_BOXV + 5)};
     }
-    if (wv < 5) *TQ(3 + wv) = f4{s_uf[(4 * wv) * 64 + lane], s_uf[(4 * wv + 1) * 64 + lane], s_uf[(4 * wv + 2) * 64 + lane], s_uf[(4 * wv + 3) * 64 + lane]};
+    if (wv < 5) *TQD(3, wv) = f4{s_uf[(4 * wv) * 64 + lane], s_uf[(4 * wv + 1) * 64 + lane], s_uf[(4 * wv + 2) * 64 + lane], s_uf[(4 * wv + 3) * 64 + lane]};
   }
 #pragma unroll
     for (int i = 0; i < 24; i++) Gkeep[i] = 0.f;
@@ -2463,7 +2497,7 @@
     __syncthreads();
   }
 #pragma unroll
-  for (int i = 0; i < 6; i++) uB[i] = SH(FS_UB + i);
+  for (int i = 0; i < 6; i++) uB[i] = sh[(FS_UB + i) * 64 + lane];
   const bool store_q = LAST || !carry_out || C.joint_limit_rows != 0;
   if (wv < 5) {
     const int f = wv;
@@ -2485,6 +2519,7 @@
       if (carry_out) { carry.ql[l] = qn; carry.qdl[l] = vn; carry.tg[l] = fin.tg[l]; }
     }
   } else if (wv == 5) {
+    const LdsWin W(sh, lane);
 #pragma unroll
     for (int i = 0; i < 6; i++) {
       float qn = 0.f, vn = 0.f;
@@ -2493,6 +2528,7 @@
     }
   } else {
     if (has_box) {
+      const LdsWin W(sh, lane);
       float vb[3], wb[3];
 #pragma unroll
       for (int i = 0; i < 3; i++) { vb[i] = SH(FS_BOXV + i); wb[i] = SH(FS_BOXV + 3 + i); }
```

Result: no change. 68.45 million, median of 6 (+0.1%).
